# rmcar17/SpectralClusterSupertree

Measured on AMD Instinct MI355X. Metric: top-level PCG build + Fiedler solve wall-time (s) at N taxa, 1/2/4/8 MI355X, lower is better.
Workload: dtype f64 (loop operator: fp32 image of W; fp64 renewal + confirmation)

## Files before the change

spectralclustersupertree_amd/csrc/scs_build.hip:

```cpp

#include <algorithm>

#include "scs_internal.h"

typedef unsigned long long u64;
typedef unsigned int u32;

constexpr u32 DEPTH_INF = 0xFFFFFFFFu;


__device__ __forceinline__ void rmq_offsets(int m, int a, int b, int (&o)[2]) {
    const int k = 31 - __clz(b - a);
    o[0] = k * m + a;
    o[1] = k * m + b - (1 << k);
}

template <typename K>
__device__ __forceinline__ K rmq_min(const K *__restrict__ base, int m, int a, int b) {
    int o[2];
    rmq_offsets(m, a, b, o);
    const K x = base[o[0]], y = base[o[1]];
    return x < y ? x : y;
}

// ... 31 lines not shown
}

__global__ void k_positions_values(const int64_t *__restrict__ tree_off,
                                   const int32_t *__restrict__ leaf_taxon,
                                   const int32_t *__restrict__ adj_depth,
                                   const double *__restrict__ adj_val,
                                   const double *__restrict__ tree_w, int t0, int tl0,
                                   int32_t *__restrict__ pos, int64_t npad,
                                   const int64_t *__restrict__ st_off, double *__restrict__ stv) {
    const int tl = tl0 + blockIdx.y;
    const int t = t0 + tl;
    const int64_t off = tree_off[t];
    const int n = (int)(tree_off[t + 1] - off);
    const int p = blockIdx.x * blockDim.x + threadIdx.x;
    if (p >= n) return;
    const unsigned tx = (unsigned)leaf_taxon[off + p];
    if (tx < (unsigned)npad) pos[(int64_t)tl * npad + tx] = p;
    if (p < n - 1)
        stv[st_off[tl] + p] = adj_depth[off + p] ? adj_val[off + p] * tree_w[t] : 0.0;
}

template <typename K, typename PICK>
__global__ void k_sparse_level(const int64_t *__restrict__ tree_off, int t0, int tl0, int k,
                               const int64_t *__restrict__ st_off, K *__restrict__ st,
                               const int64_t *__restrict__ am_off, argmin_t *__restrict__ am_all, PICK pick) {
    const int tl = tl0 + blockIdx.y;
    const int m = (int)(tree_off[t0 + tl + 1] - tree_off[t0 + tl]) - 1;
    const int p = blockIdx.x * blockDim.x + threadIdx.x;
    if (m < (1 << k) || p > m - (1 << k)) return;
    K *base = st + st_off[tl];
    const int half = 1 << (k - 1);
    const K a = base[(int64_t)(k - 1) * m + p], b = base[(int64_t)(k - 1) * m + p + half];
    base[(int64_t)k * m + p] = pick(a, b);
    if (k > ARGMIN_MAX_LEVEL) return;
    argmin_t *am = am_all + am_off[tl];
    const bool right = pick.right_less(a, b);
    int off = right ? half : 0;
    if (k > 1) off += (int)am[(int64_t)(k - 2) * m + p + (right ? half : 0)];
    am[(int64_t)(k - 1) * m + p] = (argmin_t)off;
}

constexpr int FUSED_UNROLL = 4;
template <typename K, typename PICK>
__global__ __launch_bounds__(1024) void k_sparse_levels_fused(const int64_t *__restrict__ tree_off, int t0, int tl0,
                                                               const int64_t *__restrict__ st_off,
                                                               K *__restrict__ st,
                                                               const int64_t *__restrict__ am_off,
                                                               argmin_t *__restrict__ am_all, PICK pick) {
    const int tl = tl0 + blockIdx.x;
    const int m = (int)(tree_off[t0 + tl + 1] - tree_off[t0 + tl]) - 1;
    K *base = st + st_off[tl];
    argmin_t *am = am_all + am_off[tl];
    for (int k = 1; (1 << k) <= m; ++k) {
        const K *prev = base + (int64_t)(k - 1) * m;
        K *cur = base + (int64_t)k * m;
        const int half = 1 << (k - 1), last = m - (1 << k);
        const argmin_t *am_prev = am + (int64_t)(k - 2) * m;
        argmin_t *am_cur = am + (int64_t)(k - 1) * m;
        for (int p0 = threadIdx.x; p0 <= last; p0 += 1024 * FUSED_UNROLL) {
            K a[FUSED_UNROLL], b[FUSED_UNROLL];
            int oa[FUSED_UNROLL], ob[FUSED_UNROLL];
#pragma unroll
            for (int u = 0; u < FUSED_UNROLL; ++u) {
                const int p = p0 + u * 1024;
                oa[u] = ob[u] = 0;
                if (p <= last) {
                    a[u] = prev[p];
                    b[u] = prev[p + half];
                    if (k > 1) {
                        oa[u] = (int)am_prev[p];
                        ob[u] = (int)am_prev[p + half];
                    }
                }
            }
#pragma unroll
            for (int u = 0; u < FUSED_UNROLL; ++u) {
                const int p = p0 + u * 1024;
                if (p <= last) {
                    cur[p] = pick(a[u], b[u]);
                    am_cur[p] = (argmin_t)(pick.right_less(a[u], b[u]) ? half + ob[u] : oa[u]);
                }
            }
        }
        __syncthreads();
    }
}
constexpr int SPARSE_FUSED_MAX_LEAVES = 32768;
static_assert(SPARSE_FUSED_MAX_LEAVES <= (1 << ARGMIN_MAX_LEVEL), "every level of a fused table has an argmin level");
struct pick_smaller_value {
    __device__ double operator()(double a, double b) const { return a < b ? a : b; }
    __device__ bool right_less(double a, double b) const { return b < a; }
};

__device__ __forceinline__ double min_f64(double a, double b) {
#ifdef SCS_MIN_ASM
    double r;
    asm("v_min_f64 %0, %1, %2" : "=v"(r) : "v"(a), "v"(b));
    return r;
#else
    return __builtin_fmin(a, b);
#endif
}

#include "scs_mono.h"
#include "scs_mono_wide.h"
#include "scs_gen.h"
struct pick_shallower_pair {
    __device__ gap_entry operator()(const gap_entry a, const gap_entry b) const { return gap_min(a, b); }
    __device__ bool right_less(const gap_entry a, const gap_entry b) const { return b.d < a.d; }
};

__global__ __launch_bounds__(256) void k_scatter_atomic(const int64_t *__restrict__ tree_off,
                                                         const int32_t *__restrict__ leaf_taxon, int t0,
                                                         const int64_t *__restrict__ st_off,
                                                         const double *__restrict__ stv,
                                                         double *__restrict__ w, int64_t ld) {
    const int tl = blockIdx.y;
    const int64_t off = tree_off[t0 + tl];
    const int nl = (int)(tree_off[t0 + tl + 1] - off);
    const int m = nl - 1;
    const int nbk = (nl + 63) / 64;
    int I = 0, rest = blockIdx.x;
    while (I < nbk && rest >= nbk - I) {
        rest -= nbk - I;
        ++I;
    }
    if (I >= nbk) return;
    const int J = I + rest;
    __shared__ int s_ta[64], s_tb[64];
    const int tid = threadIdx.x;
    if (tid < 64) s_ta[tid] = I * 64 + tid < nl ? leaf_taxon[off + I * 64 + tid] : -1;
    else if (tid < 128) s_tb[tid - 64] = J * 64 + tid - 64 < nl ? leaf_taxon[off + J * 64 + tid - 64] : -1;
    __syncthreads();
    const double *st = stv + st_off[tl];
    const int bj = tid & 63;
    const int pb = J * 64 + bj;
#pragma unroll 4
    for (int q = 0; q < 16; ++q) {
        const int ai = (tid >> 6) + 4 * q;
        const int pa = I * 64 + ai;
        if (pa >= pb || pb >= nl) continue;
        const double v = rmq_min<double>(st, m, pa, pb);
        if (v != 0.0) {
            const int ta = s_ta[ai], tb2 = s_tb[bj];
            atomicAdd(&w[(int64_t)ta * ld + tb2], v);
            atomicAdd(&w[(int64_t)tb2 * ld + ta], v);
        }
    }
}

__global__ __launch_bounds__(1024) void k_unpack_tiles(const double *__restrict__ gathered,
                                                      const int2 *__restrict__ tiles, int world,
                                                      int64_t chunk_doubles, int n, int row_begin,
                                                      int row_end, double *__restrict__ w,
                                                      int64_t ld) {
    const int tcw = blockDim.x;
    const int t = blockIdx.x;
    const int2 tile = tiles[t];
    const double *src = gathered + (int64_t)(t % world) * chunk_doubles +
                        (int64_t)(t / world) * SCS_TR * tcw;
    const int c = tile.y * tcw + threadIdx.x;
    if (c >= n) return;
    const int r0 = tile.x * SCS_TR;
    const bool col_is_my_row = c >= row_begin && c < row_end;
    for (int i = 0; i < SCS_TR; ++i) {
        const int r = r0 + i;
        if (r >= n) break;
        const double v = src[i * tcw + threadIdx.x];
        if (r >= row_begin && r < row_end) w[(int64_t)(r - row_begin) * ld + c] = v;
        if (col_is_my_row && ((r / tcw) + 1) * tcw <= (c / SCS_TR) * SCS_TR)
            w[(int64_t)(c - row_begin) * ld + r] = v;
    }
}

__global__ __launch_bounds__(256) void k_pack_tiles(const double *__restrict__ tile_out,
                                                    const int32_t *__restrict__ src_slot, int tcw,
                                                    double *__restrict__ sendbuf) {
    const double2 *src = (const double2 *)(tile_out + (int64_t)src_slot[blockIdx.x] * SCS_TR * tcw);
    double2 *dst = (double2 *)(sendbuf + (int64_t)blockIdx.x * SCS_TR * tcw);
    for (int q = threadIdx.x; q < SCS_TR * tcw / 2; q += 256) dst[q] = src[q];
}

__global__ __launch_bounds__(1024) void k_unpack_received(const double *__restrict__ recvbuf,
                                                         const int2 *__restrict__ tiles, int n,
                                                         int row_begin, int row_end,
                                                         double *__restrict__ w, int64_t ld) {
    const int tcw = blockDim.x;
    const int2 tile = tiles[blockIdx.x];
    const double *src = recvbuf + (int64_t)blockIdx.x * SCS_TR * tcw;
    const int c = tile.y * tcw + threadIdx.x;
    if (c >= n) return;
    const int r0 = tile.x * SCS_TR;
    const bool col_is_my_row = c >= row_begin && c < row_end;
    for (int i = 0; i < SCS_TR; ++i) {
        const int r = r0 + i;
        if (r >= n) break;
        const double v = src[i * tcw + threadIdx.x];
        if (r >= row_begin && r < row_end) w[(int64_t)(r - row_begin) * ld + c] = v;
        if (col_is_my_row && ((r / tcw) + 1) * tcw <= (c / SCS_TR) * SCS_TR)
            w[(int64_t)(c - row_begin) * ld + r] = v;
    }
}

__global__ void k_contract(const double *__restrict__ w, int64_t ld, int old_row_begin,
                           const int32_t *__restrict__ gstart, int g_begin, int g_end, int n_groups,
                           double *__restrict__ out, int64_t ld_out) {
    const int h = blockIdx.x * blockDim.x + threadIdx.x;
    if (h >= n_groups) return;
    const int c0 = gstart[h], c1 = gstart[h + 1];
    for (int g = g_begin + blockIdx.y; g < g_end; g += gridDim.y) {
        double best = 0.0;
        if (h != g) {
            const int r0 = gstart[g], r1 = gstart[g + 1];
            best = w[(int64_t)(r0 - old_row_begin) * ld + c0];
            for (int r = r0; r < r1; ++r)
                for (int c = c0; c < c1; ++c) {
                    const double v = w[(int64_t)(r - old_row_begin) * ld + c];
                    best = v > best ? v : best;
                }
        }
        out[(int64_t)(g - g_begin) * ld_out + h] = best;
    }
}

template <bool IMG>
__global__ __launch_bounds__(256) void k_degrees(const double *__restrict__ w, int64_t ld, int n,
                                                  int rows, int row_begin,
                                                  double *__restrict__ deg_full,
                                                  float *__restrict__ w32 = nullptr, int w32_full = 0) {
    const int lane = threadIdx.x & 63;
    const int r = blockIdx.x * 4 + (threadIdx.x >> 6);
    if (r >= rows) return;
    const double *row = w + (int64_t)r * ld;
    double s0 = 0.0, s1 = 0.0;
    const int n2 = n & ~1;
    const int c0 = w32_full ? 0 : (row_begin + r) / 512 * 512;
    float *row32 = IMG ? w32 + (int64_t)r * ld : nullptr;
    for (int j = lane * 2; j < n2; j += 128) {
        const double2 v = *(const double2 *)(row + j);
        s0 += v.x;
        s1 += v.y;
        if (IMG && j >= c0) *(float2 *)(row32 + j) = make_float2((float)v.x, (float)v.y);
    }
    if (IMG)
        for (int j = n2 + lane; j < ld; j += 64) row32[j] = (float)row[j];
    if ((n & 1) && lane == 0) s0 += row[n - 1];
    double s = s0 + s1;
#pragma unroll
    for (int o = 32; o > 0; o >>= 1) s += __shfl_xor(s, o, 64);
    if (lane == 0) deg_full[row_begin + r] = s;
}

__global__ __launch_bounds__(256) void k_degrees_upper_rows(const double *__restrict__ w, int64_t ld, int n,
                                                             int rows, int row_begin, int col0,
                                                             double *__restrict__ part) {
    const int lane = threadIdx.x & 63;
    const int rl = blockIdx.x * 4 + (threadIdx.x >> 6);
    if (rl >= rows) return;
    const int r = row_begin + rl;
    const int c0 = r / 256 * 256;
    const double *row = w + (int64_t)rl * ld + (c0 - col0);
    const int cnt = n - c0;
    double s0 = 0.0, s1 = 0.0;
    const int n2 = cnt & ~1;
    for (int j = lane * 2; j < n2; j += 128) {
        const double2 v = *(const double2 *)(row + j);
        s0 += v.x;
        s1 += v.y;
    }
    if ((cnt & 1) && lane == 0) s0 += row[cnt - 1];
    double s = s0 + s1;
#pragma unroll
    for (int o = 32; o > 0; o >>= 1) s += __shfl_xor(s, o, 64);
    if (lane == 0) part[r] = s;
}

__global__ __launch_bounds__(256) void k_degrees_upper_cols(const double *__restrict__ w, int64_t ld, int n,
                                                             int row_begin, int row_end, int col0,
                                                             double *__restrict__ part) {
    const int c = col0 + blockIdx.x * blockDim.x + threadIdx.x;
    if (c >= n) return;
    const int r_end = min(row_end, c / 256 * 256);
    double s = 0.0;
    for (int r = row_begin; r < r_end; ++r) s += w[(int64_t)(r - row_begin) * ld + (c - col0)];
    if (r_end > row_begin) part[c] += s;
}

__global__ void k_combine_degrees(const double *__restrict__ gathered, int world, int n,
                                  double *__restrict__ deg) {
    const int i = blockIdx.x * blockDim.x + threadIdx.x;
    if (i >= n) return;
    double d = 0.0;
    for (int r = 0; r < world; ++r) d += gathered[(int64_t)r * n + i];
    deg[i] = d;
}

__global__ void k_dinv(const double *__restrict__ deg, int n, double *__restrict__ dinv) {
    const int i = blockIdx.x * blockDim.x + threadIdx.x;
    if (i >= n) return;
    const double d = deg[i];
    dinv[i] = d == 0.0 ? 1.0 : 1.0 / sqrt(d);
}

namespace {

struct dev_buf {
    scs_ctx *ctx;
    void *p = nullptr;
    explicit dev_buf(scs_ctx *c) : ctx(c) {}
    ~dev_buf() {
        if (p) scs_dev_free(p);
    }
    int alloc(size_t bytes) {
        if (p) scs_dev_free(p);
        p = nullptr;
        SCS_HIP_CHECK(scs_dev_malloc(ctx, &p, bytes ? bytes : 16));
        return SCS_OK;
    }
};

struct cached_buf {
    scs_ctx *ctx;
    void *p = nullptr;
    explicit cached_buf(scs_ctx *c) : ctx(c) {}
    ~cached_buf() {
        if (p) scs_block_release(ctx, p);
    }
    int alloc(size_t bytes) {
        if (p) scs_block_release(ctx, p);
        p = nullptr;
        return scs_block_alloc(ctx, bytes, &p);
    }
};

struct pooled_buf {
    scs_ctx *ctx = nullptr;
    int slot = 0;
    void *p = nullptr;
    pooled_buf(scs_ctx *c, int s) : ctx(c), slot(s) {}
    ~pooled_buf() {
        auto &sl = ctx->scratch[slot];
        if (sl.cap > SCS_SCRATCH_KEEP) {
            scs_dev_free(sl.p);
            sl.p = nullptr;
            sl.cap = 0;
        }
    }
    int alloc(size_t bytes) {
        auto &sl = ctx->scratch[slot];
        if (bytes < 16) bytes = 16;
        if (sl.cap < bytes) {
            if (sl.p) scs_dev_free(sl.p);
            sl.p = nullptr;
            sl.cap = 0;
            SCS_HIP_CHECK(scs_dev_malloc(ctx, &sl.p, bytes));
            sl.cap = bytes;
        }
        p = sl.p;
        return SCS_OK;
    }
};

struct ev_pair {
    hipEvent_t a = nullptr, b = nullptr;
    ~ev_pair() {
        if (a) hipEventDestroy(a);
        if (b) hipEventDestroy(b);
    }
    int init() {
        SCS_HIP_CHECK(hipEventCreate(&a));
        SCS_HIP_CHECK(hipEventCreate(&b));
        return SCS_OK;
    }
};

int levels_for(int64_t m) {
    int l = 0;
    while (((int64_t)1 << l) <= m) ++l;
    return l;
}

}

static int graph_alloc(scs_ctx *ctx, int32_t n, int32_t row_begin, int32_t row_end,
                       hipStream_t stream, scs_graph **out, int32_t col0 = 0) {
    auto *g = new scs_graph();
    g->n = n;
    g->row_begin = row_begin;
    g->row_end = row_end;
    g->col0 = col0;
    g->upper = col0 > 0 || false;
    g->ld = scs_round_up(n - col0, SCS_LD_ALIGN);
    const size_t rows = (size_t)(row_end - row_begin);
    size_t bytes = rows * (size_t)g->ld * sizeof(double);
    if (bytes < 16) bytes = 16;
    {
        const int rc = scs_block_alloc(ctx, bytes, (void **)&g->d_w);
        if (rc != SCS_OK) {
            delete g;
            return rc;
        }
        g->w_bytes = bytes;
        g->w_block = true;
    }
    if (g->ld > n - col0) {
        hipError_t e = hipMemset2DAsync(g->d_w + (n - col0), (size_t)g->ld * 8, 0,
                                        (size_t)(g->ld - (n - col0)) * 8, rows, stream);
        if (e != hipSuccess) {
            if (g->w_block) scs_block_release(ctx, g->d_w);
            else scs_dev_free(g->d_w);
            delete g;
            scs_set_error("cannot clear the padding of W: %s", hipGetErrorString(e));
            return SCS_EHIP;
        }
    }
    *out = g;
    return SCS_OK;
}

extern "C" int scs_graph_free(scs_ctx *ctx, scs_graph *g) {
    if (!g) return SCS_OK;
    if (ctx) hipSetDevice(ctx->device);
    if (g->mf) {
        if (ctx) hipStreamSynchronize(ctx->stream);
        scs_matfree_release(g);
    }
    if (ctx && g->d_w && g->w_block) {
        scs_block_release(ctx, g->d_w);
    } else if (ctx && g->d_w) {
        if (!ctx->w_cache || g->w_bytes >= ctx->w_cache_bytes) {
            if (ctx->w_cache) scs_dev_free(ctx->w_cache);
            ctx->w_cache = g->d_w;
            ctx->w_cache_bytes = g->w_bytes;
        } else {
            scs_dev_free(g->d_w);
        }
    } else {
        scs_dev_free(g->d_w);
    }
    if (ctx && g->deg_stage) {
        hipStreamSynchronize(ctx->stream);
        scs_pinned_release(ctx, g->deg_stage);
    }
    if (ctx) {
        if (g->d_w32) {
            std::lock_guard<std::mutex> lock(ctx->cache_mu);
            if (scs_dbg("SCS_TRACE_SOLVES") && atoi(scs_dbg("SCS_TRACE_SOLVES")) && ctx->w32_cache)
                fprintf(stderr, "[image] hipFree of %.2f GB\n",
                        std::min(g->w32_bytes, ctx->w32_cache_bytes) / 1073741824.0);
            scs_dev_free(g->d_w32);
        }
        if (g->d_deg) scs_block_release(ctx, g->d_deg);
        if (g->d_dinv) scs_block_release(ctx, g->d_dinv);
    } else {
        scs_dev_free(g->d_w32);
        scs_dev_free(g->d_deg);
        scs_dev_free(g->d_dinv);
    }
    delete g;
    return SCS_OK;
}

extern "C" int scs_graph_shape(const scs_graph *g, int32_t *n, int32_t *rb, int32_t *re) {
    SCS_REQUIRE(g != nullptr, "scs_graph_shape: null graph");
    if (n) *n = g->n;
    if (rb) *rb = g->row_begin;
    if (re) *re = g->row_end;
    return SCS_OK;
}

int scs_gather_row_splits(scs_ctx *ctx, int32_t row_begin, int32_t row_end, int32_t n,
                          std::vector<int32_t> &splits) {
    const int world = ctx->comm.world;
    splits.assign(world + 1, 0);
    if (world == 1) {
        splits[0] = row_begin;
        splits[1] = row_end;
        return SCS_OK;
    }
    dev_buf send(ctx), recv(ctx);
    SCS_TRY(send.alloc(8));
    SCS_TRY(recv.alloc(8 * (size_t)world));
    double v = (double)row_begin;
    SCS_HIP_CHECK(hipMemcpyAsync(send.p, &v, 8, hipMemcpyHostToDevice, ctx->stream));
    SCS_TRY(scs_comm_allgather_f64(&ctx->comm, (const double *)send.p, (double *)recv.p, 1, ctx->stream));
    std::vector<double> h(world);
    SCS_HIP_CHECK(hipMemcpyAsync(h.data(), recv.p, 8 * (size_t)world, hipMemcpyDeviceToHost, ctx->stream));
    SCS_HIP_CHECK(hipStreamSynchronize(ctx->stream));
    for (int r = 0; r < world; ++r) splits[r] = (int32_t)h[r];
    splits[world] = n;
    for (int r = 0; r < world; ++r)
        SCS_REQUIRE(splits[r] < splits[r + 1], "row partition is not contiguous by rank");
    SCS_REQUIRE(splits[0] == 0 && splits[ctx->comm.rank] == row_begin && splits[ctx->comm.rank + 1] == row_end,
                "row partition does not tile [0, V)");
    return SCS_OK;
}

__global__ __launch_bounds__(64) void k_col_presence(const int32_t *__restrict__ pos, int64_t npad, int n,
                                                      int cols_per_group, int n_batch,
                                                      unsigned char *__restrict__ pcol) {
    const int cg = blockIdx.x, t = blockIdx.y, lane = threadIdx.x;
    bool any = false;
    for (int c = cg * cols_per_group + lane; c < min(n, (cg + 1) * cols_per_group); c += 64)
        any = any || pos[(int64_t)t * npad + c] >= 0;
    if (__ballot(any) != 0 && lane == 0) pcol[(int64_t)cg * n_batch + t] = 1;
    if (__ballot(any) == 0 && lane == 0) pcol[(int64_t)cg * n_batch + t] = 0;
}

__global__ void k_tile_lists(const int2 *__restrict__ tiles, int n_tiles, const unsigned char *__restrict__ rec,
                             int rec_bytes, int cnt_off, int n_batch, const unsigned char *__restrict__ pcol,
                             int32_t *__restrict__ lists, int32_t *__restrict__ list_cnt) {
    const int i = blockIdx.x * blockDim.x + threadIdx.x;
    if (i >= n_tiles) return;
    const int2 tile = tiles[i];
    const unsigned char *rb = rec + (int64_t)tile.x * n_batch * rec_bytes + cnt_off;
    const unsigned char *pc = pcol + (int64_t)tile.y * n_batch;
    int32_t *out = lists + (int64_t)i * n_batch;
    int c = 0;
    for (int t = 0; t < n_batch; ++t)
        if (pc[t] && *(const int *)(rb + (int64_t)t * rec_bytes) > 0) out[c++] = t;
    list_cnt[i] = c;
}

constexpr int PIPE_NG = 2;

namespace {

enum { PREP_MONO = 0, PREP_WIDE = 1, PREP_GEN = 2, PREP_NO_RECORDS = 3 };

struct prep_batch {
    const scs_tables *tb;
    int t0, nb;
    int kind;
    int32_t *pos;
    int64_t npad;
    const int64_t *st_off;
    const int64_t *am_off;
    void *st;
    argmin_t *am;
    unsigned char *rec;
    int n_blocks, row_begin, row_end;
};

int64_t table_entries(int64_t m) { return (int64_t)levels_for(m) * m; }
int64_t argmin_entries(int64_t m) { return (int64_t)argmin_levels(levels_for(m)) * m; }

int prep_piece(const prep_batch &b, int tl0, int np, hipStream_t s) {
    if (np <= 0) return SCS_OK;
    const scs_tables *tb = b.tb;
    int max_levels = 0;
    int64_t max_n = 0;
    for (int t = b.t0 + tl0; t < b.t0 + tl0 + np; ++t) {
        const int64_t nt = tb->h_tree_off[t + 1] - tb->h_tree_off[t];
        max_levels = std::max(max_levels, levels_for(nt - 1));
        max_n = std::max(max_n, nt);
    }
    const dim3 grid_l((unsigned)((max_n + 255) / 256), (unsigned)np);
    const dim3 grid_r((unsigned)b.n_blocks, (unsigned)np);
    const bool fused = max_n <= SPARSE_FUSED_MAX_LEAVES && max_levels > 1;
    if (b.kind != PREP_GEN) {
        double *st = (double *)b.st;
        k_positions_values<<<grid_l, 256, 0, s>>>(tb->d_tree_off, tb->d_leaf_taxon, tb->d_adj_depth, tb->d_adj_val,
                                                  tb->d_tree_w, b.t0, tl0, b.pos, b.npad, b.st_off, st);
        if (fused)
            k_sparse_levels_fused<double><<<(unsigned)np, 1024, 0, s>>>(tb->d_tree_off, b.t0, tl0, b.st_off, st, b.am_off,
                                                                        b.am, pick_smaller_value{});
        else
            for (int k = 1; k < max_levels; ++k)
                k_sparse_level<double><<<grid_l, 256, 0, s>>>(tb->d_tree_off, b.t0, tl0, k, b.st_off, st, b.am_off, b.am,
                                                              pick_smaller_value{});
        if (b.kind == PREP_WIDE)
            k_block_records_wide<PIPE_NG><<<grid_r, 64, 0, s>>>(tb->d_tree_off, b.t0, tl0, b.nb, b.pos, b.npad, b.st_off, st,
                                                          b.am_off, b.am, b.row_begin, b.row_end, b.rec);
        else if (b.kind == PREP_MONO)
            k_block_records_mono<<<grid_r, 64, 0, s>>>(tb->d_tree_off, b.t0, tl0, b.nb, b.pos, b.npad, b.st_off, st,
                                                       b.am_off, b.am, b.row_begin, b.row_end, b.rec);
    } else {
        gap_entry *st = (gap_entry *)b.st;
        k_positions_pairs<<<grid_l, 256, 0, s>>>(tb->d_tree_off, tb->d_leaf_taxon, tb->d_adj_depth, tb->d_adj_val,
                                                 tb->d_tree_w, b.t0, tl0, b.pos, b.npad, b.st_off, st);
        if (fused)
            k_sparse_levels_fused<gap_entry><<<(unsigned)np, 1024, 0, s>>>(tb->d_tree_off, b.t0, tl0, b.st_off, st,
                                                                           b.am_off, b.am, pick_shallower_pair{});
        else
            for (int k = 1; k < max_levels; ++k)
                k_sparse_level<gap_entry><<<grid_l, 256, 0, s>>>(tb->d_tree_off, b.t0, tl0, k, b.st_off, st, b.am_off,
                                                                 b.am, pick_shallower_pair{});
        k_block_records_gen<<<grid_r, 64, 0, s>>>(tb->d_tree_off, b.t0, tl0, b.nb, b.pos, b.npad, b.st_off, st, b.am_off,
                                                  b.am, b.row_begin, b.row_end, b.rec);
    }
    SCS_HIP_CHECK(hipGetLastError());
    return SCS_OK;
}

struct pinned_ref {
    scs_ctx *ctx;
    hipStream_t stream;
    void *p = nullptr;
    bool in_flight = false;
    pinned_ref(scs_ctx *c, hipStream_t s) : ctx(c), stream(s) {}
    ~pinned_ref() {
        if (!p) return;
        if (in_flight) hipStreamSynchronize(stream);
        scs_pinned_release(ctx, p);
    }
};

}

extern "C" int scs_pcg_build(scs_ctx *ctx, const scs_tables *tb, int32_t row_begin,
                             int32_t row_end, int32_t flags, scs_graph **out,
                             scs_build_stats *stats) {
    SCS_REQUIRE(ctx && tb && out, "scs_pcg_build: null argument");
    SCS_REQUIRE((flags & ~(SCS_BUILD_MONOTONE | SCS_BUILD_SHARED | SCS_BUILD_UPPER | SCS_BUILD_SCATTER)) == 0,
                "scs_pcg_build: unknown flag bits 0x%x", flags);
    const bool scatter = (flags & SCS_BUILD_SCATTER) != 0;
    if (scatter && tb) SCS_TRY(scs_tables_finish(ctx, tb));
    if (scatter) {
        if (!(flags & SCS_BUILD_MONOTONE) || (flags & (SCS_BUILD_SHARED | SCS_BUILD_UPPER)) ||
            row_begin != 0 || row_end != tb->n_taxa || ctx->comm.world != 1) {
            scs_set_error("scs_pcg_build: SCS_BUILD_SCATTER (the atomic comparison variant) takes monotone "
                          "tables, the whole matrix, one rank");
            return SCS_EUNSUP;
        }
    }
    SCS_REQUIRE((flags & (SCS_BUILD_SHARED | SCS_BUILD_UPPER)) != (SCS_BUILD_SHARED | SCS_BUILD_UPPER),
                "scs_pcg_build: SCS_BUILD_SHARED and SCS_BUILD_UPPER exclude each other");
    const bool monotone = (flags & SCS_BUILD_MONOTONE) != 0 &&
                          !(scs_dbg("SCS_NO_MONOTONE") && atoi(scs_dbg("SCS_NO_MONOTONE")));
    const int n = tb->n_taxa;
    SCS_REQUIRE(row_begin >= 0 && row_begin < row_end && row_end <= n,
                "scs_pcg_build: bad row range [%d, %d) for %d taxa", row_begin, row_end, n);
    SCS_HIP_CHECK(hipSetDevice(ctx->device));
    hipStream_t s = ctx->stream;
    const int world = ctx->comm.world, rank = ctx->comm.rank;
    const int cols_per_tile = MONO_TCW;
    static_assert(MONO_TCW == SCS_TCW, "one tile width for all kernels");
    const size_t entry_bytes = monotone ? 8 : sizeof(gap_entry);
    size_t rec_bytes = monotone ? R3_BYTES : G3_BYTES;
    const int n_cgroups = (n + cols_per_tile - 1) / cols_per_tile;
    const int64_t npad = scs_round_up((int64_t)n_cgroups * cols_per_tile, SCS_NPAD);
    bool shared = (flags & SCS_BUILD_SHARED) != 0 && world > 1;
    if (shared) {
        const int64_t nb_all = (n + SCS_TR - 1) / SCS_TR;
        const double tile_bytes = 0.5 * (double)nb_all * n_cgroups * SCS_TR * cols_per_tile * 8.0;
        if (tile_bytes * (1.0 + 1.0 / world) > 96.0 * 1024 * 1024 * 1024) shared = false;
    }
    const int b_row_begin = shared ? 0 : row_begin, b_row_end = shared ? n : row_end;
    const bool sym = !shared && (row_begin == 0 && row_end == n && world == 1);
    const bool trapezoid = (flags & SCS_BUILD_UPPER) != 0;
    if (trapezoid)
        SCS_REQUIRE(row_begin % cols_per_tile == 0,
                    "scs_pcg_build: SCS_BUILD_UPPER needs row_begin (%d) to be a multiple of %d", row_begin,
                    cols_per_tile);
    const bool upper = sym || shared || trapezoid;
    const int gb0 = b_row_begin / SCS_TR;
    const int rows = row_end - row_begin;
    const int n_blocks = (b_row_end - b_row_begin + SCS_TR - 1) / SCS_TR;

    scs_graph *g = nullptr;
    SCS_TRY(graph_alloc(ctx, n, row_begin, row_end, s, &g, trapezoid ? row_begin : 0));
    g->upper = trapezoid;
    if (scatter) SCS_HIP_CHECK(hipMemsetAsync(g->d_w, 0, (size_t)rows * (size_t)g->ld * 8, s));
    double *w_base = g->d_w - g->col0;
    struct guard {
        scs_ctx *c;
        scs_graph *g;
        ~guard() {
            if (g) scs_graph_free(c, g);
        }
    } gd{ctx, g};

    std::vector<int2> tiles;
    tiles.reserve((size_t)n_blocks * n_cgroups);
    for (int b = 0; b < n_blocks; ++b)
        for (int c = 0; c < n_cgroups; ++c) {
            if (upper && (int64_t)(c + 1) * cols_per_tile <= (int64_t)(gb0 + b) * SCS_TR) continue;
            tiles.push_back(make_int2(b, c));
        }
    {
        const bool per_xcd = !(scs_dbg("SCS_TILE_ORDER") && atoi(scs_dbg("SCS_TILE_ORDER")) == 0);
        auto xcd_reorder = [](std::vector<int2> &v) {
            if (v.size() <= 8) return;
            std::vector<int2> per[8];
            for (const int2 &t : v) per[t.x & 7].push_back(t);
            std::vector<int2> ordered;
            ordered.reserve(v.size());
            size_t at[8] = {0, 0, 0, 0, 0, 0, 0, 0};
            while (ordered.size() < v.size())
                for (int x = 0; x < 8; ++x)
                    if (at[x] < per[x].size()) ordered.push_back(per[x][at[x]++]);
            v.swap(ordered);
        };
        if (per_xcd && !shared) {
            xcd_reorder(tiles);
        } else if (per_xcd) {
            std::vector<std::vector<int2>> share(world);
            for (size_t i = 0; i < tiles.size(); ++i) share[i % world].push_back(tiles[i]);
            for (auto &v : share) xcd_reorder(v);
            for (int r = 0; r < world; ++r)
                for (size_t k = 0; k < share[r].size(); ++k) tiles[(size_t)world * k + r] = share[r][k];
        }
    }
    std::vector<int2> all_tiles;
    dev_buf d_all_tiles(ctx);
    cached_buf d_tile_out(ctx), d_gathered(ctx);
    size_t chunk_doubles = 0;
    const bool exchange_allgather =
        scs_dbg("SCS_EXCHANGE") && std::string(scs_dbg("SCS_EXCHANGE")) == "allgather";
    if (shared) {
        all_tiles.swap(tiles);
        for (size_t i = rank; i < all_tiles.size(); i += world) tiles.push_back(all_tiles[i]);
        const size_t slots = (all_tiles.size() + world - 1) / world;
        chunk_doubles = slots * SCS_TR * cols_per_tile;
        SCS_TRY(d_all_tiles.alloc(all_tiles.size() * sizeof(int2)));
        SCS_HIP_CHECK(hipMemcpyAsync(d_all_tiles.p, all_tiles.data(),
                                     all_tiles.size() * sizeof(int2), hipMemcpyHostToDevice, s));
        SCS_TRY(d_tile_out.alloc(chunk_doubles * 8));
        if (exchange_allgather) SCS_TRY(d_gathered.alloc(chunk_doubles * 8 * world));
        if (tiles.size() < slots)
            SCS_HIP_CHECK(hipMemsetAsync((double *)d_tile_out.p + (slots - 1) * SCS_TR * cols_per_tile,
                                         0, (size_t)SCS_TR * cols_per_tile * 8, s));
    }
    pooled_buf d_tiles(ctx, 0);
    SCS_TRY(d_tiles.alloc(std::max<size_t>(tiles.size(), 1) * sizeof(int2)));
    SCS_HIP_CHECK(hipMemcpyAsync(d_tiles.p, tiles.data(), tiles.size() * sizeof(int2),
                                 hipMemcpyHostToDevice, s));

    bool tree_par = sym && !scatter && !tiles.empty() && tiles.size() <= 24 && tb->n_trees >= 128;
    if (const char *e = scs_dbg("SCS_TREE_PARALLEL")) tree_par = sym && !scatter && !tiles.empty() && atoi(e) != 0;
    const size_t cells_per_tree = tiles.size() * (size_t)SCS_TR * cols_per_tile * 8;

    const size_t wide_min_tiles = 13;
    bool listed = monotone && !scatter && !tiles.empty() && tb->n_trees > 0 &&
                  (double)tb->n_leaves / ((double)tb->n_trees * std::max(n, 1)) < 1.0 / 64.0;
    if (const char *e = scs_dbg("SCS_TILE_LISTS")) listed = monotone && !scatter && !tiles.empty() && atoi(e) != 0;
    if (listed) tree_par = false;
    int wide_mode = (monotone && !scatter && !tree_par && !listed && tiles.size() >= wide_min_tiles) ? 3 : 0;
    bool wide_forced = false;
    if (const char *e = scs_dbg("SCS_WIDE")) {
        wide_mode = (monotone && !scatter && !tiles.empty() && atoi(e)) ? 3 : 0;
        wide_forced = wide_mode != 0;
        if (wide_mode) listed = false;
    }
    if (wide_mode && ctx->max_lds_bytes < (int)spec_layout::LDS_BYTES) {
        wide_mode = 0;
        wide_forced = false;
    }
    if (wide_mode) tree_par = false;
    const bool wide = wide_mode != 0;
    const int group_tiles = PIPE_NG;
    std::vector<int4> groups;
    dev_buf d_groups(ctx);
    if (wide) {
        rec_bytes = wide_layout<PIPE_NG>::BYTES;
        std::vector<std::vector<int>> of_block((size_t)n_blocks);
        for (size_t i = 0; i < tiles.size(); ++i) of_block[(size_t)tiles[i].x].push_back((int)i);
        std::vector<int4> per[8];
        for (int b = 0; b < n_blocks; ++b) {
            const std::vector<int> &v = of_block[(size_t)b];
            for (size_t k = 0; k < v.size(); k += group_tiles)
                per[b & 7].push_back(make_int4(v[k], k + 1 < v.size() ? v[k + 1] : -1,
                                               (group_tiles > 2 && k + 2 < v.size()) ? v[k + 2] : -1, 0));
        }
        size_t total = 0, at[8] = {0, 0, 0, 0, 0, 0, 0, 0};
        for (auto &v : per) total += v.size();
        groups.reserve(total);
        while (groups.size() < total)
            for (int x = 0; x < 8; ++x)
                if (at[x] < per[x].size()) groups.push_back(per[x][at[x]++]);
        SCS_TRY(d_groups.alloc(groups.size() * sizeof(int4)));
        SCS_HIP_CHECK(hipMemcpyAsync(d_groups.p, groups.data(), groups.size() * sizeof(int4),
                                     hipMemcpyHostToDevice, s));
    }

    const int M = tb->n_trees;
    std::vector<int> batch_start{0};
    {
        const int batch_trees_env = scs_dbg("SCS_BATCH_TREES") ? atoi(scs_dbg("SCS_BATCH_TREES")) : 0;
        int max_batch_trees = 256;
        {
            const double avg_leaves = (double)tb->n_leaves / std::max(M, 1);
            const double table_bytes =
                (double)table_entries((int64_t)std::max(avg_leaves - 1.0, 1.0)) * (double)entry_bytes;
            max_batch_trees = (int)std::min(256.0, std::max(64.0, 600e6 / std::max(table_bytes, 1.0)));
        }
        if (n <= 2048) max_batch_trees = 4096;
        const int arrived = tb->late_start.empty() ? M : tb->late_start[0];
        if (wide) {
            const int rest = M - (arrived < M ? arrived : 0);
            const int k = std::max(1, (rest + 511) / 512);
            max_batch_trees = std::max(96, (rest + k - 1) / k);
        }
        if (tree_par)
            max_batch_trees = (int)std::max<size_t>(16, std::min<size_t>((size_t)max_batch_trees,
                                                                         SCS_SCRATCH_KEEP / cells_per_tree));
        if (batch_trees_env > 0) max_batch_trees = batch_trees_env;
        if (tree_par)
            max_batch_trees = (int)std::max<size_t>(1, std::min<size_t>((size_t)max_batch_trees,
                                                                        SCS_SCRATCH_KEEP / std::max<size_t>(cells_per_tree, 1)));
        size_t used = 0;
        for (int t = 0; t < M; ++t) {
            const int64_t nt = tb->h_tree_off[t + 1] - tb->h_tree_off[t];
            const int64_t m = nt - 1;
            const size_t need = (size_t)table_entries(m) * entry_bytes + (size_t)argmin_entries(m) * sizeof(argmin_t) +
                                (size_t)npad * 4 + (size_t)n_blocks * rec_bytes;
            if ((used + need > ctx->ws_limit || t - batch_start.back() >= max_batch_trees ||
                 (t == arrived && batch_start.size() == 1)) &&
                t > batch_start.back()) {
                batch_start.push_back(t);
                used = 0;
            }
            used += need;
        }
        batch_start.push_back(M);
    }
    const int n_batches = (int)batch_start.size() - 1;

    struct ev_ref {
        hipEvent_t a, b;
    } ev_total, ev_prep, ev_acc;
    for (auto &e : ctx->build_events)
        if (!e) SCS_HIP_CHECK(hipEventCreate(&e));
    ev_total = {ctx->build_events[0], ctx->build_events[1]};
    ev_prep = {ctx->build_events[2], ctx->build_events[3]};
    ev_acc = {ctx->build_events[4], ctx->build_events[5]};
    float prep_ms = 0.f, acc_ms = 0.f;
    SCS_HIP_CHECK(hipEventRecord(ev_total.a, s));

    int spec_batches = 0, spec_trees = 0;
    float spec_ms = 0.f;
    bool single_batch_spec = false;
    pooled_buf d_pos(ctx, 1), d_am(ctx, 2), d_st(ctx, 3), d_stoff(ctx, 4), d_rec(ctx, 5), d_cells(ctx, 6);
    dev_buf d_pcol(ctx), d_lists(ctx), d_list_cnt(ctx);
    int listed_batches = 0;
    std::vector<size_t> off_at((size_t)n_batches + 1, 0);
    for (int bi = 0; bi < n_batches; ++bi)
        off_at[bi + 1] = off_at[bi] + 2 * (size_t)(batch_start[bi + 1] - batch_start[bi] + 1);
    pinned_ref h_off(ctx, s);
    SCS_TRY(scs_pinned_get(ctx, std::max<size_t>(off_at[n_batches], 2) * 8, &h_off.p));
    {
        int64_t *h = (int64_t *)h_off.p;
        for (int bi = 0; bi < n_batches; ++bi) {
            const int t0 = batch_start[bi], nb = batch_start[bi + 1] - t0;
            int64_t *st_off = h + off_at[bi], *am_off = st_off + nb + 1;
            st_off[0] = am_off[0] = 0;
            for (int t = 0; t < nb; ++t) {
                const int64_t m = tb->h_tree_off[t0 + t + 1] - tb->h_tree_off[t0 + t] - 1;
                st_off[t + 1] = st_off[t] + table_entries(m);
                am_off[t + 1] = am_off[t] + argmin_entries(m);
            }
        }
        SCS_TRY(d_stoff.alloc(off_at[n_batches] * 8));
        h_off.in_flight = true;
        SCS_HIP_CHECK(hipMemcpyAsync(d_stoff.p, h, off_at[n_batches] * 8, hipMemcpyHostToDevice, s));
    }
    const bool by_arrival = !(scs_dbg("SCS_PREP_BY_ARRIVAL") && atoi(scs_dbg("SCS_PREP_BY_ARRIVAL")) == 0);
    int prep_pieces = 0;
    for (int bi = 0; bi < n_batches; ++bi) {
        const int t0 = batch_start[bi], t1 = batch_start[bi + 1];
        const int nb = t1 - t0;
        const int64_t *h_st_off = (const int64_t *)h_off.p + off_at[bi], *h_am_off = h_st_off + nb + 1;
        int64_t max_n = 0;
        for (int t = t0; t < t1; ++t) max_n = std::max(max_n, tb->h_tree_off[t + 1] - tb->h_tree_off[t]);
        const size_t need_pos = (size_t)nb * npad * 4;
        const size_t need_st = (size_t)h_st_off[nb] * entry_bytes + 64;
        const size_t need_am = (size_t)h_am_off[nb] * sizeof(argmin_t) + 64;
        const size_t need_rec = (size_t)n_blocks * nb * rec_bytes;
        const int wide_min_trees = wide_forced ? 1 : 96;
        const bool wide_b = wide && (nb >= wide_min_trees || (groups.size() >= 8 * 256 && nb >= 16));
        if (wide_b) {
            ++spec_batches;
            spec_trees += nb;
            single_batch_spec = true;
        }
        SCS_TRY(d_pos.alloc(need_pos));
        SCS_TRY(d_st.alloc(need_st));
        SCS_TRY(d_am.alloc(need_am));
        SCS_TRY(d_rec.alloc(need_rec));

        SCS_HIP_CHECK(hipEventRecord(ev_prep.a, s));
        SCS_HIP_CHECK(hipMemsetAsync(d_pos.p, 0xFF, need_pos, s));
        prep_batch pb;
        pb.tb = tb;
        pb.t0 = t0;
        pb.nb = nb;
        pb.kind = !monotone ? PREP_GEN : wide_b ? PREP_WIDE : scatter ? PREP_NO_RECORDS : PREP_MONO;
        pb.pos = (int32_t *)d_pos.p;
        pb.npad = npad;
        pb.st_off = (const int64_t *)d_stoff.p + off_at[bi];
        pb.am_off = pb.st_off + nb + 1;
        pb.st = d_st.p;
        pb.am = (argmin_t *)d_am.p;
        pb.rec = (unsigned char *)d_rec.p;
        pb.n_blocks = n_blocks;
        pb.row_begin = b_row_begin;
        pb.row_end = b_row_end;
        for (int p0 = t0; p0 < t1;) {
            int p1 = t1;
            if (by_arrival)
                for (const int32_t c : tb->late_start)
                    if (c > p0 && c < p1) p1 = c;
            SCS_TRY(scs_tables_wait(ctx, tb, p1, s));
            SCS_TRY(prep_piece(pb, p0 - t0, p1 - p0, s));
            ++prep_pieces;
            p0 = p1;
        }
        SCS_HIP_CHECK(hipEventRecord(ev_prep.b, s));

        SCS_HIP_CHECK(hipEventRecord(ev_acc.a, s));
        const unsigned nt = (unsigned)tiles.size();
        if (scatter) {
            const int64_t nbk = (max_n + 63) / 64;
            k_scatter_atomic<<<dim3((unsigned)(nbk * (nbk + 1) / 2), (unsigned)nb), 256, 0, s>>>(
                tb->d_tree_off, tb->d_leaf_taxon, t0, pb.st_off, (const double *)d_st.p,
                g->d_w, g->ld);
        } else if (monotone) {
            mono_params mp;
            mp.tiles = (const int2 *)d_tiles.p;
            mp.rec = (const unsigned char *)d_rec.p;
            mp.pos = (const int32_t *)d_pos.p;
            mp.npad = npad;
            mp.stv = (const double *)d_st.p;
            mp.n_batch = nb;
            mp.w = w_base;
            mp.ld = g->ld;
            mp.n = n;
            mp.row_begin = b_row_begin;
            mp.row_end = b_row_end;
            mp.load_w = bi > 0;
            mp.mirror = (sym && bi == n_batches - 1) ? 1 : 0;
            mp.tile_out = shared ? (double *)d_tile_out.p : nullptr;
            mp.stamps = nullptr;
            mp.split_tiles = 0;
            mp.lists = nullptr;
            mp.list_cnt = nullptr;
            const bool stamp = scs_dbg("SCS_ACC_STAMP") && atoi(scs_dbg("SCS_ACC_STAMP"));
            if (wide_b) {
                wide_params wp;
                wp.m = mp;
                wp.groups = (const int4 *)d_groups.p;
                wp.producer_prio = 2;
                const unsigned ng = (unsigned)groups.size();
                dev_buf d_st8(ctx);
                if (stamp) {
                    SCS_TRY(d_st8.alloc(64));
                    SCS_HIP_CHECK(hipMemsetAsync(d_st8.p, 0, 64, s));
                    wp.m.stamps = (unsigned long long *)d_st8.p;
                }
#define SCS_LAUNCH_SPEC(SYM_, STAMP_)                                                                   \
    do {                                                                                                \
        SCS_HIP_CHECK(hipFuncSetAttribute((const void *)k_accumulate_spec<SYM_, STAMP_>,                \
                                          hipFuncAttributeMaxDynamicSharedMemorySize,                   \
                                          (int)spec_layout::LDS_BYTES));                                \
        k_accumulate_spec<SYM_, STAMP_><<<ng, spec_layout::THREADS, spec_layout::LDS_BYTES, s>>>(wp);   \
    } while (0)
                if (ng) {
                    if (stamp && sym) SCS_LAUNCH_SPEC(true, true);
                    else if (stamp) SCS_LAUNCH_SPEC(false, true);
                    else if (sym) SCS_LAUNCH_SPEC(true, false);
                    else SCS_LAUNCH_SPEC(false, false);
                }
#undef SCS_LAUNCH_SPEC
                if (stamp) {
                    unsigned long long h[8];
                    SCS_HIP_CHECK(hipMemcpyAsync(h, d_st8.p, 64, hipMemcpyDeviceToHost, s));
                    SCS_HIP_CHECK(hipStreamSynchronize(s));
                    const char *nm[5] = {"producer: pairs of the next tree", "producer: records + search + wait",
                                         "consumer: pair + table state", "consumer: cells + expansion", "barrier"};
                    double tot = 0;
                    for (int i = 0; i < 5; ++i) tot += (double)h[i];
                    for (int i = 0; i < 5; ++i)
                        fprintf(stderr, "[stamp spec] %-36s %6.2f %%  (%.0f cycles per wave-step)\n", nm[i],
                                100.0 * h[i] / tot, (double)h[i] / ((double)h[7] * nb));
                }
            } else if (nt && stamp) {
                dev_buf d_st8(ctx);
                SCS_TRY(d_st8.alloc(64));
                SCS_HIP_CHECK(hipMemsetAsync(d_st8.p, 0, 64, s));
                mp.stamps = (unsigned long long *)d_st8.p;
                if (sym) k_accumulate_mono<true, true><<<nt, MONO_TCW, 0, s>>>(mp);
                else k_accumulate_mono<false, true><<<nt, MONO_TCW, 0, s>>>(mp);
                unsigned long long h[8];
                SCS_HIP_CHECK(hipMemcpyAsync(h, d_st8.p, 64, hipMemcpyDeviceToHost, s));
                SCS_HIP_CHECK(hipStreamSynchronize(s));
                const char *nm[7] = {"wait loads+record", "barrier A", "combine", "search + issue",
                                     "expand", "barrier B", "cells"};
                double tot = 0;
                for (int i = 0; i < 7; ++i) tot += (double)h[i];
                for (int i = 0; i < 7; ++i)
                    fprintf(stderr, "[stamp] %-24s %6.2f %%  (%.0f cycles per wave-step)\n", nm[i],
                            100.0 * h[i] / tot, (double)h[i] / ((double)h[7] * nb));
            } else if (nt && tree_par) {
                SCS_TRY(d_cells.alloc((size_t)nb * cells_per_tree));
                mono_params ap = mp;
                ap.split_tiles = (int)nt;
                ap.load_w = 0;
                ap.mirror = 0;
                ap.tile_out = (double *)d_cells.p;
                k_accumulate_mono<true, false><<<nt * (unsigned)nb, MONO_TCW, 0, s>>>(ap);
                k_sum_tree_tiles<true, mono_params><<<nt * SCS_TR, MONO_TCW, 0, s>>>(mp, (const double *)d_cells.p,
                                                                                    (int)nt);
            } else if (nt && listed) {
                SCS_TRY(d_pcol.alloc((size_t)n_cgroups * nb));
                SCS_TRY(d_lists.alloc((size_t)nt * nb * 4));
                SCS_TRY(d_list_cnt.alloc((size_t)nt * 4));
                k_col_presence<<<dim3((unsigned)n_cgroups, (unsigned)nb), 64, 0, s>>>(
                    (const int32_t *)d_pos.p, npad, n, cols_per_tile, nb, (unsigned char *)d_pcol.p);
                k_tile_lists<<<(nt + 255) / 256, 256, 0, s>>>((const int2 *)d_tiles.p, (int)nt,
                                                             (const unsigned char *)d_rec.p, R3_BYTES, R3_CNT, nb,
                                                             (const unsigned char *)d_pcol.p, (int32_t *)d_lists.p,
                                                             (int32_t *)d_list_cnt.p);
                mp.lists = (const int32_t *)d_lists.p;
                mp.list_cnt = (const int32_t *)d_list_cnt.p;
                if (sym) k_accumulate_mono<true, false, true><<<nt, MONO_TCW, 0, s>>>(mp);
                else k_accumulate_mono<false, false, true><<<nt, MONO_TCW, 0, s>>>(mp);
                ++listed_batches;
            } else if (nt) {
                if (sym) k_accumulate_mono<true, false><<<nt, MONO_TCW, 0, s>>>(mp);
                else k_accumulate_mono<false, false><<<nt, MONO_TCW, 0, s>>>(mp);
            }
        } else {
            gen_params gp;
            gp.tiles = (const int2 *)d_tiles.p;
            gp.rec = (const unsigned char *)d_rec.p;
            gp.pos = (const int32_t *)d_pos.p;
            gp.npad = npad;
            gp.ste = (const gap_entry *)d_st.p;
            gp.n_batch = nb;
            gp.w = w_base;
            gp.ld = g->ld;
            gp.n = n;
            gp.row_begin = b_row_begin;
            gp.row_end = b_row_end;
            gp.load_w = bi > 0;
            gp.mirror = (sym && bi == n_batches - 1) ? 1 : 0;
            gp.tile_out = shared ? (double *)d_tile_out.p : nullptr;
            gp.split_tiles = 0;
            if (nt && tree_par) {
                SCS_TRY(d_cells.alloc((size_t)nb * cells_per_tree));
                gen_params ap = gp;
                ap.split_tiles = (int)nt;
                ap.load_w = 0;
                ap.mirror = 0;
                ap.tile_out = (double *)d_cells.p;
                k_accumulate_gen<true><<<nt * (unsigned)nb, MONO_TCW, 0, s>>>(ap);
                k_sum_tree_tiles<true, gen_params><<<nt * SCS_TR, MONO_TCW, 0, s>>>(gp, (const double *)d_cells.p,
                                                                                   (int)nt);
            } else if (nt) {
                if (sym) k_accumulate_gen<true><<<nt, MONO_TCW, 0, s>>>(gp);
                else k_accumulate_gen<false><<<nt, MONO_TCW, 0, s>>>(gp);
            }
        }
        SCS_HIP_CHECK(hipGetLastError());
        SCS_HIP_CHECK(hipEventRecord(ev_acc.b, s));
        if (n_batches > 1) {
            SCS_HIP_CHECK(hipEventSynchronize(ev_acc.b));
            float ms = 0.f;
            SCS_HIP_CHECK(hipEventElapsedTime(&ms, ev_prep.a, ev_prep.b));
            prep_ms += ms;
            SCS_HIP_CHECK(hipEventElapsedTime(&ms, ev_acc.a, ev_acc.b));
            acc_ms += ms;
            if (wide_b) spec_ms += ms;
        }
    }
    float exch_ms = 0.f;
    double exch_bytes = 0.0;
    if (shared && exchange_allgather) {
        ev_pair ev_x;
        SCS_TRY(ev_x.init());
        SCS_HIP_CHECK(hipEventRecord(ev_x.a, s));
        SCS_TRY(scs_comm_allgather_f64(&ctx->comm, (const double *)d_tile_out.p,
                                       (double *)d_gathered.p, chunk_doubles, s));
        k_unpack_tiles<<<(unsigned)all_tiles.size(), cols_per_tile, 0, s>>>(
            (const double *)d_gathered.p, (const int2 *)d_all_tiles.p, world,
            (int64_t)chunk_doubles, n, row_begin, row_end, g->d_w, g->ld);
        SCS_HIP_CHECK(hipGetLastError());
        SCS_HIP_CHECK(hipEventRecord(ev_x.b, s));
        SCS_HIP_CHECK(hipEventSynchronize(ev_x.b));
        SCS_HIP_CHECK(hipEventElapsedTime(&exch_ms, ev_x.a, ev_x.b));
        exch_bytes = (double)chunk_doubles * 8.0 * (world - 1);
    } else if (shared) {
        std::vector<int32_t> splits;
        SCS_TRY(scs_gather_row_splits(ctx, row_begin, row_end, n, splits));
        auto needs = [&](int dst, const int2 &t) {
            const int64_t lo = splits[dst], hi = splits[dst + 1];
            const int64_t r_lo = (int64_t)t.x * SCS_TR, r_hi = std::min<int64_t>(r_lo + SCS_TR, n);
            const int64_t c_lo = (int64_t)t.y * cols_per_tile, c_hi = std::min<int64_t>(c_lo + cols_per_tile, n);
            return (r_lo < hi && lo < r_hi) || (c_lo < hi && lo < c_hi);
        };
        std::vector<int64_t> send_off(world + 1, 0), recv_off(world + 1, 0);
        std::vector<int32_t> send_slots;
        std::vector<int2> recv_tiles;
        for (int p = 0; p < world; ++p) {
            for (size_t i = rank; i < all_tiles.size(); i += world)
                if (needs(p, all_tiles[i])) send_slots.push_back((int32_t)(i / world));
            send_off[p + 1] = (int64_t)send_slots.size() * SCS_TR * cols_per_tile;
            for (size_t i = p; i < all_tiles.size(); i += world)
                if (needs(rank, all_tiles[i])) recv_tiles.push_back(all_tiles[i]);
            recv_off[p + 1] = (int64_t)recv_tiles.size() * SCS_TR * cols_per_tile;
        }
        cached_buf d_send(ctx), d_recv(ctx);
        dev_buf d_slots(ctx), d_rtiles(ctx);
        SCS_TRY(d_send.alloc((size_t)send_off[world] * 8));
        SCS_TRY(d_recv.alloc((size_t)recv_off[world] * 8));
        SCS_TRY(d_slots.alloc(send_slots.size() * 4));
        SCS_TRY(d_rtiles.alloc(recv_tiles.size() * sizeof(int2)));
        ev_pair ev_x;
        SCS_TRY(ev_x.init());
        SCS_HIP_CHECK(hipEventRecord(ev_x.a, s));
        SCS_HIP_CHECK(hipMemcpyAsync(d_slots.p, send_slots.data(), send_slots.size() * 4,
                                     hipMemcpyHostToDevice, s));
        SCS_HIP_CHECK(hipMemcpyAsync(d_rtiles.p, recv_tiles.data(), recv_tiles.size() * sizeof(int2),
                                     hipMemcpyHostToDevice, s));
        if (!send_slots.empty())
            k_pack_tiles<<<(unsigned)send_slots.size(), 256, 0, s>>>(
                (const double *)d_tile_out.p, (const int32_t *)d_slots.p, cols_per_tile, (double *)d_send.p);
        SCS_HIP_CHECK(hipGetLastError());
        SCS_TRY(scs_comm_alltoallv_f64(&ctx->comm, (const double *)d_send.p, send_off.data(),
                                       (double *)d_recv.p, recv_off.data(), s));
        if (!recv_tiles.empty())
            k_unpack_received<<<(unsigned)recv_tiles.size(), cols_per_tile, 0, s>>>(
                (const double *)d_recv.p, (const int2 *)d_rtiles.p, n, row_begin, row_end, g->d_w,
                g->ld);
        SCS_HIP_CHECK(hipGetLastError());
        SCS_HIP_CHECK(hipEventRecord(ev_x.b, s));
        SCS_HIP_CHECK(hipEventSynchronize(ev_x.b));
        SCS_HIP_CHECK(hipEventElapsedTime(&exch_ms, ev_x.a, ev_x.b));
        exch_bytes = (double)(recv_off[world] - (recv_off[rank + 1] - recv_off[rank])) * 8.0;
    }
    SCS_HIP_CHECK(hipEventRecord(ev_total.b, s));
    SCS_HIP_CHECK(hipEventSynchronize(ev_total.b));
    h_off.in_flight = false;
    SCS_TRY(scs_tables_finish(ctx, tb));
    float total_ms = 0.f;
    SCS_HIP_CHECK(hipEventElapsedTime(&total_ms, ev_total.a, ev_total.b));
    if (n_batches == 1) {
        SCS_HIP_CHECK(hipEventElapsedTime(&prep_ms, ev_prep.a, ev_prep.b));
        SCS_HIP_CHECK(hipEventElapsedTime(&acc_ms, ev_acc.a, ev_acc.b));
        if (single_batch_spec) spec_ms = acc_ms;
    }

    if (stats) {
        memset(stats, 0, sizeof(*stats));
        stats->n_taxa = n;
        stats->n_trees = M;
        stats->row_begin = row_begin;
        stats->row_end = row_end;
        stats->symmetric = shared ? 2 : (sym ? 1 : 0);
        stats->exchange_ms = exch_ms;
        stats->exchange_bytes = exch_bytes;
        stats->n_tiles = (int32_t)tiles.size();
        stats->n_batches = n_batches;
        stats->spec_batches = spec_batches;
        stats->tree_parallel_batches = tree_par ? n_batches : 0;
        stats->spec_trees = spec_trees;
        stats->listed_batches = listed_batches;
        stats->prep_pieces = prep_pieces;
        stats->spec_ms = spec_ms;
        stats->cell_trees = (double)tiles.size() * SCS_TR * cols_per_tile * (double)M;
        stats->prep_ms = prep_ms;
        stats->accumulate_ms = acc_ms;
        stats->total_ms = total_ms;
        stats->bytes_w = 8.0 * rows * (double)n;
        stats->bytes_tables = 16.0 * (double)tb->n_leaves + 8.0 * M;
    }
    gd.g = nullptr;
    *out = g;
    return SCS_OK;
}

extern "C" int scs_graph_contract(scs_ctx *ctx, scs_graph *g, const int32_t *group_start,
                                  int32_t n_groups, scs_graph **out) {
    SCS_REQUIRE(ctx && g && group_start && out, "scs_graph_contract: null argument");
    if (g->mf) {
        scs_set_error("scs_graph_contract: a matrix-free graph has no matrix to contract");
        return SCS_EUNSUP;
    }
    if (g->upper) {
        scs_set_error("scs_graph_contract: an SCS_BUILD_UPPER graph holds no whole rows; build it "
                      "row-partitioned (SCS_BUILD_SHARED) when the node contracts");
        return SCS_EUNSUP;
    }
    SCS_REQUIRE(n_groups >= 1 && n_groups <= g->n, "scs_graph_contract: bad group count %d",
                n_groups);
    SCS_REQUIRE(group_start[0] == 0 && group_start[n_groups] == g->n,
                "scs_graph_contract: group_start must span [0, %d]", g->n);
    int g_begin = -1, g_end = -1;
    for (int i = 0; i < n_groups; ++i) {
        SCS_REQUIRE(group_start[i] < group_start[i + 1], "scs_graph_contract: empty group %d", i);
        if (group_start[i] == g->row_begin) g_begin = i;
        if (group_start[i + 1] == g->row_end) g_end = i + 1;
    }
    SCS_REQUIRE(g_begin >= 0 && g_end > g_begin,
                "scs_graph_contract: a group straddles this rank's row block [%d, %d)",
                g->row_begin, g->row_end);
    SCS_HIP_CHECK(hipSetDevice(ctx->device));
    scs_graph *ng = nullptr;
    SCS_TRY(graph_alloc(ctx, n_groups, g_begin, g_end, ctx->stream, &ng));
    int32_t *d_gs = nullptr;
    hipError_t e = scs_dev_malloc(ctx, (void **)&d_gs, (size_t)(n_groups + 1) * 4);
    if (e != hipSuccess) {
        scs_graph_free(ctx, ng);
        scs_set_error("scs_graph_contract: hipMalloc failed: %s", hipGetErrorString(e));
        return SCS_ENOMEM;
    }
    hipMemcpyAsync(d_gs, group_start, (size_t)(n_groups + 1) * 4, hipMemcpyHostToDevice,
                   ctx->stream);
    dim3 grid((unsigned)((n_groups + 255) / 256), (unsigned)std::min(g_end - g_begin, 65535));
    k_contract<<<grid, 256, 0, ctx->stream>>>(g->d_w, g->ld, g->row_begin, d_gs, g_begin, g_end,
                                              n_groups, ng->d_w, ng->ld);
    e = hipGetLastError();
    if (e == hipSuccess) e = hipStreamSynchronize(ctx->stream);
    scs_dev_free(d_gs);
    if (e != hipSuccess) {
        scs_graph_free(ctx, ng);
        scs_set_error("scs_graph_contract: kernel failed: %s", hipGetErrorString(e));
        return SCS_EHIP;
    }
    scs_graph_free(ctx, g);
    *out = ng;
    return SCS_OK;
}

extern "C" int scs_graph_download_rows(scs_ctx *ctx, const scs_graph *g, int32_t first, int32_t count,
                                       double *out);

extern "C" int scs_graph_download(scs_ctx *ctx, const scs_graph *g, double *out) {
    SCS_REQUIRE(ctx && g && out, "scs_graph_download: null argument");
    SCS_REQUIRE(!g->mf, "scs_graph_download: a matrix-free graph has no matrix");
    SCS_HIP_CHECK(hipSetDevice(ctx->device));
    SCS_HIP_CHECK(hipStreamSynchronize(ctx->stream));
    const size_t rows = (size_t)(g->row_end - g->row_begin);
    if (g->upper) return scs_graph_download_rows(ctx, g, g->row_begin, (int32_t)rows, out);
    SCS_HIP_CHECK(hipMemcpy2D(out, (size_t)g->n * 8, g->d_w, (size_t)g->ld * 8, (size_t)g->n * 8,
                              rows, hipMemcpyDeviceToHost));
    return SCS_OK;
}

extern "C" int scs_graph_download_rows(scs_ctx *ctx, const scs_graph *g, int32_t first,
                                       int32_t count, double *out) {
    SCS_REQUIRE(ctx && g && out, "scs_graph_download_rows: null argument");
    SCS_REQUIRE(!g->mf, "scs_graph_download_rows: a matrix-free graph has no matrix");
    SCS_REQUIRE(count >= 1 && first >= g->row_begin && first + count <= g->row_end,
                "scs_graph_download_rows: rows [%d, %d) outside this rank's block [%d, %d)", first,
                first + count, g->row_begin, g->row_end);
    SCS_HIP_CHECK(hipSetDevice(ctx->device));
    SCS_HIP_CHECK(hipStreamSynchronize(ctx->stream));
    if (g->upper) {
        const size_t wcols = (size_t)(g->n - g->col0);
        for (int32_t i = 0; i < count; ++i) memset(out + (size_t)i * g->n, 0, (size_t)g->n * 8);
        SCS_HIP_CHECK(hipMemcpy2D(out + g->col0, (size_t)g->n * 8,
                                  g->d_w + (int64_t)(first - g->row_begin) * g->ld, (size_t)g->ld * 8,
                                  wcols * 8, (size_t)count, hipMemcpyDeviceToHost));
        for (int32_t i = 0; i < count; ++i) {
            const int32_t c0 = (first + i) / 256 * 256;
            if (c0 > g->col0) memset(out + (size_t)i * g->n + g->col0, 0, (size_t)(c0 - g->col0) * 8);
        }
        return SCS_OK;
    }
    SCS_HIP_CHECK(hipMemcpy2D(out, (size_t)g->n * 8, g->d_w + (int64_t)(first - g->row_begin) * g->ld,
                              (size_t)g->ld * 8, (size_t)g->n * 8, (size_t)count,
                              hipMemcpyDeviceToHost));
    return SCS_OK;
}

int scs_graph_prepare_degrees_begin(scs_ctx *ctx, scs_graph *g, bool want_w32) {
    if (g->deg_stage) return SCS_OK;
    const int n = g->n;
    const int rows = g->row_end - g->row_begin;
    if (g->mf && !g->have_deg) {
        SCS_HIP_CHECK(hipSetDevice(ctx->device));
        hipStream_t s = ctx->stream;
        if (!g->d_deg) SCS_TRY(scs_block_alloc(ctx, (size_t)n * 8, (void **)&g->d_deg));
        if (!g->d_dinv) SCS_TRY(scs_block_alloc(ctx, (size_t)n * 8, (void **)&g->d_dinv));
        SCS_TRY(scs_matfree_apply(ctx, g, nullptr, 0, 4, nullptr, s));
        k_dinv<<<(n + 255) / 256, 256, 0, s>>>(g->d_deg, n, g->d_dinv);
        SCS_HIP_CHECK(hipGetLastError());
        SCS_TRY(scs_pinned_get(ctx, (size_t)n * 8, &g->deg_stage));
        SCS_HIP_CHECK(hipMemcpyAsync(g->deg_stage, g->d_deg, (size_t)n * 8, hipMemcpyDeviceToHost, s));
        return SCS_OK;
    }
    const bool img_rows = ctx->comm.world > 1 && !g->upper;
    bool need_img = want_w32 && !g->have_w32 && !g->upper &&
                    (img_rows || (ctx->comm.world == 1 && g->row_begin == 0 && rows == n));
    if (g->have_deg && !need_img) return SCS_OK;
    SCS_HIP_CHECK(hipSetDevice(ctx->device));
    hipStream_t s = ctx->stream;
    if (need_img && !g->d_w32) {
        const size_t need = (size_t)rows * g->ld * 4;
        std::lock_guard<std::mutex> lock(ctx->cache_mu);
        if (ctx->w32_cache && ctx->w32_cache_bytes >= need) {
            g->d_w32 = ctx->w32_cache;
            g->w32_bytes = ctx->w32_cache_bytes;
            ctx->w32_cache = nullptr;
            ctx->w32_cache_bytes = 0;
        } else if (scs_dev_malloc(ctx, (void **)&g->d_w32, need) == hipSuccess) {
            g->w32_bytes = need;
            if (scs_dbg("SCS_TRACE_SOLVES") && atoi(scs_dbg("SCS_TRACE_SOLVES")))
                fprintf(stderr, "[image] hipMalloc of %.2f GB\n", need / 1073741824.0);
        } else {
            (void)hipGetLastError();
            g->d_w32 = nullptr;
            need_img = false;
        }
    }
    if (!need_img && g->have_deg) return SCS_OK;
    if (need_img && img_rows && g->have_deg) {
        dev_buf tmp(ctx);
        SCS_TRY(tmp.alloc((size_t)n * 8));
        k_degrees<true><<<(rows + 3) / 4, 256, 0, s>>>(g->d_w, g->ld, n, rows, g->row_begin, (double *)tmp.p, g->d_w32, 1);
        SCS_HIP_CHECK(hipGetLastError());
        SCS_HIP_CHECK(hipStreamSynchronize(s));
        g->have_w32 = true;
        return SCS_OK;
    }
    if (!g->d_deg) SCS_TRY(scs_block_alloc(ctx, (size_t)n * 8, (void **)&g->d_deg));
    if (!g->d_dinv) SCS_TRY(scs_block_alloc(ctx, (size_t)n * 8, (void **)&g->d_dinv));
    const int world = ctx->comm.world;
    if (need_img && !img_rows) {
        k_degrees<true><<<(rows + 3) / 4, 256, 0, s>>>(g->d_w, g->ld, n, rows, g->row_begin, g->d_deg, g->d_w32);
        g->have_w32 = true;
    } else if (world == 1 && !g->upper) {
        k_degrees<false><<<(rows + 3) / 4, 256, 0, s>>>(g->d_w, g->ld, n, rows, g->row_begin, g->d_deg);
    } else {
        dev_buf send(ctx), recv(ctx);
        SCS_TRY(send.alloc((size_t)n * 8));
        SCS_TRY(recv.alloc((size_t)n * 8 * world));
        SCS_HIP_CHECK(hipMemsetAsync(send.p, 0, (size_t)n * 8, s));
        if (g->upper) {
            k_degrees_upper_rows<<<(rows + 3) / 4, 256, 0, s>>>(g->d_w, g->ld, n, rows, g->row_begin,
                                                                g->col0, (double *)send.p);
            k_degrees_upper_cols<<<(n - g->col0 + 255) / 256, 256, 0, s>>>(
                g->d_w, g->ld, n, g->row_begin, g->row_end, g->col0, (double *)send.p);
        } else if (need_img) {
            k_degrees<true><<<(rows + 3) / 4, 256, 0, s>>>(g->d_w, g->ld, n, rows, g->row_begin, (double *)send.p,
                                                           g->d_w32, 1);
            g->have_w32 = true;
        } else
        k_degrees<false><<<(rows + 3) / 4, 256, 0, s>>>(g->d_w, g->ld, n, rows, g->row_begin,
                                                        (double *)send.p);
        SCS_TRY(scs_comm_allgather_f64(&ctx->comm, (const double *)send.p, (double *)recv.p,
                                       (size_t)n, s));
        k_combine_degrees<<<(n + 255) / 256, 256, 0, s>>>((const double *)recv.p, world, n, g->d_deg);
        SCS_HIP_CHECK(hipGetLastError());
        SCS_HIP_CHECK(hipStreamSynchronize(s));
    }
    if (g->have_deg) {
        SCS_HIP_CHECK(hipGetLastError());
        return SCS_OK;
    }
    k_dinv<<<(n + 255) / 256, 256, 0, s>>>(g->d_deg, n, g->d_dinv);
    SCS_HIP_CHECK(hipGetLastError());
    SCS_TRY(scs_pinned_get(ctx, (size_t)n * 8, &g->deg_stage));
    SCS_HIP_CHECK(hipMemcpyAsync(g->deg_stage, g->d_deg, (size_t)n * 8, hipMemcpyDeviceToHost, s));
    return SCS_OK;
}

int scs_graph_prepare_degrees(scs_ctx *ctx, scs_graph *g) {
    if (g->have_deg) return SCS_OK;
    SCS_TRY(scs_graph_prepare_degrees_begin(ctx, g));
    const hipError_t e = hipStreamSynchronize(ctx->stream);
    const double *deg = (const double *)g->deg_stage;
    int iso = 0;
    double nrm2 = 0.0;
    if (e == hipSuccess)
        for (int i = 0; i < g->n; ++i) {
            if (deg[i] == 0.0) {
                ++iso;
                nrm2 += 1.0;
            } else {
                nrm2 += deg[i];
            }
        }
    scs_pinned_release(ctx, g->deg_stage);
    g->deg_stage = nullptr;
    SCS_HIP_CHECK(e);
    g->n_isolated = iso;
    g->dd_norm = sqrt(nrm2);
    g->have_deg = true;
    return SCS_OK;
}

extern "C" int scs_graph_degrees(scs_ctx *ctx, scs_graph *g, double *out) {
    SCS_REQUIRE(ctx && g && out, "scs_graph_degrees: null argument");
    SCS_TRY(scs_graph_prepare_degrees(ctx, g));
    SCS_HIP_CHECK(hipMemcpy(out, g->d_deg + g->row_begin,
                            (size_t)(g->row_end - g->row_begin) * 8, hipMemcpyDeviceToHost));
    return SCS_OK;
}

extern "C" int scs_debug_graph_raw(scs_ctx *ctx, scs_graph *g, int32_t what, void *out, int32_t *info_out) {
    SCS_REQUIRE(ctx && g && info_out, "scs_debug_graph_raw: null argument");
    SCS_REQUIRE(what >= 0 && what <= 2, "scs_debug_graph_raw: what must be 0 (W), 1 (image) or 2 (degrees), not %d",
                what);
    if (g->mf && what != 2) {
        scs_set_error("scs_debug_graph_raw: a matrix-free graph has neither a matrix nor an image");
        return SCS_EUNSUP;
    }
    const int rows = g->row_end - g->row_begin;
    const bool img_rows = ctx->comm.world > 1;
    if (what == 1) {
        if (g->upper) {
            scs_set_error("scs_debug_graph_raw: an SCS_BUILD_UPPER graph has no image");
            return SCS_EUNSUP;
        }
        if (!img_rows && !(g->row_begin == 0 && rows == g->n)) {
            scs_set_error("scs_debug_graph_raw: a row block [%d, %d) of %d on one rank has no image", g->row_begin,
                          g->row_end, g->n);
            return SCS_EUNSUP;
        }
    }
    info_out[0] = rows;
    info_out[1] = (int32_t)g->ld;
    info_out[2] = g->col0;
    info_out[3] = (what == 1 && img_rows) ? 1 : 0;
    if (!out) return SCS_OK;
    SCS_HIP_CHECK(hipSetDevice(ctx->device));
    if (what == 1) {
        SCS_TRY(scs_graph_prepare_degrees_begin(ctx, g, true));
        SCS_TRY(scs_graph_prepare_degrees(ctx, g));
        if (!g->have_w32 || !g->d_w32) {
            scs_set_error("scs_debug_graph_raw: the image could not be made (no memory)");
            return SCS_EUNSUP;
        }
    }
    if (what == 2) SCS_TRY(scs_graph_prepare_degrees(ctx, g));
    SCS_HIP_CHECK(hipStreamSynchronize(ctx->stream));
    if (what == 2)
        SCS_HIP_CHECK(hipMemcpy(out, g->d_deg, (size_t)g->n * 8, hipMemcpyDeviceToHost));
    else if (what == 1)
        SCS_HIP_CHECK(hipMemcpy(out, g->d_w32, (size_t)rows * (size_t)g->ld * 4, hipMemcpyDeviceToHost));
    else
        SCS_HIP_CHECK(hipMemcpy(out, g->d_w, (size_t)rows * (size_t)g->ld * 8, hipMemcpyDeviceToHost));
    return SCS_OK;
}

extern "C" int scs_debug_block_records(scs_ctx *ctx, const scs_tables *tb, int32_t t_begin, int32_t t_end,
                                       int32_t row_begin, int32_t row_end, int32_t kind, int32_t *spos_out,
                                       double *gap_out, int32_t *argpos_out, int32_t *depth_out, int32_t *cnt_out) {
    SCS_REQUIRE(ctx && tb && spos_out && gap_out && argpos_out && cnt_out, "scs_debug_block_records: null argument");
    SCS_REQUIRE(kind == PREP_MONO || kind == PREP_WIDE || kind == PREP_GEN,
                "scs_debug_block_records: kind must be 0 (mono), 1 (wide) or 2 (general), not %d", kind);
    SCS_REQUIRE(t_begin >= 0 && t_begin < t_end && t_end <= tb->n_trees,
                "scs_debug_block_records: bad tree range [%d, %d) of %d", t_begin, t_end, tb->n_trees);
    SCS_REQUIRE(row_begin >= 0 && row_begin < row_end && row_end <= tb->n_taxa,
                "scs_debug_block_records: bad row range [%d, %d) for %d taxa", row_begin, row_end, tb->n_taxa);
    SCS_HIP_CHECK(hipSetDevice(ctx->device));
    hipStream_t s = ctx->stream;
    const int n = tb->n_taxa, nb = t_end - t_begin;
    const int n_blocks = (row_end - row_begin + SCS_TR - 1) / SCS_TR;
    const int n_cgroups = (n + MONO_TCW - 1) / MONO_TCW;
    const int64_t npad = scs_round_up((int64_t)n_cgroups * MONO_TCW, SCS_NPAD);
    const size_t entry_bytes = kind == PREP_GEN ? sizeof(gap_entry) : 8;
    const size_t rec_bytes = kind == PREP_GEN ? G3_BYTES : kind == PREP_WIDE ? wide_layout<PIPE_NG>::BYTES : R3_BYTES;
    std::vector<int64_t> off(2 * (size_t)(nb + 1), 0);
    int64_t *st_off = off.data(), *am_off = off.data() + nb + 1;
    for (int t = 0; t < nb; ++t) {
        const int64_t m = tb->h_tree_off[t_begin + t + 1] - tb->h_tree_off[t_begin + t] - 1;
        st_off[t + 1] = st_off[t] + table_entries(m);
        am_off[t + 1] = am_off[t] + argmin_entries(m);
    }
    dev_buf d_pos(ctx), d_st(ctx), d_am(ctx), d_off(ctx), d_rec(ctx);
    const size_t need_pos = (size_t)nb * npad * 4, need_rec = (size_t)n_blocks * nb * rec_bytes;
    SCS_TRY(d_pos.alloc(need_pos));
    SCS_TRY(d_st.alloc((size_t)st_off[nb] * entry_bytes + 64));
    SCS_TRY(d_am.alloc((size_t)am_off[nb] * sizeof(argmin_t) + 64));
    SCS_TRY(d_off.alloc(off.size() * 8));
    SCS_TRY(d_rec.alloc(need_rec));
    SCS_HIP_CHECK(hipMemcpy(d_off.p, off.data(), off.size() * 8, hipMemcpyHostToDevice));
    SCS_HIP_CHECK(hipMemsetAsync(d_pos.p, 0xFF, need_pos, s));
    prep_batch pb;
    pb.tb = tb;
    pb.t0 = t_begin;
    pb.nb = nb;
    pb.kind = kind;
    pb.pos = (int32_t *)d_pos.p;
    pb.npad = npad;
    pb.st_off = (const int64_t *)d_off.p;
    pb.am_off = pb.st_off + nb + 1;
    pb.st = d_st.p;
    pb.am = (argmin_t *)d_am.p;
    pb.rec = (unsigned char *)d_rec.p;
    pb.n_blocks = n_blocks;
    pb.row_begin = row_begin;
    pb.row_end = row_end;
    SCS_TRY(scs_tables_wait(ctx, tb, t_end, s));
    SCS_TRY(prep_piece(pb, 0, nb, s));
    std::vector<unsigned char> rec(need_rec);
    SCS_HIP_CHECK(hipMemcpyAsync(rec.data(), d_rec.p, need_rec, hipMemcpyDeviceToHost, s));
    SCS_HIP_CHECK(hipStreamSynchronize(s));
    const int o_spos = kind == PREP_GEN ? G3_SPOS : kind == PREP_WIDE ? wide_layout<PIPE_NG>::SPOS : R3_SPOS;
    const int o_gap = kind == PREP_GEN ? G3_GV : kind == PREP_WIDE ? wide_layout<PIPE_NG>::G : R3_G;
    const int o_arg = kind == PREP_GEN ? G3_ARGPOS : kind == PREP_WIDE ? wide_layout<PIPE_NG>::ARGPOS : R3_ARGPOS;
    const int o_cnt = kind == PREP_GEN ? G3_CNT : kind == PREP_WIDE ? wide_layout<PIPE_NG>::CNT : R3_CNT;
    for (size_t i = 0; i < (size_t)n_blocks * nb; ++i) {
        const unsigned char *r = rec.data() + i * rec_bytes;
        memcpy(spos_out + i * 64, r + o_spos, 256);
        memcpy(gap_out + i * 64, r + o_gap, 512);
        memcpy(argpos_out + i * 64, r + o_arg, 256);
        if (kind == PREP_GEN && depth_out) memcpy(depth_out + i * 64, r + G3_GD, 256);
        memcpy(cnt_out + i, r + o_cnt, 4);
    }
    return SCS_OK;
}
```

spectralclustersupertree_amd/csrc/scs_eig.hip:

```cpp

#include <algorithm>
#include <chrono>
#include <cmath>

#include "scs_internal.h"
#include "scs_policy.h"
#include "scs_symm.h"
#include "scs_matfree.h"
#include "scs_symm_tri.h"

#include <sched.h>
#include "scs_panel.h"

constexpr int MAXB = 16;
constexpr int MAXS = 64;
constexpr int SLD = MAXS + 1;

typedef double v4d __attribute__((ext_vector_type(4)));

__global__ void k_scale_rows(const double *__restrict__ x, int ldx, int c0, int b, int n,
                             const double *__restrict__ dinv, double *__restrict__ zt,
                             int64_t ldz) {
    const int idx = blockIdx.x * blockDim.x + threadIdx.x;
    if (idx >= n * b) return;
// ... 1822 lines not shown
            k_unpack<<<(nb + 255) / 256, 256, 0, s>>>(recv.d(), chunk, b,
                                                      (const int32_t *)splits_d.p, world, n,
                                                      yfull.d());
            yf = yfull.d();
        }
        k_store_cols<<<(nb + 255) / 256, 256, 0, s>>>(yf, b, n, dst, 3 * b, c0d);
        return SCS_OK;
    }

    int gram(const double *a, int lda, int ka, const double *bm, int ldb, int kb, double *out,
             bool mfma) {
        const int nout = ka * kb;
        int nparts;
        if (mfma && ka <= 48 && kb <= 48) {
            nparts = std::min(gram_blocks, std::max(1, (n + 3) / 4));
            const int ta = (ka + 15) / 16, tb = (kb + 15) / 16;
#define GM(TA, TB)                                                                               \
    if (ta == TA && tb == TB)                                                                    \
        k_gram_mfma<TA, TB><<<nparts, 64, 0, s>>>(a, lda, ka, bm, ldb, kb, n, part.d());
            GM(1, 1) GM(1, 2) GM(1, 3) GM(2, 1) GM(2, 2) GM(2, 3) GM(3, 1) GM(3, 2) GM(3, 3)
#undef GM
        } else {
            nparts = std::min(gram_blocks, std::max(1, (n + GRAM_CH - 1) / GRAM_CH));
            k_gram<<<nparts, 256, 0, s>>>(a, lda, ka, bm, ldb, kb, n, part.d());
        }
        k_reduce_partials<<<(nout + 3) / 4, 256, 0, s>>>(part.d(), nparts, nout, out);
        SCS_HIP_CHECK(hipGetLastError());
        return SCS_OK;
    }

    int update(double *y, int ldy, int kc, double alpha, const double *a, int lda, int ka,
               const double *c, int ldc, double sign) {
        k_update<<<(n + 15) / 16, 256, 0, s>>>(y, ldy, kc, alpha, a, lda, ka, c, ldc, sign, n);
        SCS_HIP_CHECK(hipGetLastError());
        return SCS_OK;
    }

    static int panel_cap() {
        static const int cap = PANEL_BLOCKS_MAX;
        return cap;
    }
    int panel_blocks16() const { return std::max(1, std::min(panel_cap(), ((n + 15) / 16 + 3) / 4)); }
    int panel_blocks4() const { return std::max(1, std::min(panel_cap(), ((n + 3) / 4 + 3) / 4)); }

    template <int B>
    int fused_front(const double *uvec, const double *c, const double *d, const double *theta,
                    double *coef, int *mask_r, double drop_tol, double *report, double seq) {
        const int nb = panel_blocks16();
        k_panel_rr<B><<<nb, 256, 0, s>>>(q.d(), aq.d(), uvec, c, d, theta, n, part.d());
        k_small_orth<<<1, 256, 0, s>>>(part.d(), nb, B, drop_tol, coef, mask_r, theta, report, seq);
        k_panel_tf<B, true, false><<<nb, 256, 0, s>>>(q.d(), uvec, coef, n, part.d(), nullptr,
                                                      nullptr, 0);
        k_small_orth<<<1, 256, 0, s>>>(part.d(), nb, B, 0.0, coef, mask_r, theta, nullptr, 0.0);
        k_panel_tf<B, false, true><<<nb, 256, 0, s>>>(q.d(), uvec, coef, n, nullptr, g->d_dinv,
                                                      z.d(), ldz);
        SCS_HIP_CHECK(hipGetLastError());
        return SCS_OK;
    }

    template <int B>
    int fused_front_solve(const double *uvec, int nparts_in, int solve, double *theta,
                          const int *maskp_in, int *mask_r, int *maskp_out, double drop_tol,
                          double *report, double seq) {
        const int nb = panel_blocks16();
        if (overlap_pass1) {
            k_panel_rr_solve<B><<<nb, 256, 0, s>>>(q.d(), aq.d(), uvec, part3.d(), nparts_in, solve, theta,
                                                   maskp_in, mask_r, maskp_out, drop_tol, n, part.d(),
                                                   g->d_dinv, z.d(), ldz, B);
            SCS_HIP_CHECK(hipGetLastError());
            tf1.armed = true;
            tf1.drop_tol = drop_tol;
            tf1.report = report;
            tf1.seq = seq;
            return SCS_OK;
        }
        if (fold_pass2) {
            k_panel_rr_solve<B><<<nb, 256, 0, s>>>(q.d(), aq.d(), uvec, part3.d(), nparts_in, solve, theta,
                                                   maskp_in, mask_r, maskp_out, drop_tol, n, part.d(), nullptr,
                                                   nullptr, 0, gram_from32 ? B : -1);
            k_panel_tf_solve<B, true, true><<<nb, 256, 0, s>>>(q.d(), uvec, part.d(), nb, drop_tol, mask_r,
                                                               theta, report, seq, n, part2.d(), g->d_dinv,
                                                               z.d(), ldz);
            SCS_HIP_CHECK(hipGetLastError());
            return SCS_OK;
        }
        k_panel_rr_solve<B><<<nb, 256, 0, s>>>(q.d(), aq.d(), uvec, part2.d(), nparts_in, solve, theta,
                                               maskp_in, mask_r, maskp_out, drop_tol, n, part.d(), nullptr,
                                               nullptr, 0, gram_from32 ? B : -1);
        k_panel_tf_solve<B, true, false><<<nb, 256, 0, s>>>(q.d(), uvec, part.d(), nb, drop_tol, mask_r,
                                                            theta, report, seq, n, part2.d(), nullptr,
                                                            nullptr, 0);
        k_panel_tf_solve<B, false, true><<<nb, 256, 0, s>>>(q.d(), uvec, part2.d(), nb, 0.0, mask_r, theta,
                                                            nullptr, 0.0, n, nullptr, g->d_dinv, z.d(),
                                                            ldz);
        SCS_HIP_CHECK(hipGetLastError());
        return SCS_OK;
    }

    template <int B>
    int fused_back(int *nparts, double *pout) {
        hipEvent_t e0 = nullptr, e1 = nullptr;
        const bool timed = (n_apply & 3) == 0;
        time_ag = timed && world > 1;
        if (timed) {
            SCS_TRY(new_event(&e0));
            SCS_TRY(new_event(&e1));
            ev.push_back(e0);
            ev.push_back(e1);
            ev32.push_back(use32 ? 1 : 0);
        }
        gram_from32 = use32;
        const int nb = fold_pass2 ? panel_blocks16() : panel_blocks4();
        const int nb16 = panel_blocks16();
        *nparts = nb;
        if (part_mode) {
            if (timed) SCS_HIP_CHECK(hipEventRecord(e0, s));
            SCS_TRY(launch_symm(z.d(), nullptr));
            if (timed) SCS_HIP_CHECK(hipEventRecord(e1, s));
            ++n_apply;
            if (fold_pass2)
                k_panel_gram_tf_solve<B, 3><<<nb, 256, 0, s>>>(q.d(), aq.d(), fold_u, part2.d(), nb16, fold_mask_r,
                                                               fold_theta, n, recv.d(), world, g->d_dinv, pout);
            else
                k_gram_qaq<B, 3><<<nb, 256, 0, s>>>(q.d(), aq.d(), n, recv.d(), world, g->d_dinv, pout);
        } else if (world == 1) {
            if (timed) SCS_HIP_CHECK(hipEventRecord(e0, s));
            SCS_TRY(launch_symm(z.d(), nullptr));
            if (timed) SCS_HIP_CHECK(hipEventRecord(e1, s));
            ++n_apply;
            if (fold_pass2)
                k_panel_gram_tf_solve<B, 1><<<nb, 256, 0, s>>>(q.d(), aq.d(), fold_u, part2.d(), nb16, fold_mask_r,
                                                               fold_theta, n, ypart.d(), last_nseg, g->d_dinv, pout,
                                                               0, nullptr, overlap_pass1 ? coef1.d() : nullptr);
            else
                k_gram_qaq<B, 1><<<nb, 256, 0, s>>>(q.d(), aq.d(), n, ypart.d(), last_nseg,
                                                       g->d_dinv, pout);
        } else {
            if (timed) SCS_HIP_CHECK(hipEventRecord(e0, s));
            SCS_TRY(launch_symm(z.d(), yloc.d()));
            if (timed) SCS_HIP_CHECK(hipEventRecord(e1, s));
            ++n_apply;
            SCS_TRY(gather(yloc.d(), recv.d(), (size_t)chunk));
            if (fold_pass2)
                k_panel_gram_tf_solve<B, 2><<<nb, 256, 0, s>>>(q.d(), aq.d(), fold_u, part2.d(), nb16, fold_mask_r,
                                                               fold_theta, n, recv.d(), world, g->d_dinv, pout,
                                                               (int64_t)chunk, (const int32_t *)splits_d.p);
            else
                k_gram_qaq<B, 2><<<nb, 256, 0, s>>>(q.d(), aq.d(), n, recv.d(), world, g->d_dinv, pout,
                                                    (int64_t)chunk, (const int32_t *)splits_d.p);
        }
        time_ag = false;
        SCS_HIP_CHECK(hipGetLastError());
        return SCS_OK;
    }
};

constexpr int SM_G = 0;
constexpr int SM_T = SM_G + 48 * 48;
constexpr int SM_C = SM_T + 48 * 16;
constexpr int SM_D = SM_C + 48 * 16;
constexpr int SM_THETA = SM_D + 48 * 16;
constexpr int SM_RN = SM_THETA + 32;
constexpr int SM_MASK = SM_RN + 32;
constexpr int SM_TOTAL = SM_MASK + 32;

void sign_flip_and_store(const std::vector<double> &col0, const std::vector<double> &col1, int n,
                         double *maps) {
    for (int c = 0; c < 2; ++c) {
        const std::vector<double> &v = c == 0 ? col0 : col1;
        int arg = 0;
        double best = -1.0;
        for (int i = 0; i < n; ++i)
            if (std::fabs(v[i]) > best) {
                best = std::fabs(v[i]);
                arg = i;
            }
        const double sg = v[arg] < 0.0 ? -1.0 : 1.0;
        for (int i = 0; i < n; ++i) maps[(size_t)i * 2 + c] = sg * v[i];
    }
}

}

static int gather_full_rows(scs_ctx *ctx, scs_graph *g, std::vector<int32_t> &splits) {
    return scs_gather_row_splits(ctx, g->row_begin, g->row_end, g->n, splits);
}

static int fiedler_dense_onesided(scs_ctx *ctx, scs_graph *g, double *maps, scs_stats *st) {
    const int n = g->n;
    hipStream_t s = ctx->stream;
    SCS_REQUIRE(ctx->comm.world == 1 && !g->upper, "dense path needs the whole matrix on one rank (V = %d)", n);
    dbuf sd, wv, vv;
    SCS_TRY(sd.alloc((size_t)n * n * 8));
    SCS_TRY(wv.alloc(4 * 8));
    SCS_TRY(vv.alloc((size_t)n * 2 * 8));
    k_dense_s<<<(n * n + 255) / 256, 256, 0, s>>>(g->d_w, g->ld, n, g->d_dinv, sd.d());
    const size_t lds = (size_t)(n + (n & 1)) * DENSE2_LD * sizeof(double);
    SCS_HIP_CHECK(hipFuncSetAttribute((const void *)k_dense_onesided, hipFuncAttributeMaxDynamicSharedMemorySize,
                                      DENSE2_MAX * DENSE2_LD * (int)sizeof(double)));
    k_dense_onesided<<<1, 256, lds, s>>>(sd.d(), n, wv.d(), vv.d());
    SCS_HIP_CHECK(hipGetLastError());
    std::vector<double> w(4), v((size_t)n * 2), dinv(n);
    SCS_HIP_CHECK(hipMemcpyAsync(w.data(), wv.p, 4 * 8, hipMemcpyDeviceToHost, s));
    SCS_HIP_CHECK(hipMemcpyAsync(v.data(), vv.p, (size_t)n * 2 * 8, hipMemcpyDeviceToHost, s));
    SCS_HIP_CHECK(hipMemcpyAsync(dinv.data(), g->d_dinv, (size_t)n * 8, hipMemcpyDeviceToHost, s));
    SCS_HIP_CHECK(hipStreamSynchronize(s));
    std::vector<double> c0(n), c1(n);
    for (int i = 0; i < n; ++i) {
        c0[i] = v[(size_t)i * 2 + 0] * dinv[i];
        c1[i] = v[(size_t)i * 2 + 1] * dinv[i];
    }
    sign_flip_and_store(c0, c1, n, maps);
    if (st) {
        st->block = 0;
        st->converged = w[3] != 0.0 ? 1 : 0;
        st->lambda[0] = w[0];
        st->lambda[1] = w[1];
        st->lambda_next = w[2];
    }
    if (w[3] == 0.0) {
        scs_set_error("scs_fiedler: the dense one-sided Jacobi did not converge in 40 sweeps (V = %d)", n);
        return SCS_ENOCONV;
    }
    return SCS_OK;
}

static int fiedler_dense(scs_ctx *ctx, scs_graph *g, double *maps, scs_stats *st) {
    const int n = g->n;
    hipStream_t s = ctx->stream;
    SCS_REQUIRE(ctx->comm.world == 1, "dense small-V path needs world == 1 (V = %d)", n);
    dbuf sd, wv, vv;
    SCS_TRY(sd.alloc((size_t)n * n * 8));
    SCS_TRY(wv.alloc((size_t)n * 8));
    SCS_TRY(vv.alloc((size_t)n * n * 8));
    k_dense_s<<<(n * n + 255) / 256, 256, 0, s>>>(g->d_w, g->ld, n, g->d_dinv, sd.d());
    k_small_eig<<<1, 256, 0, s>>>(sd.d(), n, wv.d(), vv.d());
    std::vector<double> w(n), v((size_t)n * n), dinv(n);
    SCS_HIP_CHECK(hipMemcpyAsync(w.data(), wv.p, (size_t)n * 8, hipMemcpyDeviceToHost, s));
    SCS_HIP_CHECK(hipMemcpyAsync(v.data(), vv.p, (size_t)n * n * 8, hipMemcpyDeviceToHost, s));
    SCS_HIP_CHECK(hipMemcpyAsync(dinv.data(), g->d_dinv, (size_t)n * 8, hipMemcpyDeviceToHost, s));
    SCS_HIP_CHECK(hipStreamSynchronize(s));
    std::vector<double> c0(n), c1(n);
    for (int i = 0; i < n; ++i) {
        c0[i] = v[(size_t)i * n + 0] * dinv[i];
        c1[i] = (n > 1 ? v[(size_t)i * n + 1] : 0.0) * dinv[i];
    }
    sign_flip_and_store(c0, c1, n, maps);
    if (st) {
        st->block = 0;
        st->converged = 1;
        st->lambda[0] = w[0];
        st->lambda[1] = n > 1 ? w[1] : 0.0;
        st->lambda_next = n > 2 ? w[2] : 0.0;
    }
    return SCS_OK;
}

extern "C" int scs_fiedler(scs_ctx *ctx, scs_graph *g, const double *x_init, double tol,
                           int32_t max_iter, int32_t block, double *maps_out, scs_stats *stats) {
    SCS_REQUIRE(ctx && g && maps_out, "scs_fiedler: null argument");
    SCS_REQUIRE(g->n >= 2, "scs_fiedler: need at least 2 vertices (have %d)", g->n);
    SCS_REQUIRE(!g->upper || g->n > MAXS, "scs_fiedler: an SCS_BUILD_UPPER graph needs more than %d vertices", MAXS);
    SCS_REQUIRE(block >= 0 && block <= MAXB, "scs_fiedler: block must be in [0, %d]", MAXB);
    SCS_REQUIRE(tol > 0.0 && max_iter >= 1, "scs_fiedler: tol must be > 0 and max_iter >= 1");
    SCS_HIP_CHECK(hipSetDevice(ctx->device));
    t_ctx = ctx;
    hipStream_t s = ctx->stream;
    const int n = g->n;
    scs_stats st_local;
    scs_stats *st = stats ? stats : &st_local;
    memset(st, 0, sizeof(*st));
    st->n_vertices = n;

    for (auto &e : ctx->solve_events)
        if (!e) SCS_HIP_CHECK(hipEventCreate(&e));
    hipEvent_t ev_a = ctx->solve_events[0], ev_b = ctx->solve_events[1];
    SCS_HIP_CHECK(hipEventRecord(ev_a, s));
    const auto t_entry = std::chrono::steady_clock::now();

    if (n <= DENSE2_MAX) SCS_TRY(scs_graph_prepare_degrees(ctx, g));

    static const int dense_max = 96;
    if (n > MAXS && n <= dense_max && block == 0 && ctx->comm.world == 1 && !g->upper) {
        SCS_TRY(fiedler_dense_onesided(ctx, g, maps_out, st));
        SCS_HIP_CHECK(hipEventRecord(ev_b, s));
        SCS_HIP_CHECK(hipEventSynchronize(ev_b));
        float ms = 0.f;
        hipEventElapsedTime(&ms, ev_a, ev_b);
        st->solve_ms = ms;
        return SCS_OK;
    }
    if (n <= MAXS) {
        SCS_TRY(fiedler_dense(ctx, g, maps_out, st));
        SCS_HIP_CHECK(hipEventRecord(ev_b, s));
        SCS_HIP_CHECK(hipEventSynchronize(ev_b));
        float ms = 0.f;
        hipEventElapsedTime(&ms, ev_a, ev_b);
        st->solve_ms = ms;
        return SCS_OK;
    }

    const int lowp_mode = getenv("SCS_LOWP") ? atoi(getenv("SCS_LOWP")) : 2;
    const double lowp_tol = 1e-8, lowp_tol2 = 0.0;
    const bool loop_fused = !(scs_dbg("SCS_LEGACY_LOOP") && atoi(scs_dbg("SCS_LEGACY_LOOP"))) &&
                            !(scs_dbg("SCS_SPLIT_SMALL") && atoi(scs_dbg("SCS_SPLIT_SMALL"))) &&
                            !(scs_dbg("SCS_FOLD_PASS2") && !atoi(scs_dbg("SCS_FOLD_PASS2")));
    const double lowp_max_bytes = getenv("SCS_LOWP_MAX_BYTES") ? atof(getenv("SCS_LOWP_MAX_BYTES")) : 16.0 * (1u << 30);
    const bool image_rows = ctx->comm.world > 1 && !g->upper;
    const bool image_one = ctx->comm.world == 1 && !g->upper && g->row_begin == 0 && g->row_end == n;
    const bool image_ok = !g->mf && lowp_mode > 0 && n >= 4096 && loop_fused && (image_one || image_rows) &&
                          (g->have_w32 || 4.0 * (double)(g->row_end - g->row_begin) * (double)g->ld <= lowp_max_bytes);
    int b = block ? block : ((n >= 16384 && !image_ok) ? 8 : 4);
    if (g->upper && b > 8) b = 8;
    if (g->mf) b = std::min(b <= 4 ? 4 : 8, g->mf->b_cap);
    {
        const int allowed[] = {16, 12, 8, 4};
        const int cap = (n - 2) / 3;
        int pick = 4;
        for (int a : allowed)
            if (a <= b && a <= cap) {
                pick = a;
                break;
            }
        b = pick;
    }
    const int q3 = 3 * b;

    const bool want32 = image_ok && b == 4;
    SCS_TRY(scs_graph_prepare_degrees_begin(ctx, g, want32));

    solver sv;
    sv.ctx = ctx;
    sv.g = g;
    sv.s = s;
    sv.n = n;
    sv.b = b;
    sv.rows = g->row_end - g->row_begin;
    sv.world = ctx->comm.world;
    sv.use_mfma = !(scs_dbg("SCS_NO_MFMA") && atoi(scs_dbg("SCS_NO_MFMA")));
    sv.gram_blocks = 256;
    SCS_TRY(gather_full_rows(ctx, g, sv.splits));
    int max_rows = 0;
    for (int r = 0; r < sv.world; ++r)
        max_rows = std::max(max_rows, sv.splits[r + 1] - sv.splits[r]);
    sv.chunk = g->upper ? (int64_t)n * b : (int64_t)max_rows * b;

    SCS_TRY(sv.q.alloc((size_t)n * q3 * 8));
    SCS_TRY(sv.aq.alloc((size_t)n * q3 * 8));
    SCS_TRY(sv.alloc_symm_buffers());
    SCS_TRY(sv.yloc.alloc((size_t)sv.chunk * 8));
    SCS_TRY(sv.u.alloc((size_t)n * 8));
    SCS_TRY(sv.part.alloc((size_t)1024 * q3 * q3 * 8));
    SCS_TRY(sv.part2.alloc((size_t)1024 * q3 * q3 * 8));
    SCS_TRY(sv.part3.alloc((size_t)1024 * q3 * q3 * 8));
    SCS_TRY(sv.small.alloc((size_t)SM_TOTAL * 8));
    if (sv.world > 1 && !sv.part_mode) {
        SCS_TRY(sv.yfull.alloc((size_t)n * b * 8));
        SCS_TRY(sv.recv.alloc((size_t)sv.chunk * sv.world * 8));
        SCS_TRY(sv.splits_d.alloc((size_t)(sv.world + 1) * 4));
        SCS_HIP_CHECK(hipMemcpyAsync(sv.splits_d.p, sv.splits.data(), (size_t)(sv.world + 1) * 4,
                                     hipMemcpyHostToDevice, s));
    }
    SCS_HIP_CHECK(hipMemsetAsync(sv.q.p, 0, (size_t)n * q3 * 8, s));
    SCS_HIP_CHECK(hipMemsetAsync(sv.aq.p, 0, (size_t)n * q3 * 8, s));
    SCS_HIP_CHECK(hipMemsetAsync(sv.yloc.p, 0, (size_t)sv.chunk * 8, s));
    SCS_HIP_CHECK(hipMemsetAsync(sv.small.p, 0, (size_t)SM_TOTAL * 8, s));

    double *Q = sv.q.d(), *AQ = sv.aq.d();
    double *X = Q, *R = Q + 2 * b;
    double *AX = AQ;
    double *G = sv.small_at(SM_G), *T = sv.small_at(SM_T), *C = sv.small_at(SM_C);
    double *D = sv.small_at(SM_D);
    double *TH = sv.small_at(SM_THETA), *RN = sv.small_at(SM_RN);
    int *MASK = (int *)sv.small_at(SM_MASK);
    const double drop_tol = 1e-13;

    SCS_TRY(scs_graph_prepare_degrees(ctx, g));
    sv.use32 = want32 && g->have_w32 && (sv.tri ? sv.tri_ct == 2 : (image_rows && !sv.part_mode));
    scs_loop_policy policy;
    policy.tol = tol;
    policy.lowp_mode = lowp_mode;
    policy.lowp_tol = lowp_tol;
    policy.lowp_tol2 = lowp_tol2;
    policy.lowp_state = sv.use32 ? 1 : 0;
    const bool constrained = g->n_isolated == 0;
    const int want = constrained ? 1 : 2;

    dbuf x0d;
    if (x_init) {
        SCS_TRY(x0d.alloc((size_t)n * 8));
        SCS_HIP_CHECK(hipMemcpyAsync(x0d.p, x_init, (size_t)n * 8, hipMemcpyHostToDevice, s));
    }
    if (constrained)
        k_trivial<<<(n + 255) / 256, 256, 0, s>>>(g->d_deg, 1.0 / g->dd_norm, n, sv.u.d());

    auto project_u = [&](double *Y, int passes) -> int {
        if (!constrained) return SCS_OK;
        for (int pass = 0; pass < passes; ++pass) {
            SCS_TRY(sv.gram(sv.u.d(), 1, 1, Y, q3, b, C, false));
            SCS_TRY(sv.update(Y, q3, b, 1.0, sv.u.d(), 1, 1, C, b, -1.0));
        }
        return SCS_OK;
    };
    auto svqb = [&](double *Y, double *AY, int *mask_out) -> int {
        for (int pass = 0; pass < 2; ++pass) {
            SCS_TRY(sv.gram(Y, q3, b, Y, q3, b, G, sv.use_mfma));
            k_small_svqb<<<1, 256, 0, s>>>(G, b, pass == 0 ? drop_tol : 0.0, T, mask_out);
            SCS_TRY(sv.update(Y, q3, b, 0.0, Y, q3, b, T, b, 1.0));
            if (AY) SCS_TRY(sv.update(AY, q3, b, 0.0, AY, q3, b, T, b, 1.0));
        }
        return SCS_OK;
    };

    k_init_block<<<(n * b + 255) / 256, 256, 0, s>>>(Q, b, n, x_init ? x0d.d() : nullptr);
    SCS_TRY(project_u(X, 2));
    SCS_TRY(svqb(X, nullptr, MASK));
    SCS_TRY(sv.apply(Q, 0, AQ, 0));
    SCS_TRY(sv.gram(X, q3, b, AX, q3, b, G, sv.use_mfma));
    {
        k_fill_int<<<1, 64, 0, s>>>(MASK, 48, 1);
        k_small_rr<<<1, 256, 0, s>>>(G, 0, b, b, MASK, T, D, TH, MASK + b, drop_tol);
        SCS_TRY(sv.update(X, q3, b, 0.0, X, q3, b, T, b, 1.0));
        SCS_TRY(sv.update(AX, q3, b, 0.0, AX, q3, b, T, b, 1.0));
        k_fill_int<<<1, 64, 0, s>>>(MASK + b, b, 0);
    }

    const int res_blocks = (n + 255) / 256;
    dbuf res_part;
    SCS_TRY(res_part.alloc((size_t)res_blocks * b * 8));
    std::vector<double> h_rn(b), h_th(b + 1);
    int iter = 0;
    bool converged = false;
    double final_res[2] = {0.0, 0.0};

    const bool fused = (b == 4 || b == 8) &&
                       !(scs_dbg("SCS_LEGACY_LOOP") && atoi(scs_dbg("SCS_LEGACY_LOOP")));
    if (fused) {
        if (!ctx->h_report) {
            SCS_HIP_CHECK(hipHostMalloc((void **)&ctx->h_report, 64 * sizeof(double),
                                        hipHostMallocMapped | hipHostMallocCoherent));
            SCS_HIP_CHECK(hipHostGetDevicePointer((void **)&ctx->d_report, ctx->h_report, 0));
            memset(ctx->h_report, 0, 64 * sizeof(double));
        }
        k_unit_coeffs<<<(3 * b * b + 255) / 256, 256, 0, s>>>(T, D, b);
    }
    const double *uvec = constrained ? sv.u.d() : nullptr;
    const bool split_small = scs_dbg("SCS_SPLIT_SMALL") && atoi(scs_dbg("SCS_SPLIT_SMALL"));
    sv.fold_pass2 = fused && !split_small && !(scs_dbg("SCS_FOLD_PASS2") && !atoi(scs_dbg("SCS_FOLD_PASS2")));
    sv.overlap_pass1 = sv.fold_pass2 && sv.tri && !sv.part_mode && sv.world == 1 &&
                       !(scs_dbg("SCS_OVERLAP_PASS1") && !atoi(scs_dbg("SCS_OVERLAP_PASS1")));
    if (sv.overlap_pass1) SCS_TRY(sv.coef1.alloc((size_t)(3 * 8 + 4) * 8 * 8));
    sv.fold_u = uvec;
    sv.fold_mask_r = MASK + 2 * b;
    sv.fold_theta = TH;
    double *qaq_out = sv.fold_pass2 ? sv.part3.d() : sv.part2.d();
    int rr_solve = 0, rr_parts = 0, mpar = 0;
    int *maskp[2] = {MASK + b, MASK + 32};

    for (iter = 0; iter < max_iter; ++iter) {
        if (fused) {
            int nparts = 0;
            const double seq = (double)(++ctx->report_seq);
            if (!split_small) {
                if (b == 4) {
                    SCS_TRY(sv.fused_front_solve<4>(uvec, rr_parts, rr_solve, TH, maskp[mpar], MASK + 2 * b,
                                                    maskp[mpar ^ 1], drop_tol, ctx->d_report, seq));
                    SCS_TRY(sv.fused_back<4>(&nparts, qaq_out));
                } else {
                    SCS_TRY(sv.fused_front_solve<8>(uvec, rr_parts, rr_solve, TH, maskp[mpar], MASK + 2 * b,
                                                    maskp[mpar ^ 1], drop_tol, ctx->d_report, seq));
                    SCS_TRY(sv.fused_back<8>(&nparts, qaq_out));
                }
                rr_parts = nparts;
                rr_solve = 1;
                mpar ^= 1;
            } else {
                if (b == 4) {
                    SCS_TRY(sv.fused_front<4>(uvec, T, D, TH, C, MASK + 2 * b, drop_tol, ctx->d_report, seq));
                    SCS_TRY(sv.fused_back<4>(&nparts, sv.part.d()));
                } else {
                    SCS_TRY(sv.fused_front<8>(uvec, T, D, TH, C, MASK + 2 * b, drop_tol, ctx->d_report, seq));
                    SCS_TRY(sv.fused_back<8>(&nparts, sv.part.d()));
                }
                k_small_rr<<<1, 256, 0, s>>>(sv.part.d(), nparts, q3, b, MASK, T, D, TH, MASK + b,
                                             drop_tol);
            }
            SCS_HIP_CHECK(hipGetLastError());
            {
                volatile double *hr = (volatile double *)ctx->h_report;
                const auto t_wait = std::chrono::steady_clock::now();
                unsigned spins = 0;
                while (hr[40] != seq) {
                    __builtin_ia32_pause();
                    if (spins > (1u << 18) && (spins & 0x3FF) == 0) sched_yield();
                    if ((++spins & 0xFFFF) == 0) {
                        const hipError_t qe = hipStreamQuery(s);
                        if (qe != hipSuccess && qe != hipErrorNotReady) {
                            scs_set_error("scs_fiedler: stream failed: %s", hipGetErrorString(qe));
                            return SCS_EHIP;
                        }
                        if (qe == hipSuccess && hr[40] != seq) {
                            if (std::chrono::steady_clock::now() - t_wait > std::chrono::seconds(5)) {
                                scs_set_error("scs_fiedler: residual report lost at iteration %d", iter);
                                return SCS_EHIP;
                            }
                        }
                    }
                }
            }
            for (int j = 0; j < b; ++j) h_rn[j] = ((volatile double *)ctx->h_report)[j];
            for (int j = 0; j <= b; ++j) h_th[j] = ((volatile double *)ctx->h_report)[16 + j];
        } else {
            k_residual<<<res_blocks, 256, 0, s>>>(Q, AQ, b, TH, n, res_part.d());
            k_reduce_partials<<<(b + 3) / 4, 256, 0, s>>>(res_part.d(), res_blocks, b, RN);
            SCS_HIP_CHECK(hipMemcpyAsync(h_rn.data(), RN, (size_t)b * 8, hipMemcpyDeviceToHost, s));
            SCS_HIP_CHECK(hipMemcpyAsync(h_th.data(), TH, (size_t)(b + 1) * 8, hipMemcpyDeviceToHost, s));
            SCS_HIP_CHECK(hipStreamSynchronize(s));
        }
        double worst = 0.0;
        for (int j = 0; j < want; ++j) worst = std::max(worst, std::sqrt(h_rn[j]));
        for (int j = 0; j < want; ++j) final_res[constrained ? 1 : j] = std::sqrt(h_rn[j]);
        static const bool trace_res = scs_dbg("SCS_TRACE_RESIDUAL") && atoi(scs_dbg("SCS_TRACE_RESIDUAL"));
        if (trace_res) fprintf(stderr, "[lobpcg] it %3d  residual %.3e  theta %.12g %.12g\n", iter, worst, h_th[0], h_th[1]);
        if (!(worst == worst)) {
            scs_set_error("scs_fiedler: NaN residual at iteration %d", iter);
            return SCS_EHIP;
        }
        const int action = policy.step(worst);
        const bool stop = action == scs_loop_policy::STOP;
        if (action == scs_loop_policy::RENEW) {
            sv.use32 = false;
            SCS_TRY(sv.apply(Q, 0, AQ, 0));
            SCS_TRY(sv.apply(Q, b, AQ, b));
            sv.use32 = policy.image_in_use();
            ++st->lowp_renewals;
        }
        if (stop) {
            sv.use32 = false;
            if (policy.begin_confirmation()) {
                SCS_TRY(sv.apply(Q, 0, AQ, 0));
                SCS_TRY(sv.gram(X, q3, b, AX, q3, b, G, sv.use_mfma));
                k_fill_int<<<1, 64, 0, s>>>(MASK, 48, 1);
                k_small_rr<<<1, 256, 0, s>>>(G, 0, b, b, MASK, T, D, TH, MASK + b, drop_tol);
                SCS_TRY(sv.update(X, q3, b, 0.0, X, q3, b, T, b, 1.0));
                SCS_TRY(sv.update(AX, q3, b, 0.0, AX, q3, b, T, b, 1.0));
                k_fill_int<<<1, 64, 0, s>>>(MASK + b, b, 0);
                k_residual<<<res_blocks, 256, 0, s>>>(Q, AQ, b, TH, n, res_part.d());
                k_reduce_partials<<<(b + 3) / 4, 256, 0, s>>>(res_part.d(), res_blocks, b, RN);
                SCS_HIP_CHECK(hipMemcpyAsync(h_rn.data(), RN, (size_t)b * 8, hipMemcpyDeviceToHost, s));
                SCS_HIP_CHECK(hipMemcpyAsync(h_th.data(), TH, (size_t)(b + 1) * 8,
                                             hipMemcpyDeviceToHost, s));
                SCS_HIP_CHECK(hipStreamSynchronize(s));
                double w2 = 0.0;
                for (int j = 0; j < want; ++j) w2 = std::max(w2, std::sqrt(h_rn[j]));
                for (int j = 0; j < want; ++j) final_res[constrained ? 1 : j] = std::sqrt(h_rn[j]);
                bool conv = false;
                if (policy.confirm(w2, &conv)) {
                    converged = conv;
                    break;
                }
                if (fused) k_unit_coeffs<<<(3 * b * b + 255) / 256, 256, 0, s>>>(T, D, b);
                rr_solve = 0;
            } else {
                converged = worst <= tol;
                break;
            }
        }

        if (fused) continue;
        SCS_TRY(project_u(R, 1));
        for (int pass = 0; pass < 2; ++pass) {
            SCS_TRY(sv.gram(Q, q3, 2 * b, R, q3, b, C, sv.use_mfma));
            SCS_TRY(sv.update(R, q3, b, 1.0, Q, q3, 2 * b, C, b, -1.0));
        }
        SCS_TRY(svqb(R, nullptr, MASK + 2 * b));
        SCS_TRY(sv.apply(Q, 2 * b, AQ, 2 * b));

        SCS_TRY(sv.gram(Q, q3, q3, AQ, q3, q3, G, sv.use_mfma));
        k_small_rr<<<1, 256, 0, s>>>(G, 0, q3, b, MASK, T, D, TH, MASK + b, drop_tol);
        k_rr_update<<<(n + 15) / 16, 256, 0, s>>>(Q, b, q3, T, D, n);
        k_rr_update<<<(n + 15) / 16, 256, 0, s>>>(AQ, b, q3, T, D, n);
        SCS_HIP_CHECK(hipGetLastError());
    }

    hipEvent_t ev_c0 = nullptr, ev_c1 = nullptr;
    if (sv.new_event(&ev_c0) == SCS_OK && sv.new_event(&ev_c1) == SCS_OK) {
        sv.ev_cal[0] = ev_c0;
        sv.ev_cal[1] = ev_c1;
        hipEventRecord(ev_c0, s);
        hipEventRecord(ev_c1, s);
    }

    dbuf maps_d;
    SCS_TRY(maps_d.alloc((size_t)n * 2 * 8));
    k_extract_maps<<<(n + 255) / 256, 256, 0, s>>>(Q, q3, n, g->d_dinv, 1.0 / g->dd_norm, constrained ? 1 : 0,
                                                  maps_d.d());
    struct pinned_buf {
        scs_ctx *ctx;
        void *p = nullptr;
        ~pinned_buf() {
            if (p) scs_pinned_release(ctx, p);
        }
    } cols_h{ctx};
    SCS_TRY(scs_pinned_get(ctx, (size_t)n * 2 * 8, &cols_h.p));
    const double *cols = (const double *)cols_h.p;
    SCS_HIP_CHECK(hipMemcpyAsync(cols_h.p, maps_d.p, (size_t)n * 2 * 8, hipMemcpyDeviceToHost, s));
    if (!fused)
        SCS_HIP_CHECK(hipMemcpyAsync(h_th.data(), TH, (size_t)(b + 1) * 8, hipMemcpyDeviceToHost, s));
    SCS_HIP_CHECK(hipEventRecord(ev_b, s));
    SCS_HIP_CHECK(hipStreamSynchronize(s));
    std::vector<double> c0(n), c1(n);
    for (int i = 0; i < n; ++i) {
        c0[i] = cols[(size_t)i * 2];
        c1[i] = cols[(size_t)i * 2 + 1];
// ... 1130 lines not shown
```

spectralclustersupertree_amd/csrc/scs_internal.h:

```cpp
#pragma once

#include <hip/hip_runtime.h>

#include <cstdarg>
#include <cstdint>
#include <cstdio>
#include <cstring>
#include <mutex>
#include <string>
#include <vector>

#include "../../include/scs_hip.h"

void scs_set_error(const char *fmt, ...);

#define SCS_HIP_CHECK(expr)                                                                  \
    do {                                                                                     \
        hipError_t e_ = (expr);                                                              \
        if (e_ != hipSuccess) {                                                              \
            scs_set_error("%s failed: %s (%s:%d)", #expr, hipGetErrorString(e_), __FILE__,   \
                          __LINE__);                                                         \
            return (e_ == hipErrorOutOfMemory) ? SCS_ENOMEM : SCS_EHIP;                      \
        }                                                                                    \
    } while (0)

#define SCS_REQUIRE(cond, ...)                                                               \
    do {                                                                                     \
        if (!(cond)) {                                                                       \
            scs_set_error(__VA_ARGS__);                                                      \
            return SCS_EINVAL;                                                               \
        }                                                                                    \
    } while (0)

#define SCS_TRY(expr)                                                                        \
    do {                                                                                     \
        int rc_ = (expr);                                                                    \
        if (rc_ != SCS_OK) return rc_;                                                       \
    } while (0)

#include <cstdlib>
static inline const char *scs_dbg(const char *name) {
    static const bool on = [] {
        const char *e = getenv("SCS_DEBUG");
        return e && atoi(e) != 0;
    }();
    return on ? getenv(name) : nullptr;
}

struct scs_ctx;
hipError_t scs_dev_malloc_impl(scs_ctx *ctx, void **p, size_t bytes);
hipError_t scs_dev_free(void *p);
template <typename T>
static inline hipError_t scs_dev_malloc(scs_ctx *ctx, T **p, size_t bytes) {
    return scs_dev_malloc_impl(ctx, (void **)p, bytes);
}
size_t scs_arena_free_bytes(int device);

constexpr int SCS_TR = 64;
constexpr int SCS_TCW = 256;
constexpr int SCS_NPAD = 512;
constexpr int SCS_LD_ALIGN = 512;

constexpr size_t SCS_SCRATCH_KEEP = (size_t)1 << 30;
constexpr size_t SCS_PINNED_KEEP = (size_t)2 << 30;

struct scs_ctx;
int scs_block_alloc(scs_ctx *ctx, size_t bytes, void **out);
void scs_block_release(scs_ctx *ctx, void *p);
void scs_block_drop_free(scs_ctx *ctx);
int scs_pinned_get(scs_ctx *ctx, size_t bytes, void **out);
void scs_pinned_release(scs_ctx *ctx, void *p);

struct scs_local_group;

struct scs_comm {
    int rank = 0;
    int world = 1;
    int kind = 0;
    void *rccl_comm = nullptr;
    scs_local_group *group = nullptr;
};

int scs_comm_allgather_f64(scs_comm *comm, const double *sendbuf, double *recvbuf, size_t count,
                           hipStream_t stream);
int scs_comm_alltoallv_f64(scs_comm *comm, const double *sendbuf, const int64_t *send_off,
                           double *recvbuf, const int64_t *recv_off, hipStream_t stream);
int scs_comm_init_rccl(scs_comm *comm, int rank, int world, const void *uid);
int scs_comm_destroy(scs_comm *comm);

struct scs_ctx {
    int device = 0;
    hipStream_t stream = nullptr;
    hipStream_t copy_stream = nullptr;
    scs_comm comm;
    int n_cu = 256;
    int max_lds_bytes = 65536;
    size_t ws_limit = 0;
    double *h_report = nullptr;
    double *d_report = nullptr;
    unsigned long long report_seq = 0;
    struct scratch_slot {
        void *p = nullptr;
        size_t cap = 0;
    } scratch[8];
    hipEvent_t build_events[6] = {nullptr, nullptr, nullptr, nullptr, nullptr, nullptr};
    hipEvent_t solve_events[2] = {nullptr, nullptr};
    double *w_cache = nullptr;
    size_t w_cache_bytes = 0;
    float *w32_cache = nullptr;
    size_t w32_cache_bytes = 0;
    struct cached_block {
        void *p;
        size_t bytes;
        bool in_use;
    };
    std::mutex cache_mu;
    std::vector<cached_block> blocks;
    std::vector<cached_block> pinned;
    std::vector<hipEvent_t> event_pool;
    unsigned *h_flags = nullptr;
    struct small_slot {
        unsigned char *host = nullptr;
        unsigned char *dev = nullptr;
        size_t cap = 0;
        hipEvent_t done = nullptr;
        bool busy = false;
        size_t o_maps = 0, maps_bytes = 0, o_lam = 0, lam_bytes = 0, o_w = 0, w_bytes = 0;
        unsigned char *scratch = nullptr;
        size_t scratch_cap = 0;
    };
    std::vector<small_slot> small_slots;
    hipStream_t small_stream = nullptr;
};

struct scs_tables {
    int32_t n_taxa = 0;
    int32_t n_trees = 0;
    int64_t n_leaves = 0;
    int32_t max_leaves = 0;
    std::vector<int64_t> h_tree_off;
    void *d_block = nullptr;
    int64_t *d_tree_off = nullptr;
    int32_t *d_leaf_taxon = nullptr;
    int32_t *d_adj_depth = nullptr;
    double *d_adj_val = nullptr;
    double *d_tree_w = nullptr;
    mutable std::vector<int32_t> late_start;
    mutable std::vector<hipEvent_t> late_ev;
    unsigned *d_flags = nullptr;
};

int scs_tables_wait(scs_ctx *ctx, const scs_tables *t, int32_t t_end, hipStream_t stream);
int scs_tables_finish(scs_ctx *ctx, const scs_tables *t);

struct mf_data {
    const scs_tables *tb = nullptr;
    int64_t *d_stack_off = nullptr;
    int64_t stack_total = 0;
    int b_cap = 0;
    int chunks = 1;
    double *st_val = nullptr, *st_sum = nullptr;
    int32_t *st_dep = nullptr;
    double *sm_val = nullptr, *sm_sum = nullptr, *cy_pa = nullptr, *cy_ps = nullptr;
    int32_t *sm_dep = nullptr, *cy_dep = nullptr, *sm_cnt = nullptr, *sm_root = nullptr, *cy_cnt = nullptr;
    double *x = nullptr;
    double *y = nullptr;
    double *slabs = nullptr;
    int slabs_b = 0;
    int64_t n_apply = 0;
};

struct scs_graph {
    mf_data *mf = nullptr;
    int32_t n = 0;
    int32_t row_begin = 0;
    int32_t row_end = 0;
    int64_t ld = 0;
    double *d_w = nullptr;
    int32_t col0 = 0;
    bool upper = false;
    size_t w_bytes = 0;
    bool w_block = false;
    bool have_deg = false;
    void *deg_stage = nullptr;
    float *d_w32 = nullptr;
    size_t w32_bytes = 0;
    bool have_w32 = false;
    double *d_deg = nullptr;
    double *d_dinv = nullptr;
    int32_t n_isolated = 0;
    double dd_norm = 0.0;
};

#include <memory>
struct forest_region {
    scs_ctx *ctx = nullptr;
    std::shared_ptr<forest_region> base;
    std::vector<void *> blocks;
    void *host_block = nullptr;
    ~forest_region() {
        for (void *p : blocks) scs_block_release(ctx, p);
        if (host_block) scs_pinned_release(ctx, host_block);
    }
    int alloc(size_t bytes, void **out) {
        SCS_TRY(scs_block_alloc(ctx, bytes, out));
        blocks.push_back(*out);
        return SCS_OK;
    }
};

struct scs_forest {
    int32_t n_taxa = 0, n_trees = 0;
    int64_t n_nodes = 0, n_leaves = 0;
    std::shared_ptr<forest_region> region;
    int64_t *node_off = nullptr;
    int32_t *parent = nullptr, *taxon = nullptr;
    double *length = nullptr, *support = nullptr;
    double *weights = nullptr;
    mutable int32_t *tree_id = nullptr;
    bool has_tables = false;
    int64_t *tree_off = nullptr;
    int32_t *leaf_taxon = nullptr, *adj_depth = nullptr, *tree_index = nullptr;
    double *adj_val = nullptr;
    unsigned char *present = nullptr;
    const int64_t *h_tree_off = nullptr;
    const int32_t *h_leaf_taxon = nullptr, *h_adj_depth = nullptr, *h_tree_index = nullptr;
    const double *h_adj_val = nullptr, *h_weights = nullptr;
    const unsigned char *h_present = nullptr;
};


int scs_graph_prepare_degrees(scs_ctx *ctx, scs_graph *g);
int scs_graph_prepare_degrees_begin(scs_ctx *ctx, scs_graph *g, bool want_w32 = false);
int scs_matfree_apply(scs_ctx *ctx, scs_graph *g, const double *zt, int64_t ldz, int b, double *y_out,
                      hipStream_t stream);
void scs_matfree_release(scs_graph *g);
int scs_gather_row_splits(scs_ctx *ctx, int32_t row_begin, int32_t row_end, int32_t n,
                          std::vector<int32_t> &splits);


static inline int64_t scs_round_up(int64_t x, int64_t m) { return (x + m - 1) / m * m; }
```

spectralclustersupertree_amd/csrc/scs_mono.h:

```cpp
#pragma once

#include "scs_cells_asm.h"

constexpr int DV_LD = 65;
constexpr int DT_DOUBLES = 64 * DV_LD;
constexpr int R3_SPOS = 0;
constexpr int R3_G = 256;
constexpr int MONO_WAVES = 4;
constexpr int MONO_TCW = 64 * MONO_WAVES;
__host__ __device__ constexpr int mono_seg(int w) { return 64 * w / MONO_WAVES; }
constexpr int MONO_MAXSEG = (64 + MONO_WAVES - 1) / MONO_WAVES;
constexpr int R3_SEED = 768;
constexpr int R3_ARGPOS = R3_SEED + (MONO_WAVES - 1) * 512;
constexpr int R3_SORIG = R3_ARGPOS + 256;
constexpr int R3_RANK = R3_SORIG + 64;
constexpr int R3_PIV = R3_RANK + 64;
constexpr int R3_CNT = R3_PIV + 32;
constexpr int R3_M = R3_CNT + 4;
constexpr int R3_STOFF = R3_M + 4;
constexpr int R3_PIECE = (R3_STOFF + 8 + MONO_WAVES * 16 - 1) / (MONO_WAVES * 16) * 16;
constexpr int R3_BYTES = R3_PIECE * MONO_WAVES;
static_assert(R3_STOFF + 8 <= R3_BYTES && R3_PIECE <= 1024, "record layout");

#define SCS_BARE_BARRIER()                                        \
    do {                                                          \
        asm volatile("s_waitcnt lgkmcnt(0)" ::: "memory");        \
        __builtin_amdgcn_s_barrier();                             \
        asm volatile("" ::: "memory");                            \
    } while (0)

__global__ __launch_bounds__(64) void k_block_records_mono(
    const int64_t *__restrict__ tree_off, int t0, int tl0, int n_batch, const int32_t *__restrict__ pos,
    int64_t npad, const int64_t *__restrict__ st_off, const double *__restrict__ stv,
    const int64_t *__restrict__ am_off, const argmin_t *__restrict__ am_all,
    int row_begin, int row_end, unsigned char *__restrict__ rec_all) {
    const int blk = blockIdx.x;
    const int tl = tl0 + blockIdx.y;
    const int lane = threadIdx.x;
    const int m = (int)(tree_off[t0 + tl + 1] - tree_off[t0 + tl]) - 1;
    const int row = row_begin + blk * SCS_TR + lane;
    int p = -1;
    if (row < row_end) p = pos[(int64_t)tl * npad + row];
    const u32 pk = p < 0 ? 0x7FFFFFFFu : (u32)p;
    u64 key = ((u64)pk << 32) | (u32)lane;
    for (int k = 2; k <= 64; k <<= 1) {
        for (int j = k >> 1; j > 0; j >>= 1) {
            const u64 other = __shfl_xor(key, j, 64);
            const bool take_min = ((lane & j) == 0) == ((lane & k) == 0);
            const u64 lo = key < other ? key : other;
            const u64 hi = key < other ? other : key;
            key = take_min ? lo : hi;
        }
    }
    const int spos = (int)(key >> 32);
    const int orig = (int)(key & 63);
    const bool present = spos != 0x7FFFFFFF;
    const int cnt = __popcll(__ballot(present));
    const int next_pos = __shfl_down(spos, 1, 64);
    const double *st = stv + st_off[tl];
    double g = 0.0;
    int argpos = 0;
    if (lane < cnt - 1) g = rmq_min_at(st, am_all + am_off[tl], m, spos, next_pos, argpos);
    unsigned char *rec = rec_all + ((int64_t)blk * n_batch + tl) * R3_BYTES;
    ((int *)(rec + R3_SPOS))[lane] = spos;
    ((double *)(rec + R3_G))[lane] = g;
    ((int *)(rec + R3_ARGPOS))[lane] = argpos;
    if ((lane & 7) == 7) ((int *)(rec + R3_PIV))[lane >> 3] = spos;
    rec[R3_SORIG + lane] = (unsigned char)orig;
    rec[R3_RANK + orig] = (unsigned char)lane;
    if (lane == 0) {
        *(int *)(rec + R3_CNT) = cnt;
        *(int *)(rec + R3_M) = m;
        *(int64_t *)(rec + R3_STOFF) = st_off[tl];
    }
    {
        const double inf = __longlong_as_double(0x7FF0000000000000ll);
        double *seed = (double *)(rec + R3_SEED);
#pragma unroll
        for (int w = 1; w < MONO_WAVES; ++w) {
            const int end = mono_seg(w);
            double mine = lane < end ? g : inf;
#pragma unroll
            for (int off = 1; off < 64; off <<= 1) {
                const double other = __shfl_down(mine, off, 64);
                if (lane + off < end) mine = min_f64(mine, other);
            }
            seed[(w - 1) * 64 + lane] = mine;
        }
    }
}

struct mono_params {
    const int2 *tiles;
    const unsigned char *rec;
    const int32_t *pos;
    int64_t npad;
    const double *stv;
    int n_batch;
    double *w;
    int64_t ld;
    int n;
    int row_begin, row_end;
    int load_w;
    int mirror;
    double *tile_out;
    unsigned long long *stamps;
    int split_tiles;
    const int32_t *lists;
    const int32_t *list_cnt;
};

template <bool SYM, typename P>
__device__ __forceinline__ void tile_store(const P &p, double (&acc)[SCS_TR], const int2 tile,
                                           const int row0, const int col, const int self,
                                           const int tid, const int lane, const int wave,
                                           double *s_dv) {
    if (self >= 0) {
#pragma unroll
        for (int i = 0; i < SCS_TR; ++i)
            if (i == self) acc[i] = 0.0;
    }
    if (p.tile_out) {
        double *tp = p.tile_out + (int64_t)blockIdx.x * SCS_TR * MONO_TCW + tid;
        if (p.split_tiles > 0) {
            if (col < p.n) {
#pragma unroll
                for (int i = 0; i < SCS_TR; ++i)
                    if (row0 + i < p.row_end) tp[i * MONO_TCW] = acc[i];
            }
            return;
        }
#pragma unroll
        for (int i = 0; i < SCS_TR; ++i) tp[i * MONO_TCW] = acc[i];
        return;
    }
    if (col < p.n) {
#pragma unroll
        for (int i = 0; i < SCS_TR; ++i) {
            const int r = row0 + i;
            if (r < p.row_end) p.w[(int64_t)(r - p.row_begin) * p.ld + col] = acc[i];
        }
    }
    if (SYM && p.mirror) {
        __shared__ double t_own[MONO_TCW * 9 > DT_DOUBLES ? MONO_TCW * 9 : 1];
        double *t = MONO_TCW * 9 > DT_DOUBLES ? t_own : s_dv;
        const bool wave_mirrors = ((row0 / MONO_TCW) + 1) * MONO_TCW <= ((tile.y * MONO_TCW + wave * 64) / SCS_TR) * SCS_TR;
#pragma unroll
        for (int q = 0; q < SCS_TR / 8; ++q) {
            SCS_BARE_BARRIER();
#pragma unroll
            for (int j = 0; j < 8; ++j) t[tid * 9 + j] = acc[q * 8 + j];
            SCS_BARE_BARRIER();
            if (wave_mirrors) {
#pragma unroll
                for (int it = 0; it < 8; ++it) {
                    const int cl = wave * 64 + it * 8 + (lane >> 3);
                    const int c = tile.y * MONO_TCW + cl;
                    const int r = row0 + q * 8 + (lane & 7);
                    if (c < p.n && r < p.row_end) p.w[(int64_t)c * p.ld + r] = t[cl * 9 + (lane & 7)];
                }
            }
        }
    }
}

template <bool SYM, bool STAMPED, bool LISTED = false>
__global__ __launch_bounds__(MONO_TCW, MONO_TCW / 256) void k_accumulate_mono(mono_params p) {
    __shared__ __attribute__((aligned(16))) double s_dv[DT_DOUBLES];
    __shared__ __attribute__((aligned(16))) unsigned char s_rec[2][R3_BYTES];
    typedef __attribute__((address_space(3))) void *lds_ptr;

    unsigned long long ts[7] = {0, 0, 0, 0, 0, 0, 0}, tprev = 0;
    auto stamp = [&](int k) {
        if (STAMPED) {
            __builtin_amdgcn_sched_barrier(0);
            unsigned long long tnow;
            asm volatile("s_memtime %0\n\ts_waitcnt lgkmcnt(0)" : "=s"(tnow)::"memory");
            ts[k] += tnow - tprev;
            tprev = tnow;
            __builtin_amdgcn_sched_barrier(0);
        }
    };

    const int tid = threadIdx.x;
    const int lane = tid & 63;
    const int wave = __builtin_amdgcn_readfirstlane(tid >> 6);
    const int split = p.split_tiles;
    const int2 tile = p.tiles[split > 0 ? (int)blockIdx.x % split : (int)blockIdx.x];
    const int blk = tile.x;
    const int row0 = p.row_begin + blk * SCS_TR;
    const int col = tile.y * MONO_TCW + tid;
    const int nt = p.n_batch;
    typedef const __attribute__((address_space(4))) int32_t *clist;
    const clist lst = LISTED ? (clist)(size_t)(p.lists + (int64_t)blockIdx.x * nt) : nullptr;
    const int nl = LISTED ? __builtin_amdgcn_readfirstlane(p.list_cnt[blockIdx.x]) : nt;
    auto T = [&](int k) -> int { return LISTED ? lst[min(k, max(nl - 1, 0))] : k; };
    const int tl0 = LISTED ? 0 : (split > 0 ? (int)blockIdx.x / split : 0);
    const int tl1 = LISTED ? nl : (split > 0 ? tl0 + 1 : nt);
    const double inf = __longlong_as_double(0x7FF0000000000000ll);
    const int self = (col >= row0 && col < row0 + SCS_TR && col < p.row_end) ? col - row0 : -1;

    double acc[SCS_TR];
#pragma unroll
    for (int i = 0; i < SCS_TR; ++i) {
        double v = 0.0;
        if (p.load_w && p.tile_out)
            v = p.tile_out[((int64_t)blockIdx.x * SCS_TR + i) * MONO_TCW + tid];
        else if (p.load_w && col < p.n && row0 + i < p.row_end)
            v = p.w[(int64_t)(row0 - p.row_begin + i) * p.ld + col];
        acc[i] = v;
    }

    const unsigned char *rec_base = p.rec + (int64_t)blk * nt * R3_BYTES;
    const __amdgpu_buffer_rsrc_t r_rec =
        __builtin_amdgcn_make_buffer_rsrc((void *)rec_base, 0, nt * R3_BYTES, 0x00020000);
    const __amdgpu_buffer_rsrc_t r_pos =
        __builtin_amdgcn_make_buffer_rsrc((void *)p.pos, 0, (int)(nt * p.npad * 4), 0x00020000);
    const int lane16 = lane * 16;
    const int col4 = col * 4;
    auto issue_record = [&](int tl, int b) {
        if (lane < R3_PIECE / 16)
            __builtin_amdgcn_raw_ptr_buffer_load_lds(r_rec, (lds_ptr)(s_rec[b] + wave * R3_PIECE), 16,
                                                     lane16, tl * R3_BYTES + wave * R3_PIECE, 0, 0);
    };

    double qx = 0.0, qy = 0.0;
    int cstate = 0;
    int cpos_next = -1;

    auto column_issue = [&](int tl, int cpos, int t_next) {
        const unsigned char *rb = s_rec[tl & 1];
        const int *s_spos = (const int *)(rb + R3_SPOS);
        const int *s_arg = (const int *)(rb + R3_ARGPOS);
        const unsigned char *s_sorig = rb + R3_SORIG;
        const int *s_piv = (const int *)(rb + R3_PIV);
        const int cnt = __builtin_amdgcn_readfirstlane(*(const int *)(rb + R3_CNT));
        const bool present = cpos >= 0 && cnt > 0;
        int lo;
        {
            const int4 pa = *(const int4 *)&s_piv[0];
            const int4 pb = *(const int4 *)&s_piv[4];
            lo = ((pa.x < cpos) + (pa.y < cpos) + (pa.z < cpos) + (pa.w < cpos) + (pb.x < cpos) +
                  (pb.y < cpos) + (pb.z < cpos) + (pb.w < cpos)) * 8;
            const int base = min(lo, 56);
            int l2 = base;
#pragma unroll
            for (int s = 4; s > 0; s >>= 1)
                if (s_spos[l2 + s - 1] < cpos) l2 += s;
            lo = lo == 64 ? 64 : l2;
        }
        const bool hasl = present && self < 0 && lo > 0;
        const bool hasr = present && self < 0 && lo < cnt;
        const int il = max(lo - 1, 0), ir = min(lo, 63);
        const bool left = hasl && (!hasr || s_arg[il] >= cpos);
        const int q_anchor = s_spos[left ? il : ir];
        const int nbrow = s_sorig[left ? il : ir];
        cstate = nbrow | ((hasl || hasr) ? 256 : 0) | ((present && self >= 0) ? 512 : 0);
        const int m = __builtin_amdgcn_readfirstlane(*(const int *)(rb + R3_M));
        const unsigned so_lo = __builtin_amdgcn_readfirstlane(*(const unsigned *)(rb + R3_STOFF));
        const unsigned so_hi = __builtin_amdgcn_readfirstlane(*(const unsigned *)(rb + R3_STOFF + 4));
        const unsigned char *st = (const unsigned char *)(p.stv + (((u64)so_hi << 32) | so_lo));
        const bool any = hasl || hasr;
        int o[2];
        rmq_offsets(m, any ? (left ? q_anchor : cpos) : 0, any ? (left ? cpos : q_anchor) : 1, o);
        qx = *(const double *)(st + (unsigned)o[0] * 8u);
        qy = *(const double *)(st + (unsigned)o[1] * 8u);
        cpos_next = __builtin_amdgcn_raw_buffer_load_b32(r_pos, col4, t_next * (int)p.npad * 4, 0);
    };

    auto expand = [&](int tl) {
        const unsigned char *rb = s_rec[tl & 1];
        const int b0 = mono_seg(wave), b1 = mono_seg(wave + 1);
        const double g_rank = ((const double *)(rb + R3_G))[lane];
        const int so_rank = rb[R3_SORIG + lane];
        const int rho = rb[R3_RANK + lane];
        double cur = inf;
        if (rho < b0) cur = ((const double *)(rb + R3_SEED))[(wave - 1) * 64 + rho];
        double *row_a = &s_dv[lane * DV_LD];
        double *col_a = &s_dv[lane];
#pragma unroll
        for (int j = 0; j < MONO_MAXSEG; ++j) {
            const int b = b0 + j;
            if (b >= b1) break;
            const int lo32 = __builtin_amdgcn_readlane((int)__double2loint(g_rank), b);
            const int hi32 = __builtin_amdgcn_readlane(__double2hiint(g_rank), b);
            const int so_b = __builtin_amdgcn_readlane(so_rank, b);
            const double gb = __hiloint2double(hi32, lo32);
            if (rho <= b) {
                row_a[so_b] = cur;
                col_a[so_b * DV_LD] = cur;
                cur = min_f64(cur, gb);
            }
        }
    };

    if (LISTED && nl == 0) {
        tile_store<SYM>(p, acc, tile, row0, col, self, tid, lane, wave, s_dv);
        return;
    }
    issue_record(T(tl0), tl0 & 1);
    issue_record(T(min(tl0 + 1, nl - 1)), (tl0 + 1) & 1);
    cpos_next = __builtin_amdgcn_raw_buffer_load_b32(r_pos, col4, T(tl0) * (int)p.npad * 4, 0);
    asm volatile("s_waitcnt vmcnt(0)" ::: "memory");
    __syncthreads();
    column_issue(tl0, cpos_next, T(min(tl0 + 1, nl - 1)));
    if (STAMPED) asm volatile("s_memtime %0\n\ts_waitcnt lgkmcnt(0)" : "=s"(tprev)::"memory");

    for (int tl = tl0; tl < tl1; ++tl) {
        asm volatile("s_waitcnt vmcnt(0)" ::: "memory");
        stamp(0);
        SCS_BARE_BARRIER();
        stamp(1);
        int nb = 0;
        double vn = 0.0;
        if (cstate & 256) {
            vn = min_f64(qx, qy);
            nb = cstate & 255;
        } else if (cstate & 512) {
            nb = self;
            vn = inf;
        }
        stamp(2);
        column_issue(min(tl + 1, nl - 1), cpos_next, T(min(tl + 2, nl - 1)));
        stamp(3);
        expand(tl);
        stamp(4);
        SCS_BARE_BARRIER();
        stamp(5);
        issue_record(T(min(tl + 2, nl - 1)), tl & 1);
        {
            double tmp[SCS_CELLS_DEPTH];
            const unsigned addr =
                (unsigned)(size_t)(__attribute__((address_space(3))) double *)&s_dv[nb * DV_LD];
            SCS_CELLS_ASM(acc, tmp, addr, vn);
        }
        stamp(6);
    }

    if (STAMPED && lane == 0 && p.stamps) {
#pragma unroll
        for (int k = 0; k < 7; ++k) atomicAdd(&p.stamps[k], ts[k]);
        atomicAdd(&p.stamps[7], 1ull);
    }
    tile_store<SYM>(p, acc, tile, row0, col, self, tid, lane, wave, s_dv);
}

template <bool SYM, typename P>
__global__ __launch_bounds__(MONO_TCW) void k_sum_tree_tiles(P p, const double *__restrict__ cells, int n_tiles) {
    const int tile_i = (int)blockIdx.x / SCS_TR, i = (int)blockIdx.x % SCS_TR;
    const int2 tile = p.tiles[tile_i];
    const int row = p.row_begin + tile.x * SCS_TR + i;
    const int col = tile.y * MONO_TCW + (int)threadIdx.x;
    if (row >= p.row_end || col >= p.n) return;
    double *wcell = p.w + (int64_t)(row - p.row_begin) * p.ld + col;
    double acc = p.load_w ? *wcell : 0.0;
    const double *src = cells + ((int64_t)tile_i * SCS_TR + i) * MONO_TCW + threadIdx.x;
    const int64_t stride = (int64_t)n_tiles * SCS_TR * MONO_TCW;
    int t = 0;
    for (; t + 16 <= p.n_batch; t += 16) {
        double v[16];
#pragma unroll
        for (int k = 0; k < 16; ++k) v[k] = src[(int64_t)(t + k) * stride];
#pragma unroll
        for (int k = 0; k < 16; ++k) acc += v[k];
    }
    for (; t < p.n_batch; ++t) acc += src[(int64_t)t * stride];
    *wcell = acc;
    if (SYM && p.mirror && (row / MONO_TCW + 1) * MONO_TCW <= (col / SCS_TR) * SCS_TR)
        p.w[(int64_t)col * p.ld + row] = acc;
}
```

spectralclustersupertree_amd/csrc/scs_mono_wide.h:

```cpp
#pragma once

template <int NG>
struct wide_layout {
    static constexpr int NSEG = 4 * NG;
    static constexpr int SPOS = 0;
    static constexpr int G = 256;
    static constexpr int SEED = 768;
    static constexpr int ARGPOS = SEED + (NSEG - 1) * 512;
    static constexpr int SORIG = ARGPOS + 256;
    static constexpr int RANK = SORIG + 64;
    static constexpr int PIV = RANK + 64;
    static constexpr int CNT = PIV + 32;
    static constexpr int M = CNT + 4;
    static constexpr int STOFF = M + 4;
    static constexpr int BYTES = (STOFF + 8 + 15) / 16 * 16;
    static constexpr int PIECES = (BYTES + 1023) / 1024;
    __host__ __device__ static constexpr int seg(int w) { return 64 * w / NSEG; }
    static constexpr int MAXSEG = (64 + NSEG - 1) / NSEG;
    static_assert(STOFF % 8 == 0 && PIECES <= NSEG, "record layout");
};

template <int NG>
__global__ __launch_bounds__(64) void k_block_records_wide(
    const int64_t *__restrict__ tree_off, int t0, int tl0, int n_batch, const int32_t *__restrict__ pos,
    int64_t npad, const int64_t *__restrict__ st_off, const double *__restrict__ stv,
    const int64_t *__restrict__ am_off, const argmin_t *__restrict__ am_all,
    int row_begin, int row_end, unsigned char *__restrict__ rec_all) {
    using L = wide_layout<NG>;
    const int blk = blockIdx.x;
    const int tl = tl0 + blockIdx.y;
    const int lane = threadIdx.x;
    const int m = (int)(tree_off[t0 + tl + 1] - tree_off[t0 + tl]) - 1;
    const int row = row_begin + blk * SCS_TR + lane;
    int p = -1;
    if (row < row_end) p = pos[(int64_t)tl * npad + row];
    const u32 pk = p < 0 ? 0x7FFFFFFFu : (u32)p;
    u64 key = ((u64)pk << 32) | (u32)lane;
    for (int k = 2; k <= 64; k <<= 1) {
        for (int j = k >> 1; j > 0; j >>= 1) {
            const u64 other = __shfl_xor(key, j, 64);
            const bool take_min = ((lane & j) == 0) == ((lane & k) == 0);
            const u64 lo = key < other ? key : other;
            const u64 hi = key < other ? other : key;
            key = take_min ? lo : hi;
        }
    }
    const int spos = (int)(key >> 32);
    const int orig = (int)(key & 63);
    const bool present = spos != 0x7FFFFFFF;
    const int cnt = __popcll(__ballot(present));
    const int next_pos = __shfl_down(spos, 1, 64);
    const double *st = stv + st_off[tl];
    double g = 0.0;
    int argpos = 0;
    if (lane < cnt - 1) g = rmq_min_at(st, am_all + am_off[tl], m, spos, next_pos, argpos);
    unsigned char *rec = rec_all + ((int64_t)blk * n_batch + tl) * L::BYTES;
    ((int *)(rec + L::SPOS))[lane] = spos;
    ((double *)(rec + L::G))[lane] = g;
    ((int *)(rec + L::ARGPOS))[lane] = argpos;
    if ((lane & 7) == 7) ((int *)(rec + L::PIV))[lane >> 3] = spos;
    rec[L::SORIG + lane] = (unsigned char)orig;
    rec[L::RANK + orig] = (unsigned char)lane;
    if (lane == 0) {
        *(int *)(rec + L::CNT) = cnt;
        *(int *)(rec + L::M) = m;
        *(int64_t *)(rec + L::STOFF) = st_off[tl];
    }
    const double inf = __longlong_as_double(0x7FF0000000000000ll);
    double *seed = (double *)(rec + L::SEED);
#pragma unroll
    for (int w = 1; w < L::NSEG; ++w) {
        const int end = L::seg(w);
        double mine = lane < end ? g : inf;
#pragma unroll
        for (int off = 1; off < 64; off <<= 1) {
            const double other = __shfl_down(mine, off, 64);
            if (lane + off < end) mine = min_f64(mine, other);
        }
        seed[(w - 1) * 64 + lane] = mine;
    }
}

typedef int scs_int4 __attribute__((ext_vector_type(4)));

struct wide_params {
    mono_params m;
    const int4 *groups;
    int producer_prio;
};

template <bool SYM>
__device__ __forceinline__ void tile_store_wide(const mono_params &p, double (&acc)[SCS_TR],
                                                const int2 tile, const bool active, const int slot,
                                                const int row0, const int col, const int self,
                                                const int ltid, const int lane, const int wl,
                                                double *t) {
    if (self >= 0) {
#pragma unroll
        for (int i = 0; i < SCS_TR; ++i)
            if (i == self) acc[i] = 0.0;
    }
    if (p.tile_out) {
        if (active) {
            double *tp = p.tile_out + (int64_t)slot * SCS_TR * MONO_TCW + ltid;
#pragma unroll
            for (int i = 0; i < SCS_TR; ++i) tp[i * MONO_TCW] = acc[i];
        }
        return;
    }
    if (active && col < p.n) {
#pragma unroll
        for (int i = 0; i < SCS_TR; ++i) {
            const int r = row0 + i;
            if (r < p.row_end) p.w[(int64_t)(r - p.row_begin) * p.ld + col] = acc[i];
        }
    }
    if (SYM && p.mirror) {
        const bool wave_mirrors =
            active && ((row0 / MONO_TCW) + 1) * MONO_TCW <= ((tile.y * MONO_TCW + wl * 64) / SCS_TR) * SCS_TR;
#pragma unroll
        for (int q = 0; q < SCS_TR / 8; ++q) {
            SCS_BARE_BARRIER();
#pragma unroll
            for (int j = 0; j < 8; ++j) t[ltid * 9 + j] = acc[q * 8 + j];
            SCS_BARE_BARRIER();
            if (wave_mirrors) {
#pragma unroll
                for (int it = 0; it < 8; ++it) {
                    const int cl = wl * 64 + it * 8 + (lane >> 3);
                    const int c = tile.y * MONO_TCW + cl;
                    const int r = row0 + q * 8 + (lane & 7);
                    if (c < p.n && r < p.row_end) p.w[(int64_t)c * p.ld + r] = t[cl * 9 + (lane & 7)];
                }
            }
        }
    }
}

struct spec_layout {
    using L = wide_layout<2>;
    static constexpr int CONSUMERS = 8, PRODUCERS = 4, THREADS = 64 * (CONSUMERS + PRODUCERS);
    static constexpr size_t O_T = 0;
    static constexpr int NREC = 6;
    static constexpr size_t O_REC = 2 * (size_t)DT_DOUBLES * 8;
    static constexpr size_t O_VN = O_REC + NREC * (size_t)L::BYTES;
    static constexpr size_t O_ADDR = O_VN + 2 * 512 * 8;
    static constexpr size_t LDS_BYTES = O_ADDR + 2 * 512 * 4;
    static_assert(O_VN % 16 == 0 && 3 * (size_t)MONO_TCW * 9 * 8 <= LDS_BYTES, "layout");
};

template <bool SYM, bool STAMPED>
__global__ __launch_bounds__(spec_layout::THREADS) void k_accumulate_spec(wide_params wp) {
    using S = spec_layout;
    using L = wide_layout<2>;
    extern __shared__ __attribute__((aligned(16))) unsigned char s_mem[];
    double *const s_t = (double *)(s_mem + S::O_T);
    unsigned char *const s_rec = s_mem + S::O_REC;
    double *const s_vn = (double *)(s_mem + S::O_VN);
    unsigned *const s_addr = (unsigned *)(s_mem + S::O_ADDR);
    const mono_params &p = wp.m;

    unsigned long long ts[7] = {0, 0, 0, 0, 0, 0, 0}, tprev = 0;
    auto stamp = [&](int k) {
        if (STAMPED) {
            __builtin_amdgcn_sched_barrier(0);
            unsigned long long tnow;
            asm volatile("s_memtime %0\n\ts_waitcnt lgkmcnt(0)" : "=s"(tnow)::"memory");
            ts[k] += tnow - tprev;
            tprev = tnow;
            __builtin_amdgcn_sched_barrier(0);
        }
    };

    const int tid = threadIdx.x;
    const int lane = tid & 63;
    const int wave = __builtin_amdgcn_readfirstlane(tid >> 6);
    const bool producer = wave >= S::CONSUMERS;
    const int pw = wave - S::CONSUMERS;
    const int4 grp = wp.groups[blockIdx.x];
    const int nt = p.n_batch;
    const double inf = __longlong_as_double(0x7FF0000000000000ll);
    const int cw = producer ? 2 * pw : wave;
    const int sub = cw >> 2, wl = cw & 3;
    const int ltid = (cw & 3) * 64 + lane;
    const int ti = sub == 0 ? grp.x : grp.y;
    const bool active = ti >= 0;
    const int2 tile = p.tiles[active ? ti : grp.x];
    const int blk = tile.x;
    const int row0 = p.row_begin + blk * SCS_TR;
    const int col = tile.y * MONO_TCW + ltid;
    const int self = (col >= row0 && col < row0 + SCS_TR && col < p.row_end) ? col - row0 : -1;

    const unsigned char *rec_base = p.rec + (int64_t)blk * nt * L::BYTES;
    const __amdgpu_buffer_rsrc_t r_pos =
        __builtin_amdgcn_make_buffer_rsrc((void *)p.pos, 0, (int)(nt * p.npad * 4), 0x00020000);
    const int lane16 = lane * 16;

    const __amdgpu_buffer_rsrc_t r_rec =
        __builtin_amdgcn_make_buffer_rsrc((void *)rec_base, 0, nt * L::BYTES, 0x00020000);
    struct pieces {
        scs_int4 v[2];
    };
    auto load_record = [&](int t, pieces &r) {
        if (t >= nt) return;
#pragma unroll
        for (int pc = 0; pc < L::PIECES; pc += S::PRODUCERS) {
            const int piece = pc + pw;
            if (piece < L::PIECES) {
                const int left = (L::BYTES - piece * 1024) / 16;
                if (lane < left)
                    r.v[pc / S::PRODUCERS] =
                        __builtin_amdgcn_raw_buffer_load_b128(r_rec, lane16, t * L::BYTES + piece * 1024, 0);
            }
        }
    };
    auto store_record = [&](int t, const pieces &r) {
        if (t >= nt) return;
#pragma unroll
        for (int pc = 0; pc < L::PIECES; pc += S::PRODUCERS) {
            const int piece = pc + pw;
            if (piece < L::PIECES) {
                const int left = (L::BYTES - piece * 1024) / 16;
                if (lane < left)
                    *(scs_int4 *)(s_rec + (t % S::NREC) * L::BYTES + piece * 1024 + lane16) = r.v[pc / S::PRODUCERS];
            }
        }
    };
    int pcol4[2], pself[2], cpos[2], cpos2[2];
#pragma unroll
    for (int k = 0; k < 2; ++k) {
        const int c = tile.y * MONO_TCW + (((2 * pw + k) & 3) * 64) + lane;
        pcol4[k] = c * 4;
        pself[k] = (c >= row0 && c < row0 + SCS_TR && c < p.row_end) ? c - row0 : -1;
        cpos[k] = -1;
        cpos2[k] = -1;
    }
    struct query {
        double qx[2], qy[2];
        int cstate[2];
    };
    typedef const __attribute__((address_space(4))) int *cint;
    int tail[12];
    auto request_tail = [&](int t) {
        cint gpiv = (cint)(size_t)(rec_base + (int64_t)min(t, nt - 1) * L::BYTES + L::PIV);
#pragma unroll
        for (int k = 0; k < 12; ++k) tail[k] = gpiv[k];
    };
    auto search = [&](int t_raw, query &q) {
        const int t = min(t_raw, nt - 1);
        const unsigned char *rb = s_rec + (t % S::NREC) * L::BYTES;
        const int *s_spos = (const int *)(rb + L::SPOS);
        const int *s_arg = (const int *)(rb + L::ARGPOS);
        const unsigned char *s_sorig = rb + L::SORIG;
        const int4 pa = make_int4(tail[0], tail[1], tail[2], tail[3]);
        const int4 pb = make_int4(tail[4], tail[5], tail[6], tail[7]);
        const int cnt = tail[8], m = tail[9];
        const unsigned so_lo = (unsigned)tail[10], so_hi = (unsigned)tail[11];
        static_assert(L::CNT == L::PIV + 32 && L::M == L::PIV + 36 && L::STOFF == L::PIV + 40, "record tail");
        const unsigned char *st = (const unsigned char *)(p.stv + (((u64)so_hi << 32) | so_lo));
        int cp_now[2];
#pragma unroll
        for (int k = 0; k < 2; ++k) {
            cp_now[k] = cpos[k];
            cpos[k] = cpos2[k];
            cpos2[k] = __builtin_amdgcn_raw_buffer_load_b32(r_pos, pcol4[k], min(t + 2, nt - 1) * (int)p.npad * 4, 0);
        }
#pragma unroll
        for (int k = 0; k < 2; ++k) {
            const int cp = cp_now[k];
            const bool present = cp >= 0 && cnt > 0;
            int lo = ((pa.x < cp) + (pa.y < cp) + (pa.z < cp) + (pa.w < cp) + (pb.x < cp) + (pb.y < cp) +
                      (pb.z < cp) + (pb.w < cp)) * 8;
            const int base = min(lo, 56);
            const int4 qa = *(const int4 *)&s_spos[base];
            const int4 qb = *(const int4 *)&s_spos[base + 4];
            const int l2 = base + (qa.x < cp) + (qa.y < cp) + (qa.z < cp) + (qa.w < cp) + (qb.x < cp) +
                           (qb.y < cp) + (qb.z < cp);
            lo = lo == 64 ? 64 : l2;
            const bool hasl = present && pself[k] < 0 && lo > 0;
            const bool hasr = present && pself[k] < 0 && lo < cnt;
            const int il = max(lo - 1, 0), ir = min(lo, 63);
            const int a_il = s_arg[il];
            const int sp_il = s_spos[il], sp_ir = s_spos[ir];
            const int so_il = s_sorig[il], so_ir = s_sorig[ir];
            const bool left = hasl && (!hasr || a_il >= cp);
            const int q_anchor = left ? sp_il : sp_ir;
            const int nbrow = left ? so_il : so_ir;
            q.cstate[k] = nbrow | ((hasl || hasr) ? 256 : 0) | ((present && pself[k] >= 0) ? 512 : 0);
            const bool any = hasl || hasr;
            int o[2];
            rmq_offsets(m, any ? (left ? q_anchor : cp) : 0, any ? (left ? cp : q_anchor) : 1, o);
            q.qx[k] = *(const double *)(st + (unsigned)o[0] * 8u);
            q.qy[k] = *(const double *)(st + (unsigned)o[1] * 8u);
        }
        request_tail(t_raw + 1);
    };
    auto finish = [&](int t, const query &q) {
        const unsigned tbase =
            (unsigned)(size_t)(__attribute__((address_space(3))) double *)&s_t[(t & 1) * DT_DOUBLES];
#pragma unroll
        for (int k = 0; k < 2; ++k) {
            int nb = 0;
            double vn = 0.0;
            if (q.cstate[k] & 256) {
                vn = min_f64(q.qx[k], q.qy[k]);
                nb = q.cstate[k] & 255;
            } else if (q.cstate[k] & 512) {
                nb = pself[k];
                vn = inf;
            }
            const int slot = (t & 1) * 512 + (2 * pw + k) * 64 + lane;
            s_vn[slot] = vn;
            s_addr[slot] = tbase + (unsigned)nb * (DV_LD * 8);
        }
    };

    auto expand_whole = [&](int t) {
        const unsigned char *rb = s_rec + (t % S::NREC) * L::BYTES;
        double *dv = s_t + (t & 1) * DT_DOUBLES;
        const int b0 = L::seg(wave);
        const double g_rank = ((const double *)(rb + L::G))[lane];
        const int so_rank = rb[L::SORIG + lane];
        const int rho = rb[L::RANK + lane];
        double cur = inf;
        if (rho < b0) cur = ((const double *)(rb + L::SEED))[(wave - 1) * 64 + rho];
        double *row_a = &dv[lane * DV_LD];
        double *col_a = &dv[lane];
#pragma unroll
        for (int j = 0; j < 8; ++j) {
            const int b = b0 + j;
            const int lo32 = __builtin_amdgcn_readlane((int)__double2loint(g_rank), b);
            const int hi32 = __builtin_amdgcn_readlane(__double2hiint(g_rank), b);
            const int so_b = __builtin_amdgcn_readlane(so_rank, b);
            const double gb = __hiloint2double(hi32, lo32);
            if (rho <= b) {
                row_a[so_b] = cur;
                col_a[so_b * DV_LD] = cur;
                cur = min_f64(cur, gb);
            }
        }
    };

    if (producer) {
        pieces ra = {{{0, 0, 0, 0}, {0, 0, 0, 0}}}, rb = ra, rc = ra;
        {
            pieces first[5] = {ra, ra, ra, ra, ra};
#pragma unroll
            for (int t = 0; t < 5; ++t) load_record(t, first[t]);
#pragma unroll
            for (int t = 0; t < 5; ++t) store_record(t, first[t]);
        }
        load_record(5, ra);
        load_record(6, rb);
        load_record(7, rc);
#pragma unroll
        for (int k = 0; k < 2; ++k) {
            cpos[k] = __builtin_amdgcn_raw_buffer_load_b32(r_pos, pcol4[k], 0, 0);
            cpos2[k] = __builtin_amdgcn_raw_buffer_load_b32(r_pos, pcol4[k], min(1, nt - 1) * (int)p.npad * 4, 0);
        }
        SCS_BARE_BARRIER();
        query qa = {{0.0, 0.0}, {0.0, 0.0}, {0, 0}}, qb = qa, qc = qa;
        request_tail(0);
        search(0, qa);
        finish(0, qa);
        search(1, qa);
        search(2, qb);
        search(3, qc);
        SCS_BARE_BARRIER();
        if (STAMPED) asm volatile("s_memtime %0\n\ts_waitcnt lgkmcnt(0)" : "=s"(tprev)::"memory");
        if (wp.producer_prio == 1) __builtin_amdgcn_s_setprio(1);
        else if (wp.producer_prio == 2) __builtin_amdgcn_s_setprio(2);
        else if (wp.producer_prio == 3) __builtin_amdgcn_s_setprio(3);
        auto step = [&](int tl, query &q1, pieces &r1) __attribute__((always_inline)) {
            if (tl + 1 < nt) finish(tl + 1, q1);
            stamp(0);
            store_record(tl + 5, r1);
            load_record(tl + 8, r1);
            search(tl + 4, q1);
            stamp(1);
            SCS_BARE_BARRIER();
            stamp(4);
        };
        for (int tl = 0; tl < nt; tl += 3) {
            step(tl, qa, ra);
            if (tl + 1 < nt) step(tl + 1, qb, rb);
            if (tl + 2 < nt) step(tl + 2, qc, rc);
        }
        if (STAMPED && lane == 0 && p.stamps) {
#pragma unroll
            for (int k = 0; k < 7; ++k) atomicAdd(&p.stamps[k], ts[k]);
            atomicAdd(&p.stamps[7], 1ull);
        }
        if (!p.tile_out && SYM && p.mirror) {
#pragma unroll
            for (int q = 0; q < SCS_TR / 8; ++q) {
                SCS_BARE_BARRIER();
                SCS_BARE_BARRIER();
            }
        }
    } else {
        double acc[SCS_TR];
#pragma unroll
        for (int i = 0; i < SCS_TR; ++i) {
            double v = 0.0;
            if (active && p.load_w && p.tile_out)
                v = p.tile_out[((int64_t)ti * SCS_TR + i) * MONO_TCW + ltid];
            else if (active && p.load_w && col < p.n && row0 + i < p.row_end)
                v = p.w[(int64_t)(row0 - p.row_begin + i) * p.ld + col];
            acc[i] = v;
        }
        asm volatile("s_waitcnt vmcnt(0)" ::: "memory");
        SCS_BARE_BARRIER();
        expand_whole(0);
        SCS_BARE_BARRIER();
        if (STAMPED) asm volatile("s_memtime %0\n\ts_waitcnt lgkmcnt(0)" : "=s"(tprev)::"memory");
        for (int tl = 0; tl < nt; ++tl) {
            const int slot = (tl & 1) * 512 + wave * 64 + lane;
            const double vn = s_vn[slot];
            const unsigned addr = s_addr[slot];
            const unsigned char *rb = s_rec + (min(tl + 1, nt - 1) % S::NREC) * L::BYTES;
            const double g_rank = ((const double *)(rb + L::G))[lane];
            const int so_rank = rb[L::SORIG + lane];
            const int rho = rb[L::RANK + lane];
            const int b0 = L::seg(wave);
            double cur = inf;
            if (rho < b0) cur = ((const double *)(rb + L::SEED))[(wave - 1) * 64 + rho];
            double *dv = s_t + ((tl + 1) & 1) * DT_DOUBLES;
            const unsigned rowb = (unsigned)(size_t)(__attribute__((address_space(3))) double *)&dv[lane * DV_LD];
            const unsigned colb = (unsigned)(size_t)(__attribute__((address_space(3))) double *)&dv[lane];
            stamp(2);
            double tmp[SCS_CELLS_DEPTH];
            unsigned x1, x2;
            SCS_CELLS_EXPAND_ASM(acc, tmp, x1, x2, addr, vn, cur, (int)__double2loint(g_rank),
                                 __double2hiint(g_rank), so_rank, rho, rowb, colb, b0, DV_LD * 8);
            stamp(3);
            SCS_BARE_BARRIER();
            stamp(4);
        }
        if (STAMPED && lane == 0 && p.stamps) {
#pragma unroll
            for (int k = 0; k < 7; ++k) atomicAdd(&p.stamps[k], ts[k]);
            atomicAdd(&p.stamps[7], 1ull);
        }
        tile_store_wide<SYM>(p, acc, tile, active, ti, row0, col, self, ltid, lane, wl,
                             (double *)s_mem + (size_t)sub * MONO_TCW * 9);
    }
}
```

Baseline: 0.01400.

## Fuse degree partial sums and fp32 image writes into accumulate tile stores

The symmetric accumulate kernels now emit per-tile row and column degree partial sums, and optionally the fp32 image of W, while storing tiles. A small finish kernel reduces the partials into deg/dinv and zeroes the image padding. The host copy of degrees is queued asynchronously, so the solve no longer needs a separate degree pass over W or the extra synchronisation. Per-batch events replace the per-batch event sync inside the build loop. In exchange there are more global writes and reductions in the tile epilogue, a partials buffer of (n_cgroups+n_blocks)*n doubles, and more complex degree-state bookkeeping.

```diff
diff --git a/spectralclustersupertree_amd/csrc/scs_build.hip b/spectralclustersupertree_amd/csrc/scs_build.hip
--- a/spectralclustersupertree_amd/csrc/scs_build.hip
+++ b/spectralclustersupertree_amd/csrc/scs_build.hip
@@ -357,6 +357,58 @@
     dinv[i] = d == 0.0 ? 1.0 : 1.0 / sqrt(d);
 }
 
+constexpr int DEGF_PARTS = 8;
+__global__ __launch_bounds__(64 * DEGF_PARTS) void k_degrees_finish(const double *__restrict__ parts, int n,
+                                                                    int n_cgroups, double *__restrict__ deg,
+                                                                    double *__restrict__ dinv,
+                                                                    float *__restrict__ w32, int64_t ld) {
+    __shared__ double s_part[DEGF_PARTS][64];
+    const int r0 = blockIdx.x * 64;
+    const int lane = threadIdx.x & 63, part = threadIdx.x >> 6;
+    const int r = r0 + lane;
+    double d = 0.0;
+    if (r < n) {
+        const int grp = r / SCS_TCW;
+        const int terms = n_cgroups - grp + grp * (SCS_TCW / SCS_TR);
+        const double *src = parts + (int64_t)grp * n + r;
+        int k = part;
+        for (; k + 3 * DEGF_PARTS < terms; k += 4 * DEGF_PARTS) {
+            double v[4];
+#pragma unroll
+            for (int u = 0; u < 4; ++u) v[u] = src[(int64_t)(k + u * DEGF_PARTS) * n];
+#pragma unroll
+            for (int u = 0; u < 4; ++u) d += v[u];
+        }
+        for (; k < terms; k += DEGF_PARTS) d += src[(int64_t)k * n];
+    }
+    s_part[part][lane] = d;
+    __syncthreads();
+    if (part == 0 && r < n) {
+        d = s_part[0][lane];
+#pragma unroll
+        for (int p = 1; p < DEGF_PARTS; ++p) d += s_part[p][lane];
+        deg[r] = d;
+        dinv[r] = d == 0.0 ? 1.0 : 1.0 / sqrt(d);
+    }
+    if (w32)
+        for (int i = r0 + part; i < min(r0 + 64, n); i += DEGF_PARTS)
+            for (int64_t j = n + lane; j < ld; j += 64) w32[(int64_t)i * ld + j] = 0.f;
+}
+
+bool scs_graph_image_wanted(const scs_ctx *ctx, const scs_graph *g) {
+    const int n = g->n;
+    const int lowp_mode = getenv("SCS_LOWP") ? atoi(getenv("SCS_LOWP")) : 2;
+    const bool loop_fused = !(scs_dbg("SCS_LEGACY_LOOP") && atoi(scs_dbg("SCS_LEGACY_LOOP"))) &&
+                            !(scs_dbg("SCS_SPLIT_SMALL") && atoi(scs_dbg("SCS_SPLIT_SMALL"))) &&
+                            !(scs_dbg("SCS_FOLD_PASS2") && !atoi(scs_dbg("SCS_FOLD_PASS2")));
+    const double lowp_max_bytes = getenv("SCS_LOWP_MAX_BYTES") ? atof(getenv("SCS_LOWP_MAX_BYTES")) : 16.0 * (1u << 30);
+    const int min_n = scs_dbg("SCS_IMAGE_MIN_N") ? atoi(scs_dbg("SCS_IMAGE_MIN_N")) : 4096;
+    const bool image_rows = ctx->comm.world > 1 && !g->upper;
+    const bool image_one = ctx->comm.world == 1 && !g->upper && g->row_begin == 0 && g->row_end == n;
+    return !g->mf && lowp_mode > 0 && n >= min_n && loop_fused && (image_one || image_rows) &&
+           (g->have_w32 || 4.0 * (double)(g->row_end - g->row_begin) * (double)g->ld <= lowp_max_bytes);
+}
+
 namespace {
 
 struct dev_buf {
@@ -471,6 +523,26 @@
     }
     *out = g;
     return SCS_OK;
+}
+
+static bool graph_take_image(scs_ctx *ctx, scs_graph *g) {
+    if (g->d_w32) return true;
+    const size_t need = (size_t)(g->row_end - g->row_begin) * g->ld * 4;
+    std::lock_guard<std::mutex> lock(ctx->cache_mu);
+    if (ctx->w32_cache && ctx->w32_cache_bytes >= need) {
+        g->d_w32 = ctx->w32_cache;
+        g->w32_bytes = ctx->w32_cache_bytes;
+        ctx->w32_cache = nullptr;
+        ctx->w32_cache_bytes = 0;
+    } else if (scs_dev_malloc(ctx, (void **)&g->d_w32, need) == hipSuccess) {
+        g->w32_bytes = need;
+        if (scs_dbg("SCS_TRACE_SOLVES") && atoi(scs_dbg("SCS_TRACE_SOLVES")))
+            fprintf(stderr, "[image] hipMalloc of %.2f GB\n", need / 1073741824.0);
+    } else {
+        (void)hipGetLastError();
+        g->d_w32 = nullptr;
+    }
+    return g->d_w32 != nullptr;
 }
 
 extern "C" int scs_graph_free(scs_ctx *ctx, scs_graph *g) {
@@ -874,18 +946,28 @@
 
     struct ev_ref {
         hipEvent_t a, b;
-    } ev_total, ev_prep, ev_acc;
-    for (auto &e : ctx->build_events)
-        if (!e) SCS_HIP_CHECK(hipEventCreate(&e));
+    } ev_total;
+    if (ctx->build_events.size() < 2 + 4 * (size_t)n_batches) ctx->build_events.resize(2 + 4 * (size_t)n_batches, nullptr);
+    for (size_t i = 0; i < 2 + 4 * (size_t)n_batches; ++i)
+        if (!ctx->build_events[i]) SCS_HIP_CHECK(hipEventCreate(&ctx->build_events[i]));
     ev_total = {ctx->build_events[0], ctx->build_events[1]};
-    ev_prep = {ctx->build_events[2], ctx->build_events[3]};
-    ev_acc = {ctx->build_events[4], ctx->build_events[5]};
+    std::vector<char> batch_wide((size_t)n_batches, 0);
     float prep_ms = 0.f, acc_ms = 0.f;
     SCS_HIP_CHECK(hipEventRecord(ev_total.a, s));
 
+    bool fuse_deg = sym && monotone && !scatter && !tree_par && !listed && !trapezoid && !tiles.empty() &&
+                    !(scs_dbg("SCS_ACC_STAMP") && atoi(scs_dbg("SCS_ACC_STAMP"))) &&
+                    !(scs_dbg("SCS_FUSED_DEGREES") && atoi(scs_dbg("SCS_FUSED_DEGREES")) == 0);
+    cached_buf d_deg_parts(ctx);
+    if (fuse_deg && d_deg_parts.alloc((size_t)(n_cgroups + n_blocks) * (size_t)n * 8) != SCS_OK) fuse_deg = false;
+    if (fuse_deg) {
+        SCS_TRY(scs_block_alloc(ctx, (size_t)n * 8, (void **)&g->d_deg));
+        SCS_TRY(scs_block_alloc(ctx, (size_t)n * 8, (void **)&g->d_dinv));
+        if (scs_graph_image_wanted(ctx, g)) graph_take_image(ctx, g);
+    }
+
     int spec_batches = 0, spec_trees = 0;
     float spec_ms = 0.f;
-    bool single_batch_spec = false;
     pooled_buf d_pos(ctx, 1), d_am(ctx, 2), d_st(ctx, 3), d_stoff(ctx, 4), d_rec(ctx, 5), d_cells(ctx, 6);
     dev_buf d_pcol(ctx), d_lists(ctx), d_list_cnt(ctx);
     int listed_batches = 0;
@@ -927,13 +1009,15 @@
         if (wide_b) {
             ++spec_batches;
             spec_trees += nb;
-            single_batch_spec = true;
         }
         SCS_TRY(d_pos.alloc(need_pos));
         SCS_TRY(d_st.alloc(need_st));
         SCS_TRY(d_am.alloc(need_am));
         SCS_TRY(d_rec.alloc(need_rec));
 
+        const ev_ref ev_prep = {ctx->build_events[2 + 4 * (size_t)bi], ctx->build_events[3 + 4 * (size_t)bi]};
+        const ev_ref ev_acc = {ctx->build_events[4 + 4 * (size_t)bi], ctx->build_events[5 + 4 * (size_t)bi]};
+        batch_wide[(size_t)bi] = wide_b ? 1 : 0;
         SCS_HIP_CHECK(hipEventRecord(ev_prep.a, s));
         SCS_HIP_CHECK(hipMemsetAsync(d_pos.p, 0xFF, need_pos, s));
         prep_batch pb;
@@ -990,6 +1074,10 @@
             mp.split_tiles = 0;
             mp.lists = nullptr;
             mp.list_cnt = nullptr;
+            const bool fuse_b = fuse_deg && mp.mirror;
+            mp.deg_row = fuse_b ? (double *)d_deg_parts.p : nullptr;
+            mp.deg_col = fuse_b ? (double *)d_deg_parts.p + (size_t)n_cgroups * n : nullptr;
+            mp.w32 = fuse_b ? g->d_w32 : nullptr;
             const bool stamp = scs_dbg("SCS_ACC_STAMP") && atoi(scs_dbg("SCS_ACC_STAMP"));
             if (wide_b) {
                 wide_params wp;
@@ -1003,18 +1091,19 @@
                     SCS_HIP_CHECK(hipMemsetAsync(d_st8.p, 0, 64, s));
                     wp.m.stamps = (unsigned long long *)d_st8.p;
                 }
-#define SCS_LAUNCH_SPEC(SYM_, STAMP_)                                                                   \
-    do {                                                                                                \
-        SCS_HIP_CHECK(hipFuncSetAttribute((const void *)k_accumulate_spec<SYM_, STAMP_>,                \
-                                          hipFuncAttributeMaxDynamicSharedMemorySize,                   \
-                                          (int)spec_layout::LDS_BYTES));                                \
-        k_accumulate_spec<SYM_, STAMP_><<<ng, spec_layout::THREADS, spec_layout::LDS_BYTES, s>>>(wp);   \
+#define SCS_LAUNCH_SPEC(SYM_, STAMP_, FUSED_)                                                                   \
+    do {                                                                                                        \
+        SCS_HIP_CHECK(hipFuncSetAttribute((const void *)k_accumulate_spec<SYM_, STAMP_, FUSED_>,                \
+                                          hipFuncAttributeMaxDynamicSharedMemorySize,                           \
+                                          (int)spec_layout::LDS_BYTES));                                        \
+        k_accumulate_spec<SYM_, STAMP_, FUSED_><<<ng, spec_layout::THREADS, spec_layout::LDS_BYTES, s>>>(wp);   \
     } while (0)
                 if (ng) {
-                    if (stamp && sym) SCS_LAUNCH_SPEC(true, true);
-                    else if (stamp) SCS_LAUNCH_SPEC(false, true);
-                    else if (sym) SCS_LAUNCH_SPEC(true, false);
-                    else SCS_LAUNCH_SPEC(false, false);
+                    if (stamp && sym) SCS_LAUNCH_SPEC(true, true, false);
+                    else if (stamp) SCS_LAUNCH_SPEC(false, true, false);
+                    else if (fuse_b) SCS_LAUNCH_SPEC(true, false, true);
+                    else if (sym) SCS_LAUNCH_SPEC(true, false, false);
+                    else SCS_LAUNCH_SPEC(false, false, false);
                 }
 #undef SCS_LAUNCH_SPEC
                 if (stamp) {
@@ -1072,7 +1161,8 @@
                 else k_accumulate_mono<false, false, true><<<nt, MONO_TCW, 0, s>>>(mp);
                 ++listed_batches;
             } else if (nt) {
-                if (sym) k_accumulate_mono<true, false><<<nt, MONO_TCW, 0, s>>>(mp);
+                if (fuse_b) k_accumulate_mono<true, false, false, true><<<nt, MONO_TCW, 0, s>>>(mp);
+                else if (sym) k_accumulate_mono<true, false><<<nt, MONO_TCW, 0, s>>>(mp);
                 else k_accumulate_mono<false, false><<<nt, MONO_TCW, 0, s>>>(mp);
             }
         } else {
@@ -1109,15 +1199,15 @@
         }
         SCS_HIP_CHECK(hipGetLastError());
         SCS_HIP_CHECK(hipEventRecord(ev_acc.b, s));
-        if (n_batches > 1) {
-            SCS_HIP_CHECK(hipEventSynchronize(ev_acc.b));
-            float ms = 0.f;
-            SCS_HIP_CHECK(hipEventElapsedTime(&ms, ev_prep.a, ev_prep.b));
-            prep_ms += ms;
-            SCS_HIP_CHECK(hipEventElapsedTime(&ms, ev_acc.a, ev_acc.b));
-            acc_ms += ms;
-            if (wide_b) spec_ms += ms;
-        }
+    }
+    if (fuse_deg) {
+        k_degrees_finish<<<(n + 63) / 64, 64 * DEGF_PARTS, 0, s>>>((const double *)d_deg_parts.p, n, n_cgroups,
+                                                                   g->d_deg, g->d_dinv, g->d_w32, g->ld);
+        SCS_HIP_CHECK(hipGetLastError());
+        SCS_TRY(scs_pinned_get(ctx, (size_t)n * 8, &g->deg_stage));
+        SCS_HIP_CHECK(hipMemcpyAsync(g->deg_stage, g->d_deg, (size_t)n * 8, hipMemcpyDeviceToHost, s));
+        g->deg_fused = true;
+        g->have_w32 = g->d_w32 != nullptr;
     }
     float exch_ms = 0.f;
     double exch_bytes = 0.0;
@@ -1190,10 +1280,14 @@
     SCS_TRY(scs_tables_finish(ctx, tb));
     float total_ms = 0.f;
     SCS_HIP_CHECK(hipEventElapsedTime(&total_ms, ev_total.a, ev_total.b));
-    if (n_batches == 1) {
-        SCS_HIP_CHECK(hipEventElapsedTime(&prep_ms, ev_prep.a, ev_prep.b));
-        SCS_HIP_CHECK(hipEventElapsedTime(&acc_ms, ev_acc.a, ev_acc.b));
-        if (single_batch_spec) spec_ms = acc_ms;
+    g->deg_landed = g->deg_fused;
+    for (int bi = 0; bi < n_batches; ++bi) {
+        float ms = 0.f;
+        SCS_HIP_CHECK(hipEventElapsedTime(&ms, ctx->build_events[2 + 4 * (size_t)bi], ctx->build_events[3 + 4 * (size_t)bi]));
+        prep_ms += ms;
+        SCS_HIP_CHECK(hipEventElapsedTime(&ms, ctx->build_events[4 + 4 * (size_t)bi], ctx->build_events[5 + 4 * (size_t)bi]));
+        acc_ms += ms;
+        if (batch_wide[(size_t)bi]) spec_ms += ms;
     }
 
     if (stats) {
@@ -1321,7 +1415,7 @@
 }
 
 int scs_graph_prepare_degrees_begin(scs_ctx *ctx, scs_graph *g, bool want_w32) {
-    if (g->deg_stage) return SCS_OK;
+    if (g->deg_stage && !(g->deg_fused && want_w32 && !g->have_w32)) return SCS_OK;
     const int n = g->n;
     const int rows = g->row_end - g->row_begin;
     if (g->mf && !g->have_deg) {
@@ -1339,28 +1433,20 @@
     const bool img_rows = ctx->comm.world > 1 && !g->upper;
     bool need_img = want_w32 && !g->have_w32 && !g->upper &&
                     (img_rows || (ctx->comm.world == 1 && g->row_begin == 0 && rows == n));
-    if (g->have_deg && !need_img) return SCS_OK;
+    if ((g->have_deg || g->deg_fused) && !need_img) return SCS_OK;
     SCS_HIP_CHECK(hipSetDevice(ctx->device));
     hipStream_t s = ctx->stream;
-    if (need_img && !g->d_w32) {
-        const size_t need = (size_t)rows * g->ld * 4;
-        std::lock_guard<std::mutex> lock(ctx->cache_mu);
-        if (ctx->w32_cache && ctx->w32_cache_bytes >= need) {
-            g->d_w32 = ctx->w32_cache;
-            g->w32_bytes = ctx->w32_cache_bytes;
-            ctx->w32_cache = nullptr;
-            ctx->w32_cache_bytes = 0;
-        } else if (scs_dev_malloc(ctx, (void **)&g->d_w32, need) == hipSuccess) {
-            g->w32_bytes = need;
-            if (scs_dbg("SCS_TRACE_SOLVES") && atoi(scs_dbg("SCS_TRACE_SOLVES")))
-                fprintf(stderr, "[image] hipMalloc of %.2f GB\n", need / 1073741824.0);
-        } else {
-            (void)hipGetLastError();
-            g->d_w32 = nullptr;
-            need_img = false;
-        }
-    }
-    if (!need_img && g->have_deg) return SCS_OK;
+    if (need_img && !graph_take_image(ctx, g)) need_img = false;
+    if (!need_img && (g->have_deg || g->deg_fused)) return SCS_OK;
+    if (need_img && g->deg_fused) {
+        cached_buf tmp(ctx);
+        SCS_TRY(tmp.alloc((size_t)n * 8));
+        k_degrees<true><<<(rows + 3) / 4, 256, 0, s>>>(g->d_w, g->ld, n, rows, g->row_begin, (double *)tmp.p, g->d_w32);
+        SCS_HIP_CHECK(hipGetLastError());
+        SCS_HIP_CHECK(hipStreamSynchronize(s));
+        g->have_w32 = true;
+        return SCS_OK;
+    }
     if (need_img && img_rows && g->have_deg) {
         dev_buf tmp(ctx);
         SCS_TRY(tmp.alloc((size_t)n * 8));
@@ -1415,7 +1501,8 @@
 int scs_graph_prepare_degrees(scs_ctx *ctx, scs_graph *g) {
     if (g->have_deg) return SCS_OK;
     SCS_TRY(scs_graph_prepare_degrees_begin(ctx, g));
-    const hipError_t e = hipStreamSynchronize(ctx->stream);
+    const hipError_t e = g->deg_landed ? hipSuccess : hipStreamSynchronize(ctx->stream);
+    g->deg_landed = false;
     const double *deg = (const double *)g->deg_stage;
     int iso = 0;
     double nrm2 = 0.0;
diff --git a/spectralclustersupertree_amd/csrc/scs_eig.hip b/spectralclustersupertree_amd/csrc/scs_eig.hip
--- a/spectralclustersupertree_amd/csrc/scs_eig.hip
+++ b/spectralclustersupertree_amd/csrc/scs_eig.hip
@@ -2148,14 +2148,8 @@
 
     const int lowp_mode = getenv("SCS_LOWP") ? atoi(getenv("SCS_LOWP")) : 2;
     const double lowp_tol = 1e-8, lowp_tol2 = 0.0;
-    const bool loop_fused = !(scs_dbg("SCS_LEGACY_LOOP") && atoi(scs_dbg("SCS_LEGACY_LOOP"))) &&
-                            !(scs_dbg("SCS_SPLIT_SMALL") && atoi(scs_dbg("SCS_SPLIT_SMALL"))) &&
-                            !(scs_dbg("SCS_FOLD_PASS2") && !atoi(scs_dbg("SCS_FOLD_PASS2")));
-    const double lowp_max_bytes = getenv("SCS_LOWP_MAX_BYTES") ? atof(getenv("SCS_LOWP_MAX_BYTES")) : 16.0 * (1u << 30);
     const bool image_rows = ctx->comm.world > 1 && !g->upper;
-    const bool image_one = ctx->comm.world == 1 && !g->upper && g->row_begin == 0 && g->row_end == n;
-    const bool image_ok = !g->mf && lowp_mode > 0 && n >= 4096 && loop_fused && (image_one || image_rows) &&
-                          (g->have_w32 || 4.0 * (double)(g->row_end - g->row_begin) * (double)g->ld <= lowp_max_bytes);
+    const bool image_ok = scs_graph_image_wanted(ctx, g);
     int b = block ? block : ((n >= 16384 && !image_ok) ? 8 : 4);
     if (g->upper && b > 8) b = 8;
     if (g->mf) b = std::min(b <= 4 ? 4 : 8, g->mf->b_cap);
diff --git a/spectralclustersupertree_amd/csrc/scs_internal.h b/spectralclustersupertree_amd/csrc/scs_internal.h
--- a/spectralclustersupertree_amd/csrc/scs_internal.h
+++ b/spectralclustersupertree_amd/csrc/scs_internal.h
@@ -103,7 +103,7 @@
         void *p = nullptr;
         size_t cap = 0;
     } scratch[8];
-    hipEvent_t build_events[6] = {nullptr, nullptr, nullptr, nullptr, nullptr, nullptr};
+    std::vector<hipEvent_t> build_events;
     hipEvent_t solve_events[2] = {nullptr, nullptr};
     double *w_cache = nullptr;
     size_t w_cache_bytes = 0;
@@ -183,6 +183,7 @@
     bool w_block = false;
     bool have_deg = false;
     void *deg_stage = nullptr;
+    bool deg_fused = false, deg_landed = false;
     float *d_w32 = nullptr;
     size_t w32_bytes = 0;
     bool have_w32 = false;
@@ -232,6 +233,7 @@
 
 int scs_graph_prepare_degrees(scs_ctx *ctx, scs_graph *g);
 int scs_graph_prepare_degrees_begin(scs_ctx *ctx, scs_graph *g, bool want_w32 = false);
+bool scs_graph_image_wanted(const scs_ctx *ctx, const scs_graph *g);
 int scs_matfree_apply(scs_ctx *ctx, scs_graph *g, const double *zt, int64_t ldz, int b, double *y_out,
                       hipStream_t stream);
 void scs_matfree_release(scs_graph *g);
diff --git a/spectralclustersupertree_amd/csrc/scs_mono.h b/spectralclustersupertree_amd/csrc/scs_mono.h
--- a/spectralclustersupertree_amd/csrc/scs_mono.h
+++ b/spectralclustersupertree_amd/csrc/scs_mono.h
@@ -108,9 +108,56 @@
     int split_tiles;
     const int32_t *lists;
     const int32_t *list_cnt;
+    double *deg_row;
+    double *deg_col;
+    float *w32;
 };
 
-template <bool SYM, typename P>
+__device__ __forceinline__ unsigned long long late_u64(unsigned long long v) {
+    asm volatile("" : "+s"(v));
+    return v;
+}
+__device__ __forceinline__ int late_i32(int v) {
+    asm volatile("" : "+s"(v));
+    return v;
+}
+
+__device__ __forceinline__ void tile_col_sums(double *deg_col_blk, const double (&acc)[SCS_TR], const bool incol,
+                                              const int col, const int nrow) {
+    double cs = 0.0;
+#pragma unroll
+    for (int i = 0; i < SCS_TR; ++i) cs += i < nrow ? acc[i] : 0.0;
+    if (incol) deg_col_blk[col] = cs;
+}
+
+template <int CTRL>
+__device__ __forceinline__ double mono_dpp_f64(double v) {
+    int lo = __double2loint(v), hi = __double2hiint(v);
+    lo = __builtin_amdgcn_update_dpp(0, lo, CTRL, 0xF, 0xF, true);
+    hi = __builtin_amdgcn_update_dpp(0, hi, CTRL, 0xF, 0xF, true);
+    return __hiloint2double(hi, lo);
+}
+
+__device__ __forceinline__ void tile_row_sums(double *deg_row_tile, const double *t, const int q, const int nrow,
+                                              const int ncol, const int lane, const int wl) {
+    const int j = wl * 2 + (lane >> 5), l = lane & 31;
+    double s = 0.0;
+#pragma unroll
+    for (int m = 0; m < MONO_TCW / 32; ++m) {
+        const int cl = m * 32 + l;
+        const double v = t[cl * 9 + j];
+        s += cl < ncol ? v : 0.0;
+    }
+    s += mono_dpp_f64<0xB1>(s);
+    s += mono_dpp_f64<0x4E>(s);
+    s += mono_dpp_f64<0x141>(s);
+    s += mono_dpp_f64<0x140>(s);
+    s += __shfl_xor(s, 16, 64);
+    const int i = q * 8 + j;
+    if (l == 0 && i < nrow) deg_row_tile[i] = s;
+}
+
+template <bool SYM, bool FUSED = false, typename P>
 __device__ __forceinline__ void tile_store(const P &p, double (&acc)[SCS_TR], const int2 tile,
                                            const int row0, const int col, const int self,
                                            const int tid, const int lane, const int wave,
@@ -134,17 +181,42 @@
         for (int i = 0; i < SCS_TR; ++i) tp[i * MONO_TCW] = acc[i];
         return;
     }
+    bool fuse = false, img = false;
+    float *w32 = nullptr;
+    double *deg_row_tile = nullptr, *deg_col_blk = nullptr;
+    int64_t ld32 = 0;
+    int row_end32 = 0, n32 = 0;
+    if constexpr (SYM && FUSED) {
+        fuse = p.mirror && p.deg_row != nullptr;
+        img = fuse && p.w32 != nullptr;
+        w32 = (float *)late_u64((unsigned long long)p.w32);
+        ld32 = (int64_t)late_u64((unsigned long long)p.ld);
+        row_end32 = late_i32(p.row_end);
+        n32 = late_i32(p.n);
+        deg_row_tile = (double *)late_u64((unsigned long long)p.deg_row) + ((int64_t)tile.y * n32 + row0);
+        deg_col_blk = (double *)late_u64((unsigned long long)p.deg_col) + (int64_t)tile.x * n32;
+    }
     if (col < p.n) {
 #pragma unroll
         for (int i = 0; i < SCS_TR; ++i) {
             const int r = row0 + i;
             if (r < p.row_end) p.w[(int64_t)(r - p.row_begin) * p.ld + col] = acc[i];
+        }
+        if constexpr (SYM && FUSED) {
+            if (img) {
+#pragma unroll
+                for (int i = 0; i < SCS_TR; ++i) {
+                    const int r = row0 + i;
+                    if (r < row_end32) w32[(int64_t)r * ld32 + col] = (float)acc[i];
+                }
+            }
         }
     }
     if (SYM && p.mirror) {
         __shared__ double t_own[MONO_TCW * 9 > DT_DOUBLES ? MONO_TCW * 9 : 1];
         double *t = MONO_TCW * 9 > DT_DOUBLES ? t_own : s_dv;
         const bool wave_mirrors = ((row0 / MONO_TCW) + 1) * MONO_TCW <= ((tile.y * MONO_TCW + wave * 64) / SCS_TR) * SCS_TR;
+        const bool img_mirror = img && row0 / 512 == tile.y * MONO_TCW / 512;
 #pragma unroll
         for (int q = 0; q < SCS_TR / 8; ++q) {
             SCS_BARE_BARRIER();
@@ -157,14 +229,22 @@
                     const int cl = wave * 64 + it * 8 + (lane >> 3);
                     const int c = tile.y * MONO_TCW + cl;
                     const int r = row0 + q * 8 + (lane & 7);
-                    if (c < p.n && r < p.row_end) p.w[(int64_t)c * p.ld + r] = t[cl * 9 + (lane & 7)];
+                    if (c < p.n && r < p.row_end) {
+                        const double v = t[cl * 9 + (lane & 7)];
+                        p.w[(int64_t)c * p.ld + r] = v;
+                        if constexpr (FUSED) {
+                            if (img_mirror) w32[(int64_t)c * ld32 + r] = (float)v;
+                        }
+                    }
                 }
             }
-        }
-    }
-}
-
-template <bool SYM, bool STAMPED, bool LISTED = false>
+            if (fuse) tile_row_sums(deg_row_tile, t, q, row_end32 - row0, n32 - tile.y * MONO_TCW, lane, wave);
+        }
+        if (fuse && wave_mirrors) tile_col_sums(deg_col_blk, acc, col < n32, col, row_end32 - row0);
+    }
+}
+
+template <bool SYM, bool STAMPED, bool LISTED = false, bool FUSED = false>
 __global__ __launch_bounds__(MONO_TCW, MONO_TCW / 256) void k_accumulate_mono(mono_params p) {
     __shared__ __attribute__((aligned(16))) double s_dv[DT_DOUBLES];
     __shared__ __attribute__((aligned(16))) unsigned char s_rec[2][R3_BYTES];
@@ -295,7 +375,7 @@
     };
 
     if (LISTED && nl == 0) {
-        tile_store<SYM>(p, acc, tile, row0, col, self, tid, lane, wave, s_dv);
+        tile_store<SYM, FUSED>(p, acc, tile, row0, col, self, tid, lane, wave, s_dv);
         return;
     }
     issue_record(T(tl0), tl0 & 1);
@@ -342,7 +422,7 @@
         for (int k = 0; k < 7; ++k) atomicAdd(&p.stamps[k], ts[k]);
         atomicAdd(&p.stamps[7], 1ull);
     }
-    tile_store<SYM>(p, acc, tile, row0, col, self, tid, lane, wave, s_dv);
+    tile_store<SYM, FUSED>(p, acc, tile, row0, col, self, tid, lane, wave, s_dv);
 }
 
 template <bool SYM, typename P>
diff --git a/spectralclustersupertree_amd/csrc/scs_mono_wide.h b/spectralclustersupertree_amd/csrc/scs_mono_wide.h
--- a/spectralclustersupertree_amd/csrc/scs_mono_wide.h
+++ b/spectralclustersupertree_amd/csrc/scs_mono_wide.h
@@ -89,7 +89,7 @@
     int producer_prio;
 };
 
-template <bool SYM>
+template <bool SYM, bool FUSED>
 __device__ __forceinline__ void tile_store_wide(const mono_params &p, double (&acc)[SCS_TR],
                                                 const int2 tile, const bool active, const int slot,
                                                 const int row0, const int col, const int self,
@@ -108,16 +108,39 @@
         }
         return;
     }
+    bool fuse = false, img = false;
+    float *w32 = nullptr;
+    double *deg_row_tile = nullptr, *deg_col_blk = nullptr;
+    int64_t ld32 = 0;
+    int row_end32 = 0, n32 = 0;
+    if constexpr (SYM && FUSED) {
+        fuse = p.mirror && p.deg_row != nullptr;
+        img = fuse && p.w32 != nullptr;
+        w32 = (float *)late_u64((unsigned long long)p.w32);
+        ld32 = (int64_t)late_u64((unsigned long long)p.ld);
+        row_end32 = late_i32(p.row_end);
+        n32 = late_i32(p.n);
+        deg_row_tile = (double *)late_u64((unsigned long long)p.deg_row) + ((int64_t)tile.y * n32 + row0);
+        deg_col_blk = (double *)late_u64((unsigned long long)p.deg_col) + (int64_t)tile.x * n32;
+    }
     if (active && col < p.n) {
 #pragma unroll
         for (int i = 0; i < SCS_TR; ++i) {
             const int r = row0 + i;
             if (r < p.row_end) p.w[(int64_t)(r - p.row_begin) * p.ld + col] = acc[i];
         }
+        if (img) {
+#pragma unroll
+            for (int i = 0; i < SCS_TR; ++i) {
+                const int r = row0 + i;
+                if (r < row_end32) w32[(int64_t)r * ld32 + col] = (float)acc[i];
+            }
+        }
     }
     if (SYM && p.mirror) {
         const bool wave_mirrors =
             active && ((row0 / MONO_TCW) + 1) * MONO_TCW <= ((tile.y * MONO_TCW + wl * 64) / SCS_TR) * SCS_TR;
+        const bool img_mirror = img && row0 / 512 == tile.y * MONO_TCW / 512;
 #pragma unroll
         for (int q = 0; q < SCS_TR / 8; ++q) {
             SCS_BARE_BARRIER();
@@ -130,10 +153,16 @@
                     const int cl = wl * 64 + it * 8 + (lane >> 3);
                     const int c = tile.y * MONO_TCW + cl;
                     const int r = row0 + q * 8 + (lane & 7);
-                    if (c < p.n && r < p.row_end) p.w[(int64_t)c * p.ld + r] = t[cl * 9 + (lane & 7)];
+                    if (c < p.n && r < p.row_end) {
+                        const double v = t[cl * 9 + (lane & 7)];
+                        p.w[(int64_t)c * p.ld + r] = v;
+                        if (img_mirror) w32[(int64_t)c * ld32 + r] = (float)v;
+                    }
                 }
             }
-        }
+            if (fuse && active) tile_row_sums(deg_row_tile, t, q, row_end32 - row0, n32 - tile.y * MONO_TCW, lane, wl);
+        }
+        if (fuse && wave_mirrors) tile_col_sums(deg_col_blk, acc, col < n32, col, row_end32 - row0);
     }
 }
 
@@ -149,7 +178,7 @@
     static_assert(O_VN % 16 == 0 && 3 * (size_t)MONO_TCW * 9 * 8 <= LDS_BYTES, "layout");
 };
 
-template <bool SYM, bool STAMPED>
+template <bool SYM, bool STAMPED, bool FUSED = false>
 __global__ __launch_bounds__(spec_layout::THREADS) void k_accumulate_spec(wide_params wp) {
     using S = spec_layout;
     using L = wide_layout<2>;
@@ -442,7 +471,7 @@
             for (int k = 0; k < 7; ++k) atomicAdd(&p.stamps[k], ts[k]);
             atomicAdd(&p.stamps[7], 1ull);
         }
-        tile_store_wide<SYM>(p, acc, tile, active, ti, row0, col, self, ltid, lane, wl,
+        tile_store_wide<SYM, FUSED>(p, acc, tile, active, ti, row0, col, self, ltid, lane, wl,
                              (double *)s_mem + (size_t)sub * MONO_TCW * 9);
     }
 }
```

Result: no change. 0.01401 (+0.1%).
